# s-elkazdadi/ddp-pinocchio

Measured on AMD Instinct MI355X. Metric: DDP iterations/sec (fwd+bwd sweep), Talos nq=38 T=200, higher is better.
Workload: dtype f64

## Files before the change

### ddp_pinocchio_amd/csrc/bwd.hip

```cpp
#include <stdio.h>
#include <stdlib.h>

#include "internal.h"

namespace {

struct BwdParams {
  Dims d;
  const int64_t* ne;
  const int64_t* Epre;
  const double *lfx, *lfxx, *lx, *lu, *lxx, *lux, *luu, *fx, *fu, *fxx, *fux, *fuu;
  const double *eq_val, *eq_x, *eq_u, *eq_xx, *eq_ux, *eq_uu;
  const double *x, *mult_val, *mult_jac;
  double *fb_origin, *fb_val, *fb_jac, *vx_trace, *vxx_trace;
  double *ws_V, *ws_Q, *reg, *mu;
  int32_t* status;
  int64_t* restarts;
  const BwdJob* jobs;
  const BwdJob* jobs_half;
  int32_t njobs_half;
  int32_t half_mode;
  const double *u, *ctrl_lo, *ctrl_hi;
  double* box_stat;
  int32_t has_tensors;
  int32_t sym_tensors;
};

constexpr int BS = 256;
typedef double f64x2 __attribute__((ext_vector_type(2)));

__global__ __launch_bounds__(BS) void bwd_init(BwdParams p) {
  const int b = blockIdx.x;
  const int s = p.status[b];
  if (s == 2) return;
  const int64_t n = p.d.n;
  double* Vx = p.ws_V + (int64_t)b * (n + n * n);
  double* Vxx = Vx + n;
  const double* lfx = p.lfx + (int64_t)b * n;
  const double* lfxx = p.lfxx + (int64_t)b * n * n;
  for (int64_t i = threadIdx.x; i < n; i += BS) Vx[i] = lfx[i];
  for (int64_t i = threadIdx.x; i < n * n; i += BS) Vxx[i] = lfxx[i];
  __syncthreads();
  if (threadIdx.x == 0 && s == 1) p.status[b] = 0;
}

template <int OC>
__device__ __forceinline__ void contract_slab(const double* __restrict__ Tn, int O_rt, int L, const double* s_v,
                                              double* s_part, double* out, int out_stride) {
  const int O = OC > 0 ? OC : O_rt;
  const int hp = O >> 1;
  const int ld = hp + 1;
  const int total = hp * L;
  const f64x2* __restrict__ T2 = reinterpret_cast<const f64x2*>(Tn);
  const int tid = threadIdx.x;
#pragma unroll 4
  for (int f = tid; f < total; f += BS) {
    const f64x2 a = __builtin_nontemporal_load(&T2[f]);
    const int j = f / hp;
    const int ip = f - j * hp;
    s_part[j * ld + ip] = s_v[2 * ip] * a.x + s_v[2 * ip + 1] * a.y;
  }
  __syncthreads();
  for (int j = tid; j < L; j += BS) {
    double s = 0.0;
    const double* pj = s_part + j * ld;
    for (int k = 0; k < hp; ++k) s += pj[k];
    out[j * out_stride] += s;
  }
  __syncthreads();
}

template <int NC, int MC>
__global__ __launch_bounds__(BS) void bwd_assemble(BwdParams p, int64_t t) {
  const int b = blockIdx.y;
  if (p.status[b] != 0) return;
  const BwdJob job = p.jobs[blockIdx.x];
  const int n = NC > 0 ? NC : (int)p.d.n;
  const int m = MC > 0 ? MC : (int)p.d.m;
  const int64_t T = p.d.T;
  const int e = (int)p.ne[t];
  const int64_t Eo = p.Epre[t];
  const int64_t Etot = p.d.Etot;
  const double mu = p.mu[b];
  const int tid = threadIdx.x;
  const int kind = job.kind, c0 = job.c0, cn = job.cn;
  const int rows = kind == 0 ? n + m : m;

  const double* Vx = p.ws_V + (int64_t)b * (n + (int64_t)n * n);
  const double* Vxx = Vx + n;
  double* Q = p.ws_Q + (int64_t)b * (n + m + (int64_t)n * n + (int64_t)m * n + (int64_t)m * m);
  double* Qx = Q;
  double* Qu = Qx + n;
  double* Qxx = Qu + m;
  double* Qux = Qxx + (int64_t)n * n;
  double* Quu = Qux + (int64_t)m * n;

  const int64_t bt = (int64_t)b * T + t;
  const double* fx = p.fx + bt * n * n;
  const double* fu = p.fu + bt * n * m;
  const double* eqv = p.eq_val + (int64_t)b * Etot + Eo;
  const double* eqx = p.eq_x + ((int64_t)b * Etot + Eo) * n;
  const double* equ = p.eq_u + ((int64_t)b * Etot + Eo) * m;
  const double* pe = p.mult_val + (int64_t)b * Etot + Eo;
  const double* pex = p.mult_jac + ((int64_t)b * Etot + Eo) * n;
// ... 332 lines not shown
    for (int i = 0; i < m; ++i) {
      double s = r[i];
      for (int l = 0; l < i; ++l) s -= A[i + l * lda] * r[l];
      r[i] = s / A[i + i * lda];
    }
    for (int i = m - 1; i >= 0; --i) {
      double s = r[i];
      for (int l = i + 1; l < m; ++l) s -= A[l + i * lda] * r[l];
      r[i] = s / A[i + i * lda];
    }
  }
  __syncthreads();

  double* fbo = p.fb_origin + bt * nx;
  double* fbk = p.fb_val + bt * m;
  double* fbK = p.fb_jac + bt * m * n;
  const double* xt = p.x + ((int64_t)b * (T + 1) + t) * nx;
  for (int i = tid; i < nx; i += BS) fbo[i] = xt[i];
  for (int i = tid; i < m; i += BS) fbk[i] = R[i];
  for (int idx = tid; idx < m * n; idx += BS) fbK[idx] = R[idx % m + (idx / m + 1) * ldr];

  for (int i = tid; i < n; i += BS) {
    double s = 0.0;
    for (int l = 0; l < m; ++l) s += S[l + i * ldr] * R[l];
    const double v = Qx[i] + s;
    Vx[i] = v;
    if (p.vx_trace) p.vx_trace[bt * n + i] = v;
  }
  for (int idx = tid; idx < n * n; idx += BS) {
    const int i = idx % n, j = idx / n;
    double s = 0.0;
    const double* si = S + i * ldr;
    const double* kj = R + (j + 1) * ldr;
    for (int l = 0; l < m; ++l) s += si[l] * kj[l];
    const double v = Qxx[idx] + s;
    Vxx[idx] = v;
    if (p.vxx_trace) p.vxx_trace[bt * n * n + idx] = v;
  }
  if (t == 0 && tid == 0) p.status[b] = 2;
}

#include "bwd_fast.h"
#include "bwd_split.h"
#include "bwd_v2.h"

size_t assemble_lds_bytes(const ddp_hip_ctx* ctx, int cn_max) {
  const Dims& d = ctx->d;
  int64_t L = d.n > d.m ? d.n : d.m;
  int64_t words = d.n + d.emax + d.n * cn_max + (d.n + d.m) * cn_max + (d.n / 2 + 1) * L;
  return (size_t)words * sizeof(double);
}
size_t gains_lds_bytes(const ddp_hip_ctx* ctx) {
  const Dims& d = ctx->d;
  int64_t ld = d.m | 1;
  int64_t words = ld * d.m + ld * (d.n + 1) + ld * d.n;
  if (ctx->flags & DDP_HIP_FLAG_CONTROL_BOUNDS) words += ld * d.m + 9 * d.m;
  return (size_t)words * sizeof(double);
}

BwdParams make_params(ddp_hip_ctx* ctx, const SweepPlan& plan) {
  BwdParams p{};
  p.d = ctx->d;
  p.ne = ctx->ne_d;
  p.Epre = ctx->Epre_d;
  auto S = [&](int s) { return ctx->seq[s].ptr; };
  p.lfx = S(DDP_HIP_SEQ_LFX); p.lfxx = S(DDP_HIP_SEQ_LFXX);
  p.lx = S(DDP_HIP_SEQ_LX); p.lu = S(DDP_HIP_SEQ_LU); p.lxx = S(DDP_HIP_SEQ_LXX); p.lux = S(DDP_HIP_SEQ_LUX); p.luu = S(DDP_HIP_SEQ_LUU);
  p.fx = S(DDP_HIP_SEQ_FX); p.fu = S(DDP_HIP_SEQ_FU);
  p.fxx = S(DDP_HIP_SEQ_FXX); p.fux = S(DDP_HIP_SEQ_FUX); p.fuu = S(DDP_HIP_SEQ_FUU);
  p.eq_val = S(DDP_HIP_SEQ_EQ_VAL); p.eq_x = S(DDP_HIP_SEQ_EQ_X); p.eq_u = S(DDP_HIP_SEQ_EQ_U);
  p.eq_xx = S(DDP_HIP_SEQ_EQ_XX); p.eq_ux = S(DDP_HIP_SEQ_EQ_UX); p.eq_uu = S(DDP_HIP_SEQ_EQ_UU);
  p.x = S(DDP_HIP_SEQ_X);
  p.u = S(DDP_HIP_SEQ_U); p.ctrl_lo = S(DDP_HIP_SEQ_CTRL_LO); p.ctrl_hi = S(DDP_HIP_SEQ_CTRL_HI); p.box_stat = S(DDP_HIP_SEQ_BOX_STAT);
  p.mult_val = S(DDP_HIP_SEQ_MULT_VAL); p.mult_jac = S(DDP_HIP_SEQ_MULT_JAC);
  p.fb_origin = S(DDP_HIP_SEQ_FB_ORIGIN); p.fb_val = S(DDP_HIP_SEQ_FB_VAL); p.fb_jac = S(DDP_HIP_SEQ_FB_JAC);
  p.vx_trace = S(DDP_HIP_SEQ_VX_TRACE); p.vxx_trace = S(DDP_HIP_SEQ_VXX_TRACE);
  p.ws_V = ctx->ws_V; p.ws_Q = ctx->ws_Q; p.reg = ctx->reg_d; p.mu = ctx->mu_d;
  p.status = ctx->status_d; p.restarts = ctx->restarts_d;
  p.sym_tensors = plan.sym ? 1 : 0;
  p.jobs = plan.sym ? ctx->jobs_sym_d : ctx->jobs_d;
  p.jobs_half = plan.half_mode ? ctx->jobs_half_d : nullptr;
  p.njobs_half = plan.half_mode ? ctx->njobs_half : 0;
  p.half_mode = plan.half_mode;
  p.has_tensors = (ctx->flags & DDP_HIP_FLAG_NO_TENSORS) ? 0 : 1;
  return p;
}

template <int NC, int MC, bool BOX = false>
int launch_sweep(ddp_hip_ctx* ctx, const BwdParams& p, size_t lds_a, size_t lds_g) {
  const Dims& d = ctx->d;
  hipLaunchKernelGGL(bwd_init, dim3((unsigned)d.batch), dim3(BS), 0, ctx->stream, p);
  for (int64_t t = d.T - 1; t >= 0; --t) {
    prof_begin(ctx, DDP_HIP_K_BWD_ASSEMBLE);
    hipLaunchKernelGGL((bwd_assemble<NC, MC>), dim3((unsigned)ctx->njobs, (unsigned)d.batch), dim3(BS), lds_a, ctx->stream, p, t);
    prof_end(ctx, DDP_HIP_K_BWD_ASSEMBLE);
    prof_begin(ctx, DDP_HIP_K_BWD_GAINS);
    hipLaunchKernelGGL((bwd_gains<NC, MC, BOX>), dim3((unsigned)d.batch), dim3(BS), lds_g, ctx->stream, p, t);
    prof_end(ctx, DDP_HIP_K_BWD_GAINS);
  }
  HIP_TRY(hipGetLastError());
  return DDP_HIP_OK;
}

template <int NC, int MC, bool BOX>
int enqueue_sweep_v2(ddp_hip_ctx* ctx, const BwdParams& p) {
  const Dims& d = ctx->d;
  const int cn_max = ctx->cbx > ctx->cbu ? ctx->cbx : ctx->cbu;
  const size_t lds_c = sizeof(double) * (size_t)(NC + (NC + MC) * cn_max + 2 * (NC / 2 + 1) * MC);
  const size_t lds_h = sizeof(double) * (size_t)(NC + 3 * NC + 2 * (MC / 2 + 1) * NC);
  const size_t lds_5 = sizeof(double) * (size_t)(NC * NC + NC * (NC + MC) + NC + d.emax);
  const unsigned nblk5 = (unsigned)((NC + MC + CB5 - 1) / CB5);
  const unsigned B = (unsigned)d.batch;
  hipLaunchKernelGGL(bwd_init, dim3(B), dim3(BS), 0, ctx->stream, p);
  for (int64_t t = d.T - 1; t >= 0; --t) {
    prof_begin(ctx, DDP_HIP_K_BWD_GAINS);
    hipLaunchKernelGGL((bwd_dense2<NC, MC>), dim3(nblk5, B), dim3(BS5), lds_5, ctx->stream, p, t);
    prof_end(ctx, DDP_HIP_K_BWD_GAINS);
    if (p.has_tensors) {
      prof_begin(ctx, DDP_HIP_K_BWD_ASSEMBLE);
      if (p.jobs_half) hipLaunchKernelGGL((bwd_contract_half<NC, MC>), dim3((unsigned)p.njobs_half, B), dim3(BSF), lds_h, ctx->stream, p, t);
      else hipLaunchKernelGGL((bwd_contract<NC, MC>), dim3((unsigned)ctx->njobs, B), dim3(BSF), lds_c, ctx->stream, p, t);
      prof_end(ctx, DDP_HIP_K_BWD_ASSEMBLE);
    }
    prof_begin(ctx, DDP_HIP_K_BWD_GAINS);
    hipLaunchKernelGGL((bwd_gains2<NC, MC, BOX>), dim3(B), dim3(BS4), 0, ctx->stream, p, t);
    prof_end(ctx, DDP_HIP_K_BWD_GAINS);
  }
  HIP_TRY(hipGetLastError());
  return DDP_HIP_OK;
}

template <int NC, int MC, bool BOX>
int build_sweep_graph(ddp_hip_ctx* ctx, const BwdParams& p0, uint64_t key_misc, ddp_hip_ctx::BwdGraph** out) {
  ddp_hip_ctx::BwdGraph* slot = &ctx->bwd_graph[ctx->bwd_graph_next];
  ctx->bwd_graph_next = (ctx->bwd_graph_next + 1) % 4;
  if (slot->exec) { (void)hipGraphExecDestroy(slot->exec); slot->exec = nullptr; }
  if (slot->graph) { (void)hipGraphDestroy(slot->graph); slot->graph = nullptr; }
  HIP_TRY(hipStreamBeginCapture(ctx->stream, hipStreamCaptureModeThreadLocal));
  const int rc = enqueue_sweep_v2<NC, MC, BOX>(ctx, p0);
  hipGraph_t graph = nullptr;
  const hipError_t e = hipStreamEndCapture(ctx->stream, &graph);
  if (rc != DDP_HIP_OK || e != hipSuccess || !graph) { (void)hipGetLastError(); if (graph) (void)hipGraphDestroy(graph); return rc != DDP_HIP_OK ? rc : DDP_HIP_E_HIP; }
  hipGraphExec_t exec = nullptr;
  if (hipGraphInstantiate(&exec, graph, nullptr, nullptr, 0) != hipSuccess) { (void)hipGetLastError(); (void)hipGraphDestroy(graph); return DDP_HIP_E_HIP; }
  slot->graph = graph; slot->exec = exec; slot->key_x = p0.x; slot->key_misc = key_misc;
  *out = slot;
  return DDP_HIP_OK;
}

template <int NC, int MC, bool BOX = false>
int launch_sweep_v2(ddp_hip_ctx* ctx, const BwdParams& p0) {
  const uint32_t bwd_mask = (2u << DDP_HIP_K_BWD_ASSEMBLE) | (2u << DDP_HIP_K_BWD_GAINS);
  if (ctx->sw.bwd_no_graph || (ctx->profile_mask & bwd_mask)) return enqueue_sweep_v2<NC, MC, BOX>(ctx, p0);
  const uint64_t key_misc = (uint64_t)p0.has_tensors | ((uint64_t)(p0.vx_trace != nullptr) << 1) | ((uint64_t)p0.sym_tensors << 2) | ((uint64_t)(p0.jobs_half != nullptr) << 3) | ((uint64_t)p0.half_mode << 4);
  auto find = [&](const void* key_x) -> ddp_hip_ctx::BwdGraph* {
    for (auto& g : ctx->bwd_graph)
      if (g.exec && g.key_x == key_x && g.key_misc == key_misc) return &g;
    return nullptr;
  };
  ddp_hip_ctx::BwdGraph* slot = find(p0.x);
  if (!slot) {
    int rc = build_sweep_graph<NC, MC, BOX>(ctx, p0, key_misc, &slot);
    if (rc != DDP_HIP_OK) return rc;
    const double* other = ctx->seq[DDP_HIP_SEQ_X_NEW].ptr;
    if (other && other != p0.x && !find(other)) {
      BwdParams p1 = p0;
      p1.x = other;
      p1.u = ctx->seq[DDP_HIP_SEQ_U_NEW].ptr;
      ddp_hip_ctx::BwdGraph* twin = nullptr;
      rc = build_sweep_graph<NC, MC, BOX>(ctx, p1, key_misc, &twin);
      if (rc != DDP_HIP_OK) return rc;
      slot = find(p0.x);
      if (!slot) return DDP_HIP_E_HIP;
    }
  }
  HIP_TRY(hipGraphLaunch(slot->exec, ctx->stream));
  return DDP_HIP_OK;
}

}

SweepPlan sweep_plan(const ddp_hip_ctx* ctx) {
  const Dims& d = ctx->d;
  const DevSwitches& sw = ctx->sw;
  SweepPlan s{};
  s.fast = d.n == 76 && d.m == 38 && d.emax <= 52 && !sw.generic_bwd;
  s.sym_ok = s.fast && ctx->jobs_sym_d && !sw.k3_no_sym;
  const TensorOrigin o = ctx->tensors.origin;
  s.sym = s.sym_ok && (o == TensorOrigin::Symmetric || o == TensorOrigin::Stencil);
  const bool half_ok = s.fast && ctx->jobs_half_d && !sw.k3_no_half;
  if (half_ok && s.sym && o == TensorOrigin::Stencil) s.half_mode = 1;
  else if (half_ok && o == TensorOrigin::Analytic1) s.half_mode = 2;
  return s;
}

int bwd_setup(ddp_hip_ctx* ctx) {
  const Dims& d = ctx->d;
  const int64_t n = d.n, m = d.m, B = d.batch;
  HIP_TRY(hipMalloc(&ctx->ws_V, sizeof(double) * (size_t)(B * (n + n * n))));
  HIP_TRY(hipMalloc(&ctx->ws_Q, sizeof(double) * (size_t)(B * (n + m + n * n + m * n + m * m))));
  HIP_TRY(hipMalloc(&ctx->reg_d, sizeof(double) * (size_t)B));
  HIP_TRY(hipMalloc(&ctx->mu_d, sizeof(double) * (size_t)B));
  HIP_TRY(hipMalloc(&ctx->status_d, sizeof(int32_t) * (size_t)B));
  HIP_TRY(hipMalloc(&ctx->restarts_d, sizeof(int64_t) * (size_t)B));

  int64_t units = 3 * n + m;
  int64_t want = 2048 / B;
  if (want < 1) want = 1;
  if (want > n + m) want = n + m;
  int64_t upj = (units + want - 1) / want;
  int64_t cbx = upj / 3; if (cbx < 1) cbx = 1; if (cbx > 8) cbx = 8;
  int64_t cbu = upj;     if (cbu < 1) cbu = 1; if (cbu > 16) cbu = 16;
  if (n == 76 && m == 38) { cbx = 1; cbu = 3; }
  if (ctx->sw.bwd_cbx) cbx = ctx->sw.bwd_cbx;
  if (ctx->sw.bwd_cbu) cbu = ctx->sw.bwd_cbu;
  ctx->cbx = (int32_t)cbx; ctx->cbu = (int32_t)cbu;
  std::vector<BwdJob> jobs;
  for (int64_t c = 0; c < n; c += cbx) jobs.push_back(BwdJob{0, (int32_t)c, (int32_t)((n - c) < cbx ? (n - c) : cbx), 0});
  for (int64_t c = 0; c < m; c += cbu) jobs.push_back(BwdJob{1, (int32_t)c, (int32_t)((m - c) < cbu ? (m - c) : cbu), 0});
  ctx->njobs = (int32_t)jobs.size();
  if (n == 76 && m == 38) {
    const size_t lds_5 = sizeof(double) * (size_t)(76 * 76 + 76 * (76 + 38) + 76 + d.emax);
    HIP_TRY(hipFuncSetAttribute(reinterpret_cast<const void*>(&bwd_dense2<76, 38>), hipFuncAttributeMaxDynamicSharedMemorySize, (int)lds_5));
  }
  if ((ctx->flags & DDP_HIP_FLAG_CONTROL_BOUNDS) && gains_lds_bytes(ctx) <= 160 * 1024) {
    HIP_TRY(hipFuncSetAttribute(reinterpret_cast<const void*>(&bwd_gains<0, 0, true>), hipFuncAttributeMaxDynamicSharedMemorySize, (int)gains_lds_bytes(ctx)));
  }
  HIP_TRY(hipMalloc(&ctx->jobs_d, sizeof(BwdJob) * jobs.size()));
  HIP_TRY(hipMemcpy(ctx->jobs_d, jobs.data(), sizeof(BwdJob) * jobs.size(), hipMemcpyHostToDevice));
  if (n == 76 && m == 38 && cbx == 1) {
    std::vector<BwdJob> js = jobs;
    for (auto& j : js) if (j.kind == 0 && j.c0 >= m) j.kind = 2;
    HIP_TRY(hipMalloc(&ctx->jobs_sym_d, sizeof(BwdJob) * js.size()));
    HIP_TRY(hipMemcpy(ctx->jobs_sym_d, js.data(), sizeof(BwdJob) * js.size(), hipMemcpyHostToDevice));
    std::vector<BwdJob> jh;
    for (int64_t c = 0; c < n; c += 2) jh.push_back(BwdJob{10, (int32_t)c, 2, 0});
    for (int64_t c = 0; c < m; c += 6) jh.push_back(BwdJob{11, (int32_t)c, (int32_t)((m - c) < 6 ? (m - c) : 6), 0});
    ctx->njobs_half = (int32_t)jh.size();
    HIP_TRY(hipMalloc(&ctx->jobs_half_d, sizeof(BwdJob) * jh.size()));
    HIP_TRY(hipMemcpy(ctx->jobs_half_d, jh.data(), sizeof(BwdJob) * jh.size(), hipMemcpyHostToDevice));
  }
  return DDP_HIP_OK;
}

void bwd_teardown(ddp_hip_ctx* ctx) {
  for (auto& g : ctx->bwd_graph) {
    if (g.exec) (void)hipGraphExecDestroy(g.exec);
    if (g.graph) (void)hipGraphDestroy(g.graph);
  }
  if (ctx->ws_V) (void)hipFree(ctx->ws_V);
  if (ctx->ws_Q) (void)hipFree(ctx->ws_Q);
  if (ctx->reg_d) (void)hipFree(ctx->reg_d);
  if (ctx->mu_d) (void)hipFree(ctx->mu_d);
  if (ctx->status_d) (void)hipFree(ctx->status_d);
  if (ctx->restarts_d) (void)hipFree(ctx->restarts_d);
  if (ctx->jobs_d) (void)hipFree(ctx->jobs_d);
  if (ctx->jobs_sym_d) (void)hipFree(ctx->jobs_sym_d);
  if (ctx->jobs_half_d) (void)hipFree(ctx->jobs_half_d);
}

extern "C" int ddp_hip_backward(ddp_hip_ctx* ctx, double* reg_io, double* mu_io, int64_t* restarts_out, int64_t max_restarts) {
  if (!ctx || !reg_io || !mu_io) return DDP_HIP_E_ARG;
  const Dims& d = ctx->d;
  const int64_t B = d.batch;
  HIP_TRY(hipSetDevice(ctx->device));
  const SweepPlan plan = sweep_plan(ctx);
  BwdParams p = make_params(ctx, plan);
  if (p.has_tensors && (!p.fxx || !p.fux || !p.fuu)) return DDP_HIP_E_UNSUPPORTED;
  const bool box = (ctx->flags & DDP_HIP_FLAG_CONTROL_BOUNDS) != 0;
  if (box) { const int rc_ = box_check(ctx); if (rc_ != DDP_HIP_OK) return rc_; }
  if (p.has_tensors && ctx->tensors.mirror_pending && !plan.sym) { const int rc_ = lin_materialize_fxx(ctx); if (rc_ != DDP_HIP_OK) return rc_; }

  HIP_TRY(hipMemcpyAsync(ctx->reg_d, reg_io, sizeof(double) * (size_t)B, hipMemcpyHostToDevice, ctx->stream));
  HIP_TRY(hipMemcpyAsync(ctx->mu_d, mu_io, sizeof(double) * (size_t)B, hipMemcpyHostToDevice, ctx->stream));
  std::vector<int32_t> status((size_t)B);
  for (int64_t b = 0; b < B; ++b) status[(size_t)b] = ctx->active_h[(size_t)b] ? 0 : 2;
  HIP_TRY(hipMemcpyAsync(ctx->status_d, status.data(), sizeof(int32_t) * (size_t)B, hipMemcpyHostToDevice, ctx->stream));
  HIP_TRY(hipMemsetAsync(ctx->restarts_d, 0, sizeof(int64_t) * (size_t)B, ctx->stream));

  const int cn_max = ctx->cbx > ctx->cbu ? ctx->cbx : ctx->cbu;
  const size_t lds_a = assemble_lds_bytes(ctx, cn_max);
  const size_t lds_g = gains_lds_bytes(ctx);
  if (lds_a > 160 * 1024 || lds_g > 160 * 1024) return DDP_HIP_E_UNSUPPORTED;

  bool any_restart = false;
  int rc = DDP_HIP_OK;
  for (int64_t attempt = 0;; ++attempt) {
    if (plan.fast) rc = box ? launch_sweep_v2<76, 38, true>(ctx, p) : launch_sweep_v2<76, 38>(ctx, p);
    else if (d.n == 12 && d.m == 6) rc = box ? launch_sweep<12, 6, true>(ctx, p, lds_a, lds_g) : launch_sweep<12, 6>(ctx, p, lds_a, lds_g);
    else rc = box ? launch_sweep<0, 0, true>(ctx, p, lds_a, lds_g) : launch_sweep<0, 0>(ctx, p, lds_a, lds_g);
    if (rc != DDP_HIP_OK) return rc;
    HIP_TRY(hipMemcpyAsync(status.data(), ctx->status_d, sizeof(int32_t) * (size_t)B, hipMemcpyDeviceToHost, ctx->stream));
    HIP_TRY(hipStreamSynchronize(ctx->stream));
    bool failed = false;
    for (int64_t b = 0; b < B; ++b) failed |= status[(size_t)b] == 1;
    if (!failed) break;
    any_restart = true;
    if (max_restarts >= 0 && attempt >= max_restarts) { rc = DDP_HIP_E_MAX_RESTARTS; break; }
  }
  HIP_TRY(hipMemcpyAsync(reg_io, ctx->reg_d, sizeof(double) * (size_t)B, hipMemcpyDeviceToHost, ctx->stream));
  HIP_TRY(hipMemcpyAsync(mu_io, ctx->mu_d, sizeof(double) * (size_t)B, hipMemcpyDeviceToHost, ctx->stream));
  if (restarts_out)
    HIP_TRY(hipMemcpyAsync(restarts_out, ctx->restarts_d, sizeof(int64_t) * (size_t)B, hipMemcpyDeviceToHost, ctx->stream));
  HIP_TRY(hipStreamSynchronize(ctx->stream));
  if (rc != DDP_HIP_OK) return rc;
  return any_restart ? DDP_HIP_EV_LLT_RESTART : DDP_HIP_OK;
}

#ifdef BWD_STAMPS
extern "C" int ddp_hip_debug_stamps(unsigned long long* out32) {
  return hipMemcpyFromSymbol(out32, HIP_SYMBOL(g_bwd_stamps), sizeof(unsigned long long) * 32) == hipSuccess ? 0 : -2;
}
#endif
```

### ddp_pinocchio_amd/csrc/bwd_split.h

```cpp
#pragma once

template <int N, int M>
__global__ __launch_bounds__(BSF, BWD_WAVES_PER_SIMD) void bwd_contract(BwdParams p, int64_t t) {
  int b, jb;
  {
    const int njobs = (int)gridDim.x, B = (int)gridDim.y;
    const int lin = blockIdx.y * njobs + blockIdx.x;
    if ((B & 7) == 0) {
      const int xcd = lin & 7, k = lin >> 3;
      b = xcd + 8 * (k / njobs);
      jb = k % njobs;
    } else { b = blockIdx.y; jb = blockIdx.x; }
  }
  if (p.status[b] != 0) return;
  const BwdJob job = p.jobs[jb];
  constexpr int n = N, m = M;
  const int64_t T = p.d.T;
  const int tid = threadIdx.x;
  const int kind = job.kind, c0 = job.c0, cn = job.cn;
  const int rows = kind == 1 ? m : n + m;
  static_assert(N == 2 * M, "half-slabs: the state tangent is twice the control dimension");
  const int64_t bt = (int64_t)b * T + t;

  const double* Vx = p.ws_V + (int64_t)b * (n + n * n);
// ... 11 lines not shown

  const int upc = kind == 0 ? 3 : (kind == 2 ? 2 : 1);
  const int part0 = kind == 2 ? 1 : 0;
  const int U = upc * cn;
  const double* Txx = p.fxx + (bt * n + c0) * (int64_t)n * n;
  const double* Tux = p.fux + (bt * n + c0) * (int64_t)n * m;
  const double* Tuu = p.fuu + (bt * m + c0) * (int64_t)n * m;
  auto unit_ptr = [&](int u) -> const double* {
    const int c = u / upc, part = u - c * upc + part0;
    if (kind != 1) return part < 2 ? Txx + (int64_t)c * n * n + part * (M * n) : Tux + (int64_t)c * n * m;
    return Tuu + (int64_t)c * n * m;
  };
  const bool sym = p.sym_tensors != 0;
  auto unit_jmin = [&](int u) -> int {
    if (!sym) return 0;
    const int c = u / upc, part = u - c * upc + part0, col = c0 + c;
    if (kind == 1) return col;
    if (part == 0) return col < M ? col : M;
    if (part == 1) return col > M ? col - M : 0;
    return 0;
  };
  f64x2 buf0[US::R], buf1[US::R], buf2[US::R], buf3[US::R];
#define C_ISSUE(BUF, u) do { if ((u) < U) slab_issue_from<N, M, BWD_NT>(unit_ptr(u), BUF, unit_jmin(u)); } while (0)
  C_ISSUE(buf0, 0); C_ISSUE(buf1, 1); C_ISSUE(buf2, 2); C_ISSUE(buf3, 3);

  for (int i = tid; i < n; i += BSF) s_v[i] = Vx[i];
  for (int i = tid; i < rows * cn; i += BSF) s_out[i] = 0.0;
  __syncthreads();

#define C_STEP(BUF, u)                                                                      \
  do {                                                                                      \
    if ((u) < U) {                                                                          \
      double* sp = ((u) & 1) ? s_p1 : s_p0;                                                 \
      _Pragma("unroll") for (int r = 0; r < US::R; ++r) {                                   \
        const int f = tid + r * BSF;                                                        \
        if (r < US::R - 1 || f < US::TOTAL) {                                               \
          const int j = f / US::HP;                                                         \
          const int ip = f - j * US::HP;                                                    \
          const f64x2 vv = *reinterpret_cast<const f64x2*>(s_v + 2 * ip);                   \
          sp[j * US::LD + ip] = vv.x * BUF[r].x + vv.y * BUF[r].y;                          \
        }                                                                                   \
      }                                                                                     \
      __syncthreads();                                                                      \
      if (tid < M) {                                                                        \
        const double* pj = sp + tid * US::LD;                                               \
        double sacc = 0.0;                                                                  \
        _Pragma("unroll") for (int k = 0; k < US::HP; ++k) sacc += pj[k];                   \
        const int c_ = (u) / upc, part_ = (u) - c_ * upc + part0;                           \
        s_out[c_ * rows + part_ * M + tid] = sacc;                                          \
      }                                                                                     \
      C_ISSUE(BUF, (u) + 4);                                                                \
    }                                                                                       \
  } while (0)
  for (int u = 0; u < U; u += 4) {
    C_STEP(buf0, u);
    C_STEP(buf1, u + 1);
    C_STEP(buf2, u + 2);
    C_STEP(buf3, u + 3);
  }
  __syncthreads();
#undef C_STEP
#undef C_ISSUE
  for (int idx = tid; idx < rows * cn; idx += BSF) {
    const int r = idx % rows, c = idx / rows;
    const int col = c0 + c;
    if (kind == 2 && r < M) continue;
    const bool square = kind == 1 || r < n;
    if (sym && square && r < col) continue;
    double* dst = kind != 1 ? (r < n ? Cxx + r + col * n : Cux + (r - n) + col * m) : Cuu + r + col * m;
    *dst = *dst + s_out[idx];
    if (sym && square && r > col) {
      double* dm = kind != 1 ? Cxx + col + r * n : Cuu + col + r * m;
      *dm = *dm + s_out[idx];
    }
  }
}

template <int N, int M>
struct HalfShape {
  static constexpr int HP = M / 2, LD = M / 2 + 1, TOTAL = (M / 2) * N, R = ((M / 2) * N + BSF - 1) / BSF;
};
static_assert(38 % 2 == 0, "row pairs");

template <int N, int M>
__global__ __launch_bounds__(BSF, BWD_WAVES_PER_SIMD) void bwd_contract_half(BwdParams p, int64_t t) {
  int b, jb;
  {
    const int njobs = (int)gridDim.x, B = (int)gridDim.y;
    const int lin = blockIdx.y * njobs + blockIdx.x;
    if ((B & 7) == 0) {
      const int xcd = lin & 7, k = lin >> 3;
      b = xcd + 8 * (k / njobs);
      jb = k % njobs;
    } else { b = blockIdx.y; jb = blockIdx.x; }
  }
  if (p.status[b] != 0) return;
  const BwdJob job = p.jobs_half[jb];
  constexpr int n = N, m = M;
  static_assert(N == 2 * M && M % 2 == 0, "lower halves of M rows, in row pairs");
  const int64_t T = p.d.T;
  const int tid = threadIdx.x;
  const int kind = job.kind, c0 = job.c0, cn = job.cn;
  const bool m1 = p.half_mode == 2;
  const int64_t bt = (int64_t)b * T + t;
  const double* Vx = p.ws_V + (int64_t)b * (n + n * n);
  double* C = p.ws_Q + (int64_t)b * (n + m + n * n + m * n + m * m) + n + m;
  double* Cxx = C;
  double* Cux = Cxx + n * n;
  double* Cuu = Cux + m * n;
  using HS = HalfShape<N, M>;
  extern __shared__ __attribute__((aligned(16))) double smem[];
  double* s_v = smem;
  double* s_out = s_v + n;
  double* s_p0 = s_out + 3 * N;
  double* s_p1 = s_p0 + HS::LD * N;
  const int U = kind == 10 ? 3 : cn / 2;
  auto unit_base = [&](int u) -> const double* {
    if (kind == 10) return u < 2 ? p.fxx + (bt * n + c0 + u) * (int64_t)n * n : p.fux + (bt * n + c0) * (int64_t)n * m;
    return p.fuu + (bt * m + c0 + 2 * u) * (int64_t)n * m;
  };
  auto col_info = [&](int u, int jj, int& slab, int& j, bool& xcol) -> bool {
    if (kind == 10) {
      if (u < 2) { slab = c0 + u; j = jj; xcol = true; return m1 || j >= slab; }
      slab = c0 + (jj >= m ? 1 : 0); j = jj >= m ? jj - m : jj; xcol = false; return true;
    }
    slab = c0 + 2 * u + (jj >= m ? 1 : 0); j = jj >= m ? jj - m : jj; xcol = false; return m1 || j >= slab;
  };
  f64x2 buf0[HS::R], buf1[HS::R], buf2[HS::R], buf3[HS::R];
  double top0[2], top1[2], top2[2], top3[2];
  auto issue = [&](int u, f64x2 (&buf)[HS::R], double (&top)[2]) {
    const f64x2* base = reinterpret_cast<const f64x2*>(unit_base(u));
#pragma unroll
    for (int r = 0; r < HS::R; ++r) {
      const int f = tid + r * BSF;
      bool need = r < HS::R - 1 || f < HS::TOTAL;
      const int jj = f / HS::HP, ip = f - jj * HS::HP;
      int slab, j; bool xcol;
      if (need) need = col_info(u, jj < n ? jj : n - 1, slab, j, xcol) && !(m1 && kind == 11);
      if (need) buf[r] = BWD_NT ? __builtin_nontemporal_load(&base[jj * (N / 2) + HS::HP + ip]) : base[jj * (N / 2) + HS::HP + ip];
      else buf[r] = f64x2{0.0, 0.0};
    }
    top[0] = 0.0; top[1] = 0.0;
    if (tid < n) {
      int slab, j; bool xcol;
      if (col_info(u, tid, slab, j, xcol) && kind == 10 && !m1) {
        const double* colp = unit_base(u) + (int64_t)tid * n;
        top[0] = colp[slab % M];
        if (xcol && (j % M) != (slab % M)) top[1] = colp[j % M];
      }
    }
  };
  if (U > 0) issue(0, buf0, top0);
  if (U > 1) issue(1, buf1, top1);
  if (U > 2) issue(2, buf2, top2);
  double* dst = nullptr;
  double* dm = nullptr;
  double old_d = 0.0, old_m = 0.0;
  static_assert(3 * N <= BSF, "one output entry per lane");
  if (tid < U * N) {
    const int u = tid / N, jj = tid - u * N;
    int slab, j; bool xcol;
    if (col_info(u, jj, slab, j, xcol)) {
      if (kind == 10) {
        if (u < 2) { dst = Cxx + j + slab * n; if (j > slab && !m1) dm = Cxx + slab + j * n; }
        else dst = Cux + j + slab * m;
      } else { dst = Cuu + j + slab * m; if (j > slab && !m1) dm = Cuu + slab + j * m; }
      old_d = *dst;
      if (dm) old_m = *dm;
    }
  }
  for (int i = tid; i < n; i += BSF) s_v[i] = Vx[i];
  __syncthreads();
  auto step = [&](int u, f64x2 (&buf)[HS::R], double (&top)[2]) {
    double* sp = (u & 1) ? s_p1 : s_p0;
#pragma unroll
    for (int r = 0; r < HS::R; ++r) {
      const int f = tid + r * BSF;
      if (r < HS::R - 1 || f < HS::TOTAL) {
        const int jj = f / HS::HP, ip = f - jj * HS::HP;
        const f64x2 vv = *reinterpret_cast<const f64x2*>(s_v + M + 2 * ip);
        sp[jj * HS::LD + ip] = vv.x * buf[r].x + vv.y * buf[r].y;
      }
    }
    __syncthreads();
    if (tid < n) {
      int slab, j; bool xcol;
      const bool need = col_info(u, tid, slab, j, xcol);
      double sacc = 0.0;
      if (need && kind == 10 && !m1) {
        const int ra = slab % M, rb = xcol ? j % M : ra;
        const int lo = ra < rb ? ra : rb, hi = ra < rb ? rb : ra;
        const double tlo = ra <= rb ? top[0] : top[1], thi = ra <= rb ? (ra == rb ? 0.0 : top[1]) : top[0];
        if (lo == hi) {
          const int e = lo & ~1;
          const f64x2 vv = *reinterpret_cast<const f64x2*>(s_v + e);
          const double tx = (lo & 1) ? 0.0 : tlo, ty = (lo & 1) ? tlo : 0.0;
          sacc += vv.x * tx + vv.y * ty;
        } else if ((lo >> 1) == (hi >> 1)) {
          const f64x2 vv = *reinterpret_cast<const f64x2*>(s_v + lo);
          sacc += vv.x * tlo + vv.y * thi;
        } else {
          const f64x2 va = *reinterpret_cast<const f64x2*>(s_v + (lo & ~1));
          const f64x2 vb = *reinterpret_cast<const f64x2*>(s_v + (hi & ~1));
          sacc += va.x * ((lo & 1) ? 0.0 : tlo) + va.y * ((lo & 1) ? tlo : 0.0);
          sacc += vb.x * ((hi & 1) ? 0.0 : thi) + vb.y * ((hi & 1) ? thi : 0.0);
        }
      }
      const double* pj = sp + tid * HS::LD;
#pragma unroll
      for (int k = 0; k < HS::HP; ++k) sacc += pj[k];
      s_out[u * N + tid] = sacc;
    }
  };
  if (U > 0) step(0, buf0, top0);
  if (U > 1) step(1, buf1, top1);
  if (U > 2) step(2, buf2, top2);
  (void)buf3; (void)top3;
  __syncthreads();
  if (dst) {
    const double v = s_out[tid];
    *dst = old_d + v;
    if (dm) *dm = old_m + v;
  }
}
```

### ddp_pinocchio_amd/csrc/ctx.hip

```cpp
#include <math.h>
#include <stdio.h>
#include <stdlib.h>
#include <string.h>

#include <limits>
#include <new>

#include "internal.h"

extern "C" int ddp_hip_abi_version(void) { return DDP_HIP_ABI_VERSION; }

extern "C" const char* ddp_hip_strerror(int code) {
  switch (code) {
    case DDP_HIP_OK: return "ok";
    case DDP_HIP_EV_LLT_RESTART: return "backward sweep restarted after a non-positive LLT pivot";
    case DDP_HIP_EV_LINESEARCH_FLOOR: return "line search reached step < 1e-10";
    case DDP_HIP_E_ARG: return "invalid argument";
    case DDP_HIP_E_HIP: return "HIP runtime error";
    case DDP_HIP_E_NODEVICE: return "no HIP device (there is no CPU fallback)";
    case DDP_HIP_E_UNSUPPORTED: return "unsupported configuration";
    case DDP_HIP_E_MAX_RESTARTS: return "backward sweep exceeded max_restarts";
    case DDP_HIP_E_COMM: return "RCCL error";
    default: return "unknown";
  }
// ... 104 lines not shown
bool ddp_hip_build_tables(DevModel& dm) { return build_slot_tables(dm); }

static int64_t seq_size_of(const Dims& d, int s) {
  const int64_t T = d.T, n = d.n, m = d.m, nx = d.nx, E = d.Etot;
  switch (s) {
    case DDP_HIP_SEQ_X: case DDP_HIP_SEQ_X_NEW: return (T + 1) * nx;
    case DDP_HIP_SEQ_U: case DDP_HIP_SEQ_U_NEW: return T * m;
    case DDP_HIP_SEQ_LFX: return n;
    case DDP_HIP_SEQ_LFXX: return n * n;
    case DDP_HIP_SEQ_LX: return T * n;
    case DDP_HIP_SEQ_LU: return T * m;
    case DDP_HIP_SEQ_LXX: return T * n * n;
    case DDP_HIP_SEQ_LUX: return T * m * n;
    case DDP_HIP_SEQ_LUU: return T * m * m;
    case DDP_HIP_SEQ_F_VAL: return T * nx;
    case DDP_HIP_SEQ_FX: return T * n * n;
    case DDP_HIP_SEQ_FU: return T * n * m;
    case DDP_HIP_SEQ_FXX: return T * n * n * n;
    case DDP_HIP_SEQ_FUX: return T * n * m * n;
    case DDP_HIP_SEQ_FUU: return T * n * m * m;
    case DDP_HIP_SEQ_EQ_VAL: return E;
    case DDP_HIP_SEQ_EQ_X: return E * n;
    case DDP_HIP_SEQ_EQ_U: return E * m;
    case DDP_HIP_SEQ_EQ_XX: return E * n * n;
    case DDP_HIP_SEQ_EQ_UX: return E * m * n;
    case DDP_HIP_SEQ_EQ_UU: return E * m * m;
    case DDP_HIP_SEQ_MULT_ORIGIN: return T * nx;
    case DDP_HIP_SEQ_MULT_VAL: return E;
    case DDP_HIP_SEQ_MULT_JAC: return E * n;
    case DDP_HIP_SEQ_FB_ORIGIN: return T * nx;
    case DDP_HIP_SEQ_FB_VAL: return T * m;
    case DDP_HIP_SEQ_FB_JAC: return T * m * n;
    case DDP_HIP_SEQ_VX_TRACE: return T * n;
    case DDP_HIP_SEQ_VXX_TRACE: return T * n * n;
    case DDP_HIP_SEQ_COSTS_OLD: case DDP_HIP_SEQ_COSTS_NEW: return T + 1;
    case DDP_HIP_SEQ_COST_XREF: return (T + 1) * nx;
    case DDP_HIP_SEQ_COST_WX: return (T + 1) * n;
    case DDP_HIP_SEQ_COST_UREF: case DDP_HIP_SEQ_COST_WU: return T * m;
    case DDP_HIP_SEQ_CTRL_LO: case DDP_HIP_SEQ_CTRL_HI: return T * m;
    case DDP_HIP_SEQ_BOX_STAT: return T * 2;
    default: return -1;
  }
}

static bool is_tensor_seq(int s) {
  return s == DDP_HIP_SEQ_FXX || s == DDP_HIP_SEQ_FUX || s == DDP_HIP_SEQ_FUU || s == DDP_HIP_SEQ_EQ_XX ||
         s == DDP_HIP_SEQ_EQ_UX || s == DDP_HIP_SEQ_EQ_UU;
}
static bool is_trace_seq(int s) { return s == DDP_HIP_SEQ_VX_TRACE || s == DDP_HIP_SEQ_VXX_TRACE; }
static bool is_cost_seq(int s) { return s >= DDP_HIP_SEQ_COST_XREF && s <= DDP_HIP_SEQ_COST_WU; }
static bool is_box_seq(int s) { return s >= DDP_HIP_SEQ_CTRL_LO && s <= DDP_HIP_SEQ_BOX_STAT; }
static bool nan_init_seq(int s) {
  return s == DDP_HIP_SEQ_LFX || s == DDP_HIP_SEQ_LFXX || s == DDP_HIP_SEQ_F_VAL || s == DDP_HIP_SEQ_FB_ORIGIN ||
         s == DDP_HIP_SEQ_FB_VAL || s == DDP_HIP_SEQ_FB_JAC || s == DDP_HIP_SEQ_X || s == DDP_HIP_SEQ_U ||
         s == DDP_HIP_SEQ_X_NEW || s == DDP_HIP_SEQ_U_NEW || is_trace_seq(s);
}

__global__ void fill_kernel(double* p, int64_t n, double v) {
  int64_t i = (int64_t)blockIdx.x * blockDim.x + threadIdx.x;
  int64_t stride = (int64_t)gridDim.x * blockDim.x;
  for (; i < n; i += stride) p[i] = v;
}

static int fill_device(ddp_hip_ctx* ctx, double* p, int64_t n, double v) {
  if (n <= 0) return DDP_HIP_OK;
  if (v == 0.0) {
    HIP_TRY(hipMemsetAsync(p, 0, (size_t)n * sizeof(double), ctx->stream));
    return DDP_HIP_OK;
  }
  int64_t blocks = (n + 255) / 256;
  if (blocks > 2048) blocks = 2048;
  hipLaunchKernelGGL(fill_kernel, dim3((unsigned)blocks), dim3(256), 0, ctx->stream, p, n, v);
  HIP_TRY(hipGetLastError());
  return DDP_HIP_OK;
}

static DevSwitches read_switches() {
  auto on = [](const char* name) { return getenv(name) != nullptr; };
  auto knob = [](const char* name, int lo, int hi) { const char* ev = getenv(name); const int v = ev ? atoi(ev) : 0; return v >= lo && v <= hi ? v : 0; };
  DevSwitches sw;
  sw.generic_bwd = on("DDP_HIP_GENERIC_BWD");
  sw.k3_no_sym = on("DDP_HIP_K3_NO_SYM");
  sw.k3_no_half = on("DDP_HIP_K3_NO_HALF");
  sw.fxx_full = on("DDP_HIP_FXX_FULL");
  sw.no_static = on("DDP_HIP_NO_STATIC");
  sw.no_qcache = on("DDP_HIP_NO_QCACHE");
  sw.cfg_full_aba = on("DDP_HIP_CFG_FULL_ABA");
  sw.ana_own_aba = on("DDP_HIP_ANA_OWN_ABA");
  sw.ana_split = on("DDP_HIP_ANA_SPLIT");
  sw.ana_eq_kernel = on("DDP_HIP_ANA_EQ_KERNEL");
  sw.bwd_no_graph = on("DDP_HIP_BWD_NO_GRAPH");
  sw.solve_sync = on("DDP_HIP_SOLVE_SYNC");
  sw.bwd_cbx = knob("DDP_HIP_BWD_CBX", 1, 8);
  sw.bwd_cbu = knob("DDP_HIP_BWD_CBU", 1, 16);
  sw.qws_bt = knob("DDP_HIP_QWS_BT", 16, 65536);
  sw.ana_bt = knob("DDP_HIP_ANA_BT", 1, 65536);
  return sw;
}

static int frame_orient_reset(ddp_hip_ctx* ctx) {
  const int64_t slots = ctx->d.batch * (ctx->d.T + 1) * DDP_HIP_MAX_COST_FRAMES;
  std::vector<double> qt((size_t)(slots * 4), 0.0);
  for (size_t k = 3; k < qt.size(); k += 4) qt[k] = 1.0;
  HIP_TRY(hipMemcpyAsync(ctx->fo_quat_d, qt.data(), sizeof(double) * qt.size(), hipMemcpyHostToDevice, ctx->stream));
  HIP_TRY(hipMemsetAsync(ctx->fo_weight_d, 0, sizeof(double) * (size_t)(slots * 3), ctx->stream));
  HIP_TRY(hipStreamSynchronize(ctx->stream));
  ctx->fo_live = false;
  return DDP_HIP_OK;
}

extern "C" int ddp_hip_create(const ddp_hip_problem* prob, int device, uint32_t flags, ddp_hip_ctx** out) {
  if (!prob || !out) return DDP_HIP_E_ARG;
  *out = nullptr;
  const ddp_hip_model& mo = prob->model;
  if (prob->T < 1 || prob->batch < 1 || mo.nv < 1 || mo.nv > DDP_MAXJ) return DDP_HIP_E_ARG;
  if (mo.kind != DDP_HIP_MODEL_PENDULUM && mo.kind != DDP_HIP_MODEL_TREE) return DDP_HIP_E_ARG;
  if (mo.kind == DDP_HIP_MODEL_PENDULUM && mo.nv != 1) return DDP_HIP_E_ARG;
  if (prob->fd_mode < 0 || prob->fd_mode > 2) return DDP_HIP_E_ARG;
  if ((flags & DDP_HIP_FLAG_FRAME_COST) && mo.kind != DDP_HIP_MODEL_TREE) return DDP_HIP_E_UNSUPPORTED;
  if ((flags & DDP_HIP_FLAG_FRAME_ORIENT_COST) && !(flags & DDP_HIP_FLAG_FRAME_COST)) return DDP_HIP_E_ARG;
  if (prob->eq_kind != DDP_HIP_EQ_NONE && (!prob->ne || prob->eq_advance < 0 || prob->eq_advance > 4)) return DDP_HIP_E_ARG;
  if (prob->eq_kind == DDP_HIP_EQ_FRAME && (mo.kind != DDP_HIP_MODEL_TREE || prob->frame_joint < 0 ||
                                            prob->frame_joint >= (mo.jtype && mo.jtype[0] == DDP_HIP_JOINT_FREEFLYER ? mo.nv - 5 : mo.nv)))
    return DDP_HIP_E_ARG;
  bool ff = false;
  if (mo.kind == DDP_HIP_MODEL_TREE) {
    if (!mo.parent || !mo.jtype || !mo.axis || !mo.Rp || !mo.pp || !mo.mass_j || !mo.com || !mo.Ic) return DDP_HIP_E_ARG;
    ff = mo.jtype[0] == DDP_HIP_JOINT_FREEFLYER;
    const int nj = ff ? mo.nv - 5 : mo.nv;
    if (nj < 1 || (ff && mo.parent[0] != -1)) return DDP_HIP_E_ARG;
    for (int i = 0; i < nj; ++i) {
      if (mo.parent[i] >= i || mo.parent[i] < -1) return DDP_HIP_E_ARG;
      if (i > 0 && mo.jtype[i] != DDP_HIP_JOINT_REVOLUTE && mo.jtype[i] != DDP_HIP_JOINT_PRISMATIC) return DDP_HIP_E_ARG;
    }
    if (ff && (prob->fd_mode == 1 || prob->eq_kind == DDP_HIP_EQ_CONFIG)) return DDP_HIP_E_UNSUPPORTED;
  }
  int ndev = ddp_hip_device_count();
  if (ndev <= 0) return DDP_HIP_E_NODEVICE;
  if (device < 0 || device >= ndev) return DDP_HIP_E_ARG;
  HIP_TRY(hipSetDevice(device));

  ddp_hip_ctx* ctx = new (std::nothrow) ddp_hip_ctx();
  if (!ctx) return DDP_HIP_E_HIP;
  ctx->device = device;
  ctx->flags = flags;
  ctx->sw = read_switches();
  ctx->active_h.assign((size_t)prob->batch, 1);
  Dims& d = ctx->d;
  d.T = prob->T; d.nv = mo.nv; d.n = 2 * (int64_t)mo.nv; d.m = mo.nv; d.nx = 2 * (int64_t)mo.nv + (ff ? 1 : 0); d.batch = prob->batch;
  ctx->ne_h.assign((size_t)d.T, 0);
  ctx->Epre_h.assign((size_t)d.T + 1, 0);
  d.emax = 0;
  for (int64_t t = 0; t < d.T; ++t) {
    int64_t e = (prob->eq_kind != DDP_HIP_EQ_NONE && prob->ne) ? prob->ne[t] : 0;
    if (e < 0) { delete ctx; return DDP_HIP_E_ARG; }
    if (prob->eq_kind == DDP_HIP_EQ_CONFIG && e != 0 && e != mo.nv) { delete ctx; return DDP_HIP_E_ARG; }
    if (prob->eq_kind == DDP_HIP_EQ_FRAME && e != 0 && e != 3) { delete ctx; return DDP_HIP_E_ARG; }
    ctx->ne_h[(size_t)t] = e;
    ctx->Epre_h[(size_t)t + 1] = ctx->Epre_h[(size_t)t] + e;
    if (e > d.emax) d.emax = e;
  }
  d.Etot = ctx->Epre_h[(size_t)d.T];

#define CTX_TRY(expr)                                                              \
  do {                                                                             \
    hipError_t e__ = (expr);                                                       \
// ... 40 lines not shown
  if (flags & DDP_HIP_FLAG_TRACKING_COST) {
    std::vector<double> xr((size_t)(ctx->seq[DDP_HIP_SEQ_COST_XREF].size * d.batch), 0.0);
    if (ff)
      for (size_t k = 0; k < xr.size(); k += (size_t)d.nx) xr[k + 6] = 1.0;
    CTX_TRY(hipMemcpyAsync(ctx->seq[DDP_HIP_SEQ_COST_XREF].ptr, xr.data(), sizeof(double) * xr.size(), hipMemcpyHostToDevice, ctx->stream));
    CTX_TRY(hipStreamSynchronize(ctx->stream));
  }
  if (flags & DDP_HIP_FLAG_FRAME_COST) {
    const size_t words = (size_t)(d.batch * (d.T + 1) * DDP_HIP_MAX_COST_FRAMES * 3);
    CTX_TRY(hipMalloc(&ctx->fc_target_d, sizeof(double) * words));
    CTX_TRY(hipMalloc(&ctx->fc_weight_d, sizeof(double) * words));
    CTX_TRY(hipMemsetAsync(ctx->fc_target_d, 0, sizeof(double) * words, ctx->stream));
    CTX_TRY(hipMemsetAsync(ctx->fc_weight_d, 0, sizeof(double) * words, ctx->stream));
  }
  if (flags & DDP_HIP_FLAG_FRAME_ORIENT_COST) {
    const int64_t slots = d.batch * (d.T + 1) * DDP_HIP_MAX_COST_FRAMES;
    CTX_TRY(hipMalloc(&ctx->fo_quat_d, sizeof(double) * (size_t)(slots * 4)));
    CTX_TRY(hipMalloc(&ctx->fo_weight_d, sizeof(double) * (size_t)(slots * 3)));
    if (frame_orient_reset(ctx) != DDP_HIP_OK) { ddp_hip_destroy(ctx); return DDP_HIP_E_HIP; }
  }
  if (flags & DDP_HIP_FLAG_STATE_LIMITS) {
    const int64_t words = d.batch * (d.T + 1) * d.n;
    CTX_TRY(hipMalloc(&ctx->sl_d, sizeof(double) * (size_t)(3 * words)));
    if (fill_device(ctx, ctx->sl_d, words, -INFINITY) != DDP_HIP_OK || fill_device(ctx, ctx->sl_d + words, words, INFINITY) != DDP_HIP_OK ||
        fill_device(ctx, ctx->sl_d + 2 * words, words, 0.0) != DDP_HIP_OK) {
      ddp_hip_destroy(ctx);
      return DDP_HIP_E_HIP;
    }
  }
  int rc = bwd_setup(ctx);
  if (rc == DDP_HIP_OK) rc = fwd_setup(ctx);
  if (rc == DDP_HIP_OK) rc = lin_setup(ctx);
  if (rc != DDP_HIP_OK) { ddp_hip_destroy(ctx); return rc; }
  CTX_TRY(hipStreamSynchronize(ctx->stream));
#undef CTX_TRY
  *out = ctx;
  return DDP_HIP_OK;
}

extern "C" int ddp_hip_destroy(ddp_hip_ctx* ctx) {
  if (!ctx) return DDP_HIP_E_ARG;
  (void)hipSetDevice(ctx->device);
  if (ctx->stream) (void)hipStreamSynchronize(ctx->stream);
  lin_teardown(ctx);
  fwd_teardown(ctx);
  bwd_teardown(ctx);
  for (int s = 0; s < DDP_HIP_SEQ_COUNT; ++s)
    if (ctx->seq[s].ptr) (void)hipFree(ctx->seq[s].ptr);
  if (ctx->fc_target_d) (void)hipFree(ctx->fc_target_d);
  if (ctx->fc_weight_d) (void)hipFree(ctx->fc_weight_d);
  if (ctx->fo_quat_d) (void)hipFree(ctx->fo_quat_d);
  if (ctx->fo_weight_d) (void)hipFree(ctx->fo_weight_d);
  if (ctx->sl_d) (void)hipFree(ctx->sl_d);
  if (ctx->ne_d) (void)hipFree(ctx->ne_d);
  if (ctx->Epre_d) (void)hipFree(ctx->Epre_d);
  if (ctx->target_d) (void)hipFree(ctx->target_d);
  if (ctx->model_d) (void)hipFree(ctx->model_d);
  for (int k = 0; k < DDP_HIP_K_COUNT; ++k) {
    for (auto e : ctx->prof[k].starts) (void)hipEventDestroy(e);
    for (auto e : ctx->prof[k].stops) (void)hipEventDestroy(e);
  }
  if (ctx->stream) (void)hipStreamDestroy(ctx->stream);
  delete ctx;
  return DDP_HIP_OK;
}

extern "C" void* ddp_hip_stream(ddp_hip_ctx* ctx) { return ctx ? (void*)ctx->stream : nullptr; }

extern "C" int ddp_hip_synchronize(ddp_hip_ctx* ctx) {
  if (!ctx) return DDP_HIP_E_ARG;
  HIP_TRY(hipStreamSynchronize(ctx->stream));
  return DDP_HIP_OK;
}

extern "C" int64_t ddp_hip_batch(const ddp_hip_ctx* ctx) { return ctx ? ctx->d.batch : -1; }

extern "C" int64_t ddp_hip_seq_size(const ddp_hip_ctx* ctx, int seq) {
  if (!ctx || seq < 0 || seq >= DDP_HIP_SEQ_COUNT) return -1;
  return ctx->seq[seq].size;
}

extern "C" double* ddp_hip_device_ptr(ddp_hip_ctx* ctx, int seq) {
  if (!ctx || seq < 0 || seq >= DDP_HIP_SEQ_COUNT) return nullptr;
  if (seq == DDP_HIP_SEQ_FXX || seq == DDP_HIP_SEQ_FUU) (void)hipSetDevice(ctx->device);
  if (tensors_written_outside(ctx, seq) != DDP_HIP_OK) return nullptr;
  return ctx->seq[seq].ptr;
}

static int check_range(ddp_hip_ctx* ctx, int seq, int64_t first, int64_t count) {
  if (!ctx || seq < 0 || seq >= DDP_HIP_SEQ_COUNT) return DDP_HIP_E_ARG;
  if (first < 0 || count < 0 || first + count > ctx->d.batch) return DDP_HIP_E_ARG;
  if (ctx->seq[seq].size > 0 && !ctx->seq[seq].ptr) return DDP_HIP_E_UNSUPPORTED;
  return DDP_HIP_OK;
}

static bool cost_weight_ok(double w) { return isfinite(w) && w >= 0.0; }
static bool cost_quat_ok(double norm2) { return isfinite(norm2) && fabs(sqrt(norm2) - 1.0) <= 1e-10; }

static bool bound_ok(int seq, double v) { return !isnan(v) && !(seq == DDP_HIP_SEQ_CTRL_LO ? v == INFINITY : v == -INFINITY); }

static bool cost_values_ok(const ddp_hip_ctx* ctx, int seq, const double* host, int64_t words) {
  if (seq == DDP_HIP_SEQ_CTRL_LO || seq == DDP_HIP_SEQ_CTRL_HI) {
    for (int64_t i = 0; i < words; ++i)
      if (!bound_ok(seq, host[i])) return false;
    return true;
  }
  if (seq == DDP_HIP_SEQ_COST_WX || seq == DDP_HIP_SEQ_COST_WU) {
    for (int64_t i = 0; i < words; ++i)
      if (!cost_weight_ok(host[i])) return false;
  } else if (seq == DDP_HIP_SEQ_COST_XREF && ctx->model_h.ff) {
    for (int64_t k = 0; k < words; k += ctx->d.nx) {
      const double* qt = host + k + 3;
      if (!cost_quat_ok(qt[0] * qt[0] + qt[1] * qt[1] + qt[2] * qt[2] + qt[3] * qt[3])) return false;
    }
  }
  return true;
}

extern "C" int ddp_hip_upload(ddp_hip_ctx* ctx, int seq, const double* host, int64_t first, int64_t count) {
  int rc = check_range(ctx, seq, first, count);
  if (rc != DDP_HIP_OK) return rc;
  int64_t sz = ctx->seq[seq].size;
  if (is_box_seq(seq) && !(ctx->flags & DDP_HIP_FLAG_CONTROL_BOUNDS)) return DDP_HIP_E_UNSUPPORTED;
  if (sz == 0 || count == 0) return DDP_HIP_OK;
  if (!host) return DDP_HIP_E_ARG;
  if (!cost_values_ok(ctx, seq, host, sz * count)) return DDP_HIP_E_ARG;
  HIP_TRY(hipSetDevice(ctx->device));
  { const int rc_ = tensors_written_outside(ctx, seq); if (rc_ != DDP_HIP_OK) return rc_; }
  HIP_TRY(hipMemcpyAsync(ctx->seq[seq].ptr + first * sz, host, sizeof(double) * (size_t)(sz * count), hipMemcpyHostToDevice, ctx->stream));
  HIP_TRY(hipStreamSynchronize(ctx->stream));
  if (seq == DDP_HIP_SEQ_CTRL_LO || seq == DDP_HIP_SEQ_CTRL_HI) ctx->box_dirty = true;
  return DDP_HIP_OK;
}

int box_check(ddp_hip_ctx* ctx) {
  if (!ctx->box_dirty) return DDP_HIP_OK;
  const size_t words = (size_t)(ctx->seq[DDP_HIP_SEQ_CTRL_LO].size * ctx->d.batch);
  std::vector<double> lo(words), hi(words);
  HIP_TRY(hipMemcpyAsync(lo.data(), ctx->seq[DDP_HIP_SEQ_CTRL_LO].ptr, sizeof(double) * words, hipMemcpyDeviceToHost, ctx->stream));
  HIP_TRY(hipMemcpyAsync(hi.data(), ctx->seq[DDP_HIP_SEQ_CTRL_HI].ptr, sizeof(double) * words, hipMemcpyDeviceToHost, ctx->stream));
  HIP_TRY(hipStreamSynchronize(ctx->stream));
  for (size_t i = 0; i < words; ++i)
    if (lo[i] > hi[i]) return DDP_HIP_E_ARG;
  ctx->box_dirty = false;
  return DDP_HIP_OK;
}

extern "C" int ddp_hip_download(ddp_hip_ctx* ctx, int seq, double* host, int64_t first, int64_t count) {
  int rc = check_range(ctx, seq, first, count);
  if (rc != DDP_HIP_OK) return rc;
  int64_t sz = ctx->seq[seq].size;
  if (sz == 0 || count == 0) return DDP_HIP_OK;
  if (!host) return DDP_HIP_E_ARG;
  HIP_TRY(hipSetDevice(ctx->device));
  if (seq == DDP_HIP_SEQ_FXX || seq == DDP_HIP_SEQ_FUU) { const int rc_ = lin_materialize_fxx(ctx); if (rc_ != DDP_HIP_OK) return rc_; }
  HIP_TRY(hipMemcpyAsync(host, ctx->seq[seq].ptr + first * sz, sizeof(double) * (size_t)(sz * count), hipMemcpyDeviceToHost, ctx->stream));
  HIP_TRY(hipStreamSynchronize(ctx->stream));
  return DDP_HIP_OK;
}

extern "C" int ddp_hip_fill(ddp_hip_ctx* ctx, int seq, double value) {
  int rc = check_range(ctx, seq, 0, 0);
  if (rc != DDP_HIP_OK) return rc;
  if ((seq == DDP_HIP_SEQ_COST_WX || seq == DDP_HIP_SEQ_COST_WU) && !cost_weight_ok(value)) return DDP_HIP_E_ARG;
  if (seq == DDP_HIP_SEQ_COST_XREF && ctx->model_h.ff && !cost_quat_ok(4 * value * value)) return DDP_HIP_E_ARG;
  if ((seq == DDP_HIP_SEQ_CTRL_LO || seq == DDP_HIP_SEQ_CTRL_HI) && !bound_ok(seq, value)) return DDP_HIP_E_ARG;
  if (seq == DDP_HIP_SEQ_CTRL_LO || seq == DDP_HIP_SEQ_CTRL_HI) ctx->box_dirty = true;
  HIP_TRY(hipSetDevice(ctx->device));
  { const int rc_ = tensors_written_outside(ctx, seq); if (rc_ != DDP_HIP_OK) return rc_; }
  return fill_device(ctx, ctx->seq[seq].ptr, ctx->seq[seq].size * ctx->d.batch, value);
}

extern "C" int ddp_hip_frame_cost_set_frames(ddp_hip_ctx* ctx, int32_t n_frames, const int32_t* joint, const double* off) {
  if (!ctx) return DDP_HIP_E_ARG;
  if (!(ctx->flags & DDP_HIP_FLAG_FRAME_COST)) return DDP_HIP_E_UNSUPPORTED;
  if (n_frames < 1 || n_frames > DDP_HIP_MAX_COST_FRAMES || !joint || !off) return DDP_HIP_E_ARG;
  for (int f = 0; f < n_frames; ++f) {
    if (joint[f] < 0 || joint[f] >= ctx->model_h.nj) return DDP_HIP_E_ARG;
    for (int a = 0; a < 3; ++a)
      if (!isfinite(off[3 * f + a])) return DDP_HIP_E_ARG;
  }
  if (n_frames != ctx->fc_nf) {
    HIP_TRY(hipSetDevice(ctx->device));
    const size_t words = (size_t)(ctx->d.batch * (ctx->d.T + 1) * DDP_HIP_MAX_COST_FRAMES * 3);
    HIP_TRY(hipMemsetAsync(ctx->fc_target_d, 0, sizeof(double) * words, ctx->stream));
    HIP_TRY(hipMemsetAsync(ctx->fc_weight_d, 0, sizeof(double) * words, ctx->stream));
    ctx->fc_live = false;
    if (ctx->flags & DDP_HIP_FLAG_FRAME_ORIENT_COST) { const int rc_ = frame_orient_reset(ctx); if (rc_ != DDP_HIP_OK) return rc_; }
  }
  ctx->fc_nf = n_frames;
  for (int f = 0; f < n_frames; ++f) {
    ctx->fc_joint[f] = joint[f];
    for (int a = 0; a < 3; ++a) ctx->fc_off[f][a] = off[3 * f + a];
  }
  return DDP_HIP_OK;
}

static int frame_cost_range(ddp_hip_ctx* ctx, int64_t first, int64_t count) {
  if (!ctx) return DDP_HIP_E_ARG;
  if (!(ctx->flags & DDP_HIP_FLAG_FRAME_COST)) return DDP_HIP_E_UNSUPPORTED;
  if (first < 0 || count < 0 || first + count > ctx->d.batch) return DDP_HIP_E_ARG;
  return DDP_HIP_OK;
}

extern "C" int ddp_hip_frame_cost_upload(ddp_hip_ctx* ctx, const double* target, const double* weight, int64_t first, int64_t count) {
  int rc = frame_cost_range(ctx, first, count);
  if (rc != DDP_HIP_OK) return rc;
  if (ctx->fc_nf == 0) return DDP_HIP_E_ARG;
  const int64_t sz = (ctx->d.T + 1) * ctx->fc_nf * 3;
  bool nonzero = false;
  if (target)
    for (int64_t i = 0; i < sz * count; ++i)
      if (!isfinite(target[i])) return DDP_HIP_E_ARG;
  if (weight)
    for (int64_t i = 0; i < sz * count; ++i) {
      if (!cost_weight_ok(weight[i])) return DDP_HIP_E_ARG;
      nonzero |= weight[i] != 0.0;
    }
  if (count == 0 || (!target && !weight)) return DDP_HIP_OK;
  HIP_TRY(hipSetDevice(ctx->device));
  if (target) HIP_TRY(hipMemcpyAsync(ctx->fc_target_d + first * sz, target, sizeof(double) * (size_t)(sz * count), hipMemcpyHostToDevice, ctx->stream));
  if (weight) HIP_TRY(hipMemcpyAsync(ctx->fc_weight_d + first * sz, weight, sizeof(double) * (size_t)(sz * count), hipMemcpyHostToDevice, ctx->stream));
  HIP_TRY(hipStreamSynchronize(ctx->stream));
  if (weight) ctx->fc_live = nonzero || (ctx->fc_live && !(first == 0 && count == ctx->d.batch));
  return DDP_HIP_OK;
}

extern "C" int ddp_hip_frame_cost_download(ddp_hip_ctx* ctx, double* target, double* weight, int64_t first, int64_t count) {
  int rc = frame_cost_range(ctx, first, count);
  if (rc != DDP_HIP_OK) return rc;
  const int64_t sz = (ctx->d.T + 1) * ctx->fc_nf * 3;
  if (sz == 0 || count == 0 || (!target && !weight)) return DDP_HIP_OK;
  HIP_TRY(hipSetDevice(ctx->device));
  if (target) HIP_TRY(hipMemcpyAsync(target, ctx->fc_target_d + first * sz, sizeof(double) * (size_t)(sz * count), hipMemcpyDeviceToHost, ctx->stream));
  if (weight) HIP_TRY(hipMemcpyAsync(weight, ctx->fc_weight_d + first * sz, sizeof(double) * (size_t)(sz * count), hipMemcpyDeviceToHost, ctx->stream));
  HIP_TRY(hipStreamSynchronize(ctx->stream));
  return DDP_HIP_OK;
}
// ... 239 lines not shown
```

### ddp_pinocchio_amd/csrc/internal.h

```cpp
#pragma once

#include <hip/hip_runtime.h>
#include <stdint.h>

#include <vector>

#include "ddp_hip/ddp_hip.h"

#define DDP_MAXJ DDP_HIP_MAX_JOINTS

struct DevModel {
  int32_t kind, nv;
  int32_t ff, nj, nq, pad0_;
  double mass, length;
  double gravity[3];
  double dt, c;
  int32_t parent[DDP_MAXJ];
  int32_t jtype[DDP_MAXJ];
  double axis[DDP_MAXJ][3];
  double Rp[DDP_MAXJ][9];
  double pp[DDP_MAXJ][3];
  double I6[DDP_MAXJ][21];
  int32_t has_child[DDP_MAXJ];
  int32_t first_contrib[DDP_MAXJ];
  int32_t last_child[DDP_MAXJ];
  int32_t slot_up[DDP_MAXJ];
  int32_t slot_down[DDP_MAXJ];
  int32_t n_slots;
  int32_t n_levels, max_level_width;
  int32_t lvl_start[DDP_MAXJ + 1];
  int32_t lvl_joint[DDP_MAXJ];
  int32_t child_start[DDP_MAXJ + 1];
  int32_t child_list[DDP_MAXJ];
  int32_t eq_kind, eq_advance, frame_joint, first_order_fd, fd_mode, pad_;
  double frame_off[3];
};

struct Dims {
  int64_t T, n, m, nx, nv, batch;
  int64_t Etot;
  int64_t emax;
};

struct SeqBuf {
  double* ptr = nullptr;
  int64_t size = 0;
};

struct BwdJob {
  int32_t kind;
  int32_t c0, cn;
  int32_t pad_;
};

struct DevSwitches {
  bool generic_bwd = false;
  bool k3_no_sym = false;
  bool k3_no_half = false;
  bool fxx_full = false;
  bool no_static = false;
  bool no_qcache = false;
  bool cfg_full_aba = false;
  bool ana_own_aba = false;
  bool ana_split = false;
  bool ana_eq_kernel = false;
  bool bwd_no_graph = false;
  bool solve_sync = false;
  int32_t bwd_cbx = 0, bwd_cbu = 0;
  int64_t qws_bt = 0;
  int64_t ana_bt = 0;
};

struct SweepPlan {
  bool fast;
  bool sym_ok;
  bool sym;
  int32_t half_mode;
};

enum class LinFirst : int32_t {
  Base,
  AnalyticSmall,
  AnalyticWave,
  AnalyticFF,
  FdStatic,
  FdGeneric,
};
enum class LinSecond : int32_t {
  None,
  Zeros,
  Mode2Static,
  Mode2Caches,
  Mode2Plain,
  Mode1Small,
  Mode1Wave,
};
enum class LinEq : int32_t {
  None,
  PerLane,
  Analytic,
  Chain,
};
enum class LinEqJac : int32_t { None, Fd, FfLookahead };
enum class LinEqSecond : int32_t { None, Zeros, Mode2, Mode1Small, Mode1Wave };
struct LinPlan {
  int32_t refuse = 0;
  int32_t nj = 0;
  int32_t topo = 0;
  LinFirst first = LinFirst::Base;
  LinSecond second = LinSecond::None;
  LinEq eq = LinEq::None;
  LinEqJac eq_jac = LinEqJac::None;
  LinEqSecond eq_second = LinEqSecond::None;
  bool eq_inline = false;
  bool accel_static = false;
  bool accel_with_u = false;
  bool m1_fused = false;
  int32_t ncfg = 0, nvcfg = 0;
  bool has_tensors = false;
  bool skip_top = false;
  bool skip_qv_mirror = false;
  bool ws_lin = false, ws_qws = false, ws_qws2 = false;
  bool ws_ana_T = false, ws_ana_M = false, ws_ana_M0 = false, ws_ana_A = false, ws_ana_F = false;
  bool ws_eq = false;
  bool ana_sliced = false;
  int64_t eq_fxk_off = 0, eq_c_off = 0, eq_words = 0;
  int32_t lin_path = 0, first_order = 0;
};
LinPlan lin_plan_decide(const DevModel& m, const Dims& d, uint32_t flags, const DevSwitches& sw, int topo_id, bool sweep_sym_ok);

enum class TensorOrigin : int32_t {
  Unknown,
  Symmetric,
  Stencil,
  Analytic1,
};
struct TensorState {
  TensorOrigin origin = TensorOrigin::Unknown;
  bool mirror_pending = false;
};

struct LinCall {
  bool ana_A_fresh = false;
  bool ana_M0_fresh = false;
  bool fuu_zero = false;
};

struct ProfSlot {
  std::vector<hipEvent_t> starts, stops;
  size_t used = 0;
  double total_ms = 0;
  int64_t launches = 0;
};

struct ddp_hip_ctx {
  int device = 0;
  uint32_t flags = 0;
  hipStream_t stream = nullptr;
  Dims d{};
  std::vector<int64_t> ne_h, Epre_h;
  int64_t* ne_d = nullptr;
  int64_t* Epre_d = nullptr;
  double* target_d = nullptr;
  DevModel model_h{};
  DevModel* model_d = nullptr;
  SeqBuf seq[DDP_HIP_SEQ_COUNT];
  DevSwitches sw;

  double* ws_V = nullptr;
  double* ws_Q = nullptr;
  double* reg_d = nullptr;
  double* mu_d = nullptr;
  int32_t* status_d = nullptr;
  int64_t* restarts_d = nullptr;
  BwdJob* jobs_d = nullptr;
  BwdJob* jobs_half_d = nullptr;
  int32_t njobs_half = 0;
  TensorState tensors;
  BwdJob* jobs_sym_d = nullptr;
  int32_t njobs = 0;
  int32_t cbx = 0, cbu = 0;
  struct BwdGraph { const void* key_x = nullptr; uint64_t key_misc = 0; hipGraphExec_t exec = nullptr; hipGraph_t graph = nullptr; };
  BwdGraph bwd_graph[4];
  int bwd_graph_next = 0;

  double* fw_x = nullptr;
  double* fw_u = nullptr;
  double* fw_dcost = nullptr;
  double* fw_cost = nullptr;
  double* fw_cost_old = nullptr;
  double* step_d = nullptr;
  int32_t* fw_state_d = nullptr;
  double* fw_dcost_acc_d = nullptr;
  int32_t n_alpha_max = 8;
  double* pick_pair_d = nullptr;

  double* eq_ws = nullptr;
  double* lin_ws = nullptr;
  LinPlan plan;
  double* lin_qws = nullptr;
  int64_t lin_qws_bt = 0;
  double* lin_qws2 = nullptr;
  hipStream_t lin_stream2 = nullptr;
  hipEvent_t lin_ev_up[2] = {nullptr, nullptr}, lin_ev_dn[2] = {nullptr, nullptr};
  double* ana_T = nullptr;
  double* ana_M = nullptr;
  double* ana_F = nullptr;
  double* ana_M0 = nullptr;
  double* ana_A = nullptr;
  int64_t ana_nbt = 0;

  std::vector<int32_t> active_h;
  bool all_active = true;

  int32_t fc_nf = 0;
  int32_t fc_joint[DDP_HIP_MAX_COST_FRAMES] = {};
  double fc_off[DDP_HIP_MAX_COST_FRAMES][3] = {};
  double* fc_target_d = nullptr;
  double* fc_weight_d = nullptr;
  bool fc_live = false;
  double* fo_quat_d = nullptr;
  double* fo_weight_d = nullptr;
// ... 40 lines not shown
```

### ddp_pinocchio_amd/csrc/lin.hip

```cpp
#include <float.h>
#include <math.h>
#include <stdlib.h>

#include "frame_cost.h"
#include "internal.h"
#include "lin_common.h"
#include "rbd.h"
#include "rbd_deriv.h"
#include "state_limits.h"

namespace {



__global__ void lin_cost_kernel(LinParams p) {
  const int64_t T = p.d.T;
  const int64_t bt = blockIdx.x;
  const int b = (int)(bt / T);
  const int64_t t = bt % T;
  const int n = (int)p.d.n, m = (int)p.d.m;
  const double c = p.model->c;
  const int tid = threadIdx.x;
  if (t == 0) {
    for (int i = tid; i < n; i += blockDim.x) p.lfx[(int64_t)b * n + i] = 0.0;
// ... 793 lines not shown
  if (stage == 0) { i = (int)pid; j = -1; }
  else {
    i = (int)floor(((2.0 * W - 1.0) - sqrt((2.0 * W - 1.0) * (2.0 * W - 1.0) - 8.0 * (double)pid)) * 0.5);
    if (i < 0) i = 0;
    while ((int64_t)i * (2 * W - i - 1) / 2 > pid) --i;
    while ((int64_t)(i + 1) * (2 * W - i - 2) / 2 <= pid) ++i;
    j = (int)(pid - (int64_t)i * (2 * W - i - 1) / 2) + i + 1;
  }
  const DevModel& m = *p.model;
  constexpr int EM = NJ > 3 ? NJ : 3;
  double x[2 * NJ + 1], u[NJ], f1[EM];
  load_xu<NJ>(p, b, t, x, u);
  const double eps = sqrt(sqrt(DBL_EPSILON));
  const double eps2 = eps * eps;
  const int64_t Eo = p.Epre[t], Eb = (int64_t)b * p.d.Etot + Eo;
  const double* f0 = p.eq_val + Eb;
  double* exx = p.eq_xx + Eb * n * n;
  double* eux = p.eq_ux + Eb * mm * n;
  double* euu = p.eq_uu + Eb * mm * mm;
  const bool at_x_1 = i < n;
  const int idx_1 = at_x_1 ? i : i - n;
  const bool both_base = stage != 0 && m.ff && i < 6 && j < 6;
  if (both_base) {
    double nu[6] = {0, 0, 0, 0, 0, 0}, q7[7];
    nu[i] = eps; nu[j] = eps;
    lie::se3_integrate(x, nu, q7);
    for (int k = 0; k < 7; ++k) x[k] = q7[k];
  } else if (at_x_1) lie::perturb_x(m, x, idx_1, eps); else u[idx_1] = u[idx_1] + eps;
  const double* fcol_1 = at_x_1 ? p.eq_x + Eb * n + (int64_t)idx_1 * e : p.eq_u + Eb * mm + (int64_t)idx_1 * e;
  const int L1 = at_x_1 ? n : mm;
  double* tensor_1 = at_x_1 ? exx : euu;
  if (stage == 0) {
    eq_eval<NJ>(m, p.target + Eo, e, x, u, f1);
    for (int k = 0; k < e; ++k) {
      double df = f1[k] - f0[k];
      df -= eps * fcol_1[k];
      df *= 2;
      tensor_1[k + (int64_t)idx_1 * e + (int64_t)idx_1 * e * L1] = df / eps2;
    }
    return;
  }
  const bool at_x_2 = j < n;
  const int idx_2 = at_x_2 ? j : j - n;
  if (both_base) {} else if (at_x_2) lie::perturb_x(m, x, idx_2, eps); else u[idx_2] = u[idx_2] + eps;
  const double* fcol_2 = at_x_2 ? p.eq_x + Eb * n + (int64_t)idx_2 * e : p.eq_u + Eb * mm + (int64_t)idx_2 * e;
  const int L2 = at_x_2 ? n : mm;
  const double* tensor_2 = at_x_2 ? exx : euu;
  double* tensor;
  int L;
  if (at_x_1) { if (at_x_2) { tensor = exx; L = n; } else { tensor = eux; L = mm; } }
  else { tensor = euu; L = mm; }
  eq_eval<NJ>(m, p.target + Eo, e, x, u, f1);
  for (int k = 0; k < e; ++k) {
    double df = f1[k] - f0[k];
    df -= eps * fcol_1[k];
    df -= eps * fcol_2[k];
    df *= 2;
    const double val = 0.5 * (df / eps2 - tensor_1[k + (int64_t)idx_1 * e + (int64_t)idx_1 * e * L1] -
                              tensor_2[k + (int64_t)idx_2 * e + (int64_t)idx_2 * e * L2]);
    tensor[k + (int64_t)idx_2 * e + (int64_t)idx_1 * e * L] = val;
    if (at_x_1 == at_x_2) tensor[k + (int64_t)idx_1 * e + (int64_t)idx_2 * e * L] = val;
  }
}

__global__ void tensor_mirror_kernel(double* Tn, int64_t BT, int n, int L) {
  const int64_t per = (int64_t)n * L * L, total = BT * per;
  for (int64_t g = (int64_t)blockIdx.x * blockDim.x + threadIdx.x; g < total; g += (int64_t)gridDim.x * blockDim.x) {
    const int64_t bt = g / per, r = g % per;
    const int k = (int)(r % n), j = (int)((r / n) % L), c = (int)(r / ((int64_t)n * L));
    if (j >= c) continue;
    double* T = Tn + bt * per;
    T[k + (int64_t)j * n + (int64_t)c * n * L] = T[k + (int64_t)c * n + (int64_t)j * n * L];
  }
}

__global__ void tensor_zero_top_kernel(double* Tn, int64_t total_cols, int n, int nv) {
  const int64_t total = total_cols * nv;
  for (int64_t g = (int64_t)blockIdx.x * blockDim.x + threadIdx.x; g < total; g += (int64_t)gridDim.x * blockDim.x) {
    const int64_t col = g / nv;
    Tn[col * n + (g % nv)] = 0.0;
  }
}

LinParams make_params(ddp_hip_ctx* ctx) {
  LinParams p{};
  p.d = ctx->d;
  p.model = ctx->model_d;
  p.ne = ctx->ne_d;
  p.Epre = ctx->Epre_d;
  p.target = ctx->target_d;
  auto S = [&](int s) { return ctx->seq[s].ptr; };
  p.x = S(DDP_HIP_SEQ_X); p.u = S(DDP_HIP_SEQ_U);
  p.lfx = S(DDP_HIP_SEQ_LFX); p.lfxx = S(DDP_HIP_SEQ_LFXX);
  p.lx = S(DDP_HIP_SEQ_LX); p.lu = S(DDP_HIP_SEQ_LU); p.lxx = S(DDP_HIP_SEQ_LXX); p.lux = S(DDP_HIP_SEQ_LUX); p.luu = S(DDP_HIP_SEQ_LUU);
  p.f_val = S(DDP_HIP_SEQ_F_VAL); p.fx = S(DDP_HIP_SEQ_FX); p.fu = S(DDP_HIP_SEQ_FU);
  p.fxx = S(DDP_HIP_SEQ_FXX); p.fux = S(DDP_HIP_SEQ_FUX); p.fuu = S(DDP_HIP_SEQ_FUU);
  p.eq_val = S(DDP_HIP_SEQ_EQ_VAL); p.eq_x = S(DDP_HIP_SEQ_EQ_X); p.eq_u = S(DDP_HIP_SEQ_EQ_U);
  p.eq_xx = S(DDP_HIP_SEQ_EQ_XX); p.eq_ux = S(DDP_HIP_SEQ_EQ_UX); p.eq_uu = S(DDP_HIP_SEQ_EQ_UU);
  const LinPlan& pl = ctx->plan;
  p.has_tensors = pl.has_tensors ? 1 : 0;
  p.skip_top = pl.skip_top ? 1 : 0;
  p.skip_qv_mirror = pl.skip_qv_mirror ? 1 : 0;
  p.eq_xk = ctx->eq_ws;
  if (p.eq_xk) { p.eq_fxk = p.eq_xk + pl.eq_fxk_off; p.eq_c = p.eq_xk + pl.eq_c_off; }
  p.qcache = ctx->lin_ws;
  p.ncfg = pl.ncfg; p.nvcfg = pl.nvcfg;
  p.vcache = p.qcache ? p.qcache + ctx->d.batch * ctx->d.T * (int64_t)pl.ncfg * ctx->d.nv * rbd::QC_STRIDE : nullptr;
  p.xref = S(DDP_HIP_SEQ_COST_XREF); p.wx = S(DDP_HIP_SEQ_COST_WX); p.uref = S(DDP_HIP_SEQ_COST_UREF); p.wu = S(DDP_HIP_SEQ_COST_WU);
  return p;
}

inline unsigned blocks_for(int64_t total) { return (unsigned)((total + LBS - 1) / LBS); }

template <int NJ>
int eq_second_order(ddp_hip_ctx* ctx, const LinParams& p, LinCall& call, uint32_t stages) {
  const Dims& d = ctx->d;
  const int64_t BT = d.batch * d.T;
  const int W = (int)(d.n + d.m);
  const int64_t P = (int64_t)W * (W - 1) / 2;
  switch (ctx->plan.eq_second) {
    case LinEqSecond::None: break;
    case LinEqSecond::Mode2:
      hipLaunchKernelGGL((eq_second_m2_kernel<NJ>), dim3(blocks_for(BT * W)), dim3(LBS), 0, ctx->stream, p, 0);
      hipLaunchKernelGGL((eq_second_m2_kernel<NJ>), dim3(blocks_for(BT * P)), dim3(LBS), 0, ctx->stream, p, 1);
      break;
    case LinEqSecond::Mode1Small:
      if constexpr (NJ <= 6) hipLaunchKernelGGL((second_m1_kernel<NJ>), dim3(blocks_for(BT * W)), dim3(LBS), 0, ctx->stream, p, 1);
      break;
    case LinEqSecond::Mode1Wave: {
      const int fl = LIN_ANA_EQ | ((stages & DDP_HIP_LIN_SECOND) ? LIN_ANA_F : 0);
      if (fl & LIN_ANA_F) prof_begin(ctx, DDP_HIP_K_LIN_SECOND);
      const int rc_ = lin_analytic_launch(ctx, p, call, 1, fl);
      if (fl & LIN_ANA_F) prof_end(ctx, DDP_HIP_K_LIN_SECOND);
      if (rc_ != DDP_HIP_OK) return rc_;
      break;
    }
    case LinEqSecond::Zeros:
      HIP_TRY(hipMemsetAsync(p.eq_xx, 0, sizeof(double) * (size_t)(ctx->seq[DDP_HIP_SEQ_EQ_XX].size * d.batch), ctx->stream));
      HIP_TRY(hipMemsetAsync(p.eq_ux, 0, sizeof(double) * (size_t)(ctx->seq[DDP_HIP_SEQ_EQ_UX].size * d.batch), ctx->stream));
      HIP_TRY(hipMemsetAsync(p.eq_uu, 0, sizeof(double) * (size_t)(ctx->seq[DDP_HIP_SEQ_EQ_UU].size * d.batch), ctx->stream));
      break;
  }
  return DDP_HIP_OK;
}

template <int NJ>
int run_linearize(ddp_hip_ctx* ctx, const LinParams& p, LinCall& call, uint32_t stages) {
  const LinPlan& pl = ctx->plan;
  const Dims& d = ctx->d;
  const int64_t BT = d.batch * d.T;
  const int W = (int)(d.n + d.m);
  const int nv = (int)d.nv;
  [[maybe_unused]] constexpr bool small = NJ <= 6;
  const bool second_stage = (stages & DDP_HIP_LIN_SECOND) && pl.second != LinSecond::None;
  const bool eq_stage = (stages & DDP_HIP_LIN_EQ) && pl.eq != LinEq::None;
  const bool m1_fused = pl.m1_fused && eq_stage;
  if (stages & DDP_HIP_LIN_COST) {
    if (ctx->flags & DDP_HIP_FLAG_TRACKING_COST)
      hipLaunchKernelGGL(lin_track_cost_kernel, dim3((unsigned)(BT + d.batch)), dim3(64), 0, ctx->stream, p);
    else hipLaunchKernelGGL(lin_cost_kernel, dim3((unsigned)BT), dim3(64), 0, ctx->stream, p);
    const FrameCostDev fc = frame_cost_dev(ctx);
    if (fc.target) hipLaunchKernelGGL(lin_frame_cost_kernel, dim3((unsigned)(BT + d.batch)), dim3(64), 0, ctx->stream, p, fc);
    if (fc.oquat) hipLaunchKernelGGL(lin_frame_orient_cost_kernel, dim3((unsigned)(BT + d.batch)), dim3(64), 0, ctx->stream, p, fc);
    const StateLimitsDev sl = state_limits_dev(ctx);
    if (sl.weight) hipLaunchKernelGGL(lin_limit_cost_kernel, dim3((unsigned)(BT + d.batch)), dim3(64), 0, ctx->stream, p, sl);
  }
  bool caches_built = false;
  int static_rc = DDP_HIP_OK;
  auto build_caches = [&]() {
    if (caches_built) return;
    if (pl.topo) { const int rc_ = lin_static_launch(ctx, p, StaticLevel::Caches); if (rc_ != DDP_HIP_OK) static_rc = rc_; }
    else {
      hipLaunchKernelGGL((lin_qcache_kernel<NJ>), dim3(blocks_for(BT * (nv + 1))), dim3(LBS), 0, ctx->stream, p);
      hipLaunchKernelGGL((lin_vcache_kernel<NJ>), dim3(blocks_for(BT * (2 * nv + 1))), dim3(LBS), 0, ctx->stream, p);
    }
    caches_built = true;
  };
  if (stages & DDP_HIP_LIN_FIRST) {
    prof_begin(ctx, DDP_HIP_K_LIN_FIRST);
    hipLaunchKernelGGL((lin_base_kernel<NJ>), dim3(blocks_for(BT)), dim3(LBS), 0, ctx->stream, p);
    switch (pl.first) {
      case LinFirst::Base: break;
      case LinFirst::AnalyticSmall:
        if constexpr (small) hipLaunchKernelGGL((lin_first_analytic_small_kernel<NJ>), dim3(blocks_for(BT)), dim3(LBS), 0, ctx->stream, p);
        break;
// ... 4 lines not shown
        if (rc_ != DDP_HIP_OK) return rc_;
        break;
      }
      case LinFirst::FdStatic: {
        build_caches();
        const int rc_ = lin_static_launch(ctx, p, StaticLevel::FirstOrder);
        if (rc_ != DDP_HIP_OK) return rc_;
        break;
      }
      case LinFirst::FdGeneric:
        hipLaunchKernelGGL((lin_first_kernel<NJ>), dim3(blocks_for(BT * W)), dim3(LBS), 0, ctx->stream, p);
        break;
    }
    prof_end(ctx, DDP_HIP_K_LIN_FIRST);
  }
  if (second_stage) {
    const int64_t P = (int64_t)W * (W - 1) / 2, TRI = (int64_t)nv * (nv - 1) / 2, Pv = (int64_t)nv * nv + TRI, Pu = 2 * (int64_t)nv * nv + TRI;
    prof_begin(ctx, DDP_HIP_K_LIN_SECOND);
    switch (pl.second) {
      case LinSecond::None: break;
      case LinSecond::Mode2Static:
        build_caches();
        for (StaticLevel level : {StaticLevel::UDiagonal, StaticLevel::Torque, StaticLevel::Velocity, StaticLevel::Configuration}) {
          const int rc_ = lin_static_launch(ctx, p, level);
          if (rc_ != DDP_HIP_OK) return rc_;
        }
        break;
      case LinSecond::Mode2Caches:
        build_caches();
        hipLaunchKernelGGL((lin_diag_kernel<NJ>), dim3(blocks_for(BT * W)), dim3(LBS), 0, ctx->stream, p);
        hipLaunchKernelGGL((lin_offdiag_kernel<NJ, 3>), dim3(blocks_for(BT * Pu)), dim3(LBS), 0, ctx->stream, p);
        hipLaunchKernelGGL((lin_offdiag_kernel<NJ, 2>), dim3(blocks_for(BT * Pv)), dim3(LBS), 0, ctx->stream, p);
        hipLaunchKernelGGL((lin_offdiag_kernel<NJ, 1>), dim3(blocks_for(BT * TRI)), dim3(LBS), 0, ctx->stream, p);
        break;
      case LinSecond::Mode2Plain:
        hipLaunchKernelGGL((lin_diag_kernel<NJ>), dim3(blocks_for(BT * W)), dim3(LBS), 0, ctx->stream, p);
        hipLaunchKernelGGL((lin_offdiag_kernel<NJ, 0>), dim3(blocks_for(BT * P)), dim3(LBS), 0, ctx->stream, p);
        break;
      case LinSecond::Mode1Small:
        if constexpr (small) hipLaunchKernelGGL((second_m1_kernel<NJ>), dim3(blocks_for(BT * W)), dim3(LBS), 0, ctx->stream, p, 0);
        break;
      case LinSecond::Mode1Wave:
        if (!m1_fused) { const int rc_ = lin_analytic_launch(ctx, p, call, 1, LIN_ANA_F); if (rc_ != DDP_HIP_OK) return rc_; }
        break;
      case LinSecond::Zeros:
        HIP_TRY(hipMemsetAsync(p.fxx, 0, sizeof(double) * (size_t)(ctx->seq[DDP_HIP_SEQ_FXX].size * d.batch), ctx->stream));
        HIP_TRY(hipMemsetAsync(p.fux, 0, sizeof(double) * (size_t)(ctx->seq[DDP_HIP_SEQ_FUX].size * d.batch), ctx->stream));
        HIP_TRY(hipMemsetAsync(p.fuu, 0, sizeof(double) * (size_t)(ctx->seq[DDP_HIP_SEQ_FUU].size * d.batch), ctx->stream));
        break;
    }
    prof_end(ctx, DDP_HIP_K_LIN_SECOND);
  }
  if (eq_stage) {
    switch (pl.eq) {
      case LinEq::None: break;
      case LinEq::PerLane:
        if constexpr (small) hipLaunchKernelGGL((eq_first_kernel<NJ>), dim3(blocks_for(BT)), dim3(LBS), 0, ctx->stream, p);
        break;
      case LinEq::Analytic: {
        const int rc_ = lin_analytic_launch(ctx, p, call, 0, LIN_ANA_EQ);
        if (rc_ != DDP_HIP_OK) return rc_;
        break;
      }
      case LinEq::Chain: {
        const int K = ctx->model_h.eq_advance;
        if (K < 1) return DDP_HIP_E_UNSUPPORTED;
        hipLaunchKernelGGL((eq_chain_kernel<NJ>), dim3(blocks_for(BT)), dim3(LBS), 0, ctx->stream, p);
        if (pl.eq_jac == LinEqJac::Fd) hipLaunchKernelGGL((eq_fdjac_kernel<NJ>), dim3(blocks_for(BT * (K - 1) * d.n)), dim3(LBS), 0, ctx->stream, p);
        else if (pl.eq_jac == LinEqJac::FfLookahead) { const int rc_ = lin_analytic_ff_lookahead(ctx, p); if (rc_ != DDP_HIP_OK) return rc_; }
        hipLaunchKernelGGL(eq_combine_kernel, dim3((unsigned)BT), dim3(256), sizeof(double) * (size_t)(2 * d.emax * d.n), ctx->stream, p);
        break;
      }
    }
    const int rc_ = eq_second_order<NJ>(ctx, p, call, stages);
    if (rc_ != DDP_HIP_OK) return rc_;
  }
  HIP_TRY(hipGetLastError());
  return static_rc;
}

int tensors_begin_second(ddp_hip_ctx* ctx, const LinParams& p, LinCall& call) {
  const TensorOrigin was = ctx->tensors.origin;
  ctx->tensors.origin = TensorOrigin::Unknown;
  call.fuu_zero = was == TensorOrigin::Analytic1;
  if (p.skip_top && was != TensorOrigin::Stencil) {
    const int64_t BT = ctx->d.batch * ctx->d.T, n = ctx->d.n, m = ctx->d.m;
    const int nv = (int)ctx->d.nv;
    hipLaunchKernelGGL(tensor_zero_top_kernel, dim3(8192), dim3(256), 0, ctx->stream, p.fxx, BT * n * n, (int)n, nv);
    hipLaunchKernelGGL(tensor_zero_top_kernel, dim3(8192), dim3(256), 0, ctx->stream, p.fux, BT * m * n, (int)n, nv);
    hipLaunchKernelGGL(tensor_zero_top_kernel, dim3(8192), dim3(256), 0, ctx->stream, p.fuu, BT * m * m, (int)n, nv);
    HIP_TRY(hipGetLastError());
  }
  return DDP_HIP_OK;
}

void tensors_end_second(ddp_hip_ctx* ctx, const LinParams& p, const LinCall& call) {
  TensorState& t = ctx->tensors;
  if (ctx->model_h.fd_mode == 1) t.origin = call.fuu_zero ? TensorOrigin::Analytic1 : TensorOrigin::Unknown;
  else t.origin = p.skip_top ? TensorOrigin::Stencil : TensorOrigin::Symmetric;
  t.mirror_pending = p.skip_qv_mirror != 0;
}

}

int lin_setup(ddp_hip_ctx* ctx) {
  const Dims& d = ctx->d;
  const int topo_id = ctx->model_h.kind == DDP_HIP_MODEL_TREE ? lin_static_supported(ctx->model_h) : 0;
  ctx->plan = lin_plan_decide(ctx->model_h, d, ctx->flags, ctx->sw, topo_id, sweep_plan(ctx).sym_ok);
  const LinPlan& pl = ctx->plan;
  if (pl.refuse) return pl.refuse;
  if (pl.ws_lin)
    HIP_TRY(hipMalloc(&ctx->lin_ws, sizeof(double) * (size_t)(d.batch * d.T * ((int64_t)pl.ncfg * d.nv * rbd::QC_STRIDE + (int64_t)pl.nvcfg * d.nv * rbd::VC_STRIDE))));
  if (pl.ws_qws) {
    const int64_t BT = d.batch * d.T;
    int64_t slice = 1024;
    if (ctx->sw.qws_bt) slice = ctx->sw.qws_bt;
    ctx->lin_qws_bt = BT < slice ? BT : slice;
    HIP_TRY(hipMalloc(&ctx->lin_qws, sizeof(double) * (size_t)(ctx->lin_qws_bt * lin_static_ws_per_bt(ctx->model_h))));
    if (pl.ws_qws2) {
      HIP_TRY(hipMalloc(&ctx->lin_qws2, sizeof(double) * (size_t)(ctx->lin_qws_bt * lin_static_ws_per_bt(ctx->model_h))));
      HIP_TRY(hipStreamCreateWithFlags(&ctx->lin_stream2, hipStreamNonBlocking));
      for (int k = 0; k < 2; ++k) {
        HIP_TRY(hipEventCreateWithFlags(&ctx->lin_ev_up[k], hipEventDisableTiming));
        HIP_TRY(hipEventCreateWithFlags(&ctx->lin_ev_dn[k], hipEventDisableTiming));
      }
    }
  }
  { const int rc_ = lin_analytic_setup(ctx); if (rc_ != DDP_HIP_OK) return rc_; }
  if (pl.ws_eq) HIP_TRY(hipMalloc(&ctx->eq_ws, sizeof(double) * (size_t)pl.eq_words));
  return DDP_HIP_OK;
}
void lin_teardown(ddp_hip_ctx* ctx) {
  lin_analytic_teardown(ctx);
  for (int k = 0; k < 2; ++k) {
    if (ctx->lin_ev_up[k]) (void)hipEventDestroy(ctx->lin_ev_up[k]);
    if (ctx->lin_ev_dn[k]) (void)hipEventDestroy(ctx->lin_ev_dn[k]);
  }
  if (ctx->lin_stream2) (void)hipStreamDestroy(ctx->lin_stream2);
  if (ctx->lin_qws2) (void)hipFree(ctx->lin_qws2);
  if (ctx->lin_qws) (void)hipFree(ctx->lin_qws);
  if (ctx->eq_ws) (void)hipFree(ctx->eq_ws);
  if (ctx->lin_ws) (void)hipFree(ctx->lin_ws);
}

extern "C" int ddp_hip_linearize_stages(ddp_hip_ctx* ctx, uint32_t stages) {
  if (!ctx) return DDP_HIP_E_ARG;
  HIP_TRY(hipSetDevice(ctx->device));
  LinParams p = make_params(ctx);
  LinCall call;
  const bool second = (stages & DDP_HIP_LIN_SECOND) && p.has_tensors;
  if (second) { const int rc_ = tensors_begin_second(ctx, p, call); if (rc_ != DDP_HIP_OK) return rc_; }
  int rc;
  switch (ctx->plan.nj) {
    case 1: rc = run_linearize<1>(ctx, p, call, stages); break;
    case 6: rc = run_linearize<6>(ctx, p, call, stages); break;
    case 38: rc = run_linearize<38>(ctx, p, call, stages); break;
    default: rc = run_linearize<64>(ctx, p, call, stages); break;
  }
  if (rc != DDP_HIP_OK) return rc;
  END_SYNC(ctx);
  if (second) tensors_end_second(ctx, p, call);
  return DDP_HIP_OK;
}

int tensors_written_outside(ddp_hip_ctx* ctx, int seq) {
  if (seq != DDP_HIP_SEQ_FXX && seq != DDP_HIP_SEQ_FUX && seq != DDP_HIP_SEQ_FUU) return DDP_HIP_OK;
  TensorState& t = ctx->tensors;
  if (seq == DDP_HIP_SEQ_FUX) {
    t.origin = (t.origin == TensorOrigin::Symmetric || t.origin == TensorOrigin::Stencil) ? TensorOrigin::Symmetric : TensorOrigin::Unknown;
    return DDP_HIP_OK;
  }
  const int rc_ = lin_materialize_fxx(ctx);
  if (rc_ != DDP_HIP_OK) return rc_;
  t.origin = TensorOrigin::Unknown;
  return DDP_HIP_OK;
}

int lin_materialize_fxx(ddp_hip_ctx* ctx) {
  if (!ctx->tensors.mirror_pending) return DDP_HIP_OK;
  double* fxx = ctx->seq[DDP_HIP_SEQ_FXX].ptr;
  double* fuu = ctx->seq[DDP_HIP_SEQ_FUU].ptr;
  if (fxx && fuu) {
    const int64_t BT = ctx->d.batch * ctx->d.T;
    hipLaunchKernelGGL(tensor_mirror_kernel, dim3(8192), dim3(256), 0, ctx->stream, fxx, BT, (int)ctx->d.n, (int)ctx->d.n);
    hipLaunchKernelGGL(tensor_mirror_kernel, dim3(4096), dim3(256), 0, ctx->stream, fuu, BT, (int)ctx->d.n, (int)ctx->d.m);
    HIP_TRY(hipGetLastError());
    HIP_TRY(hipStreamSynchronize(ctx->stream));
  }
  ctx->tensors.mirror_pending = false;
  return DDP_HIP_OK;
}

extern "C" int ddp_hip_linearize(ddp_hip_ctx* ctx) {
  return ddp_hip_linearize_stages(ctx, DDP_HIP_LIN_COST | DDP_HIP_LIN_FIRST | DDP_HIP_LIN_SECOND | DDP_HIP_LIN_EQ);
}
```

### ddp_pinocchio_amd/csrc/lin_common.h

```cpp
#pragma once
#include "internal.h"

struct LinParams {
  Dims d;
  const DevModel* model;
  const int64_t* ne;
  const int64_t* Epre;
  const double* target;
  const double *x, *u;
  double *lfx, *lfxx, *lx, *lu, *lxx, *lux, *luu;
  double *f_val, *fx, *fu, *fxx, *fux, *fuu;
  double *eq_val, *eq_x, *eq_u, *eq_xx, *eq_ux, *eq_uu;
  int32_t has_tensors;
  double *eq_xk, *eq_fxk, *eq_c;
  double* vcache;
  double* qcache;
  int32_t skip_qv_mirror;
  int32_t skip_top;
  double* accel_out;
  int32_t ncfg, nvcfg;
  const double *xref, *wx, *uref, *wu;
};

constexpr int LBS = 64;

int lin_static_supported(const DevModel& m);
enum class StaticLevel {
  Caches,
  FirstOrder,
  UDiagonal,
  Torque,
  Velocity,
  Configuration,
  AccelX,
  AccelXU,
};
int lin_static_launch(ddp_hip_ctx* ctx, const LinParams& p, StaticLevel level);
int64_t lin_static_ws_per_bt(const DevModel& m);

int lin_analytic_setup(ddp_hip_ctx* ctx);
void lin_analytic_teardown(ddp_hip_ctx* ctx);
constexpr int LIN_ANA_F = 1, LIN_ANA_EQ = 2;
constexpr int LIN_ANA_ACCEL = 4;
int lin_analytic_launch(ddp_hip_ctx* ctx, const LinParams& p, LinCall& call, int stage, int flags);
int lin_analytic_ff_lookahead(ddp_hip_ctx* ctx, const LinParams& p);
```

### ddp_pinocchio_amd/csrc/lin_plan.cpp

```cpp
#include "internal.h"

LinPlan lin_plan_decide(const DevModel& m, const Dims& d, uint32_t flags, const DevSwitches& sw, int topo_id, bool sweep_sym_ok) {
  LinPlan pl;
  const bool tree = m.kind == DDP_HIP_MODEL_TREE, ff = m.ff != 0, fo_fd = m.first_order_fd != 0;
  const bool tensors = !(flags & DDP_HIP_FLAG_NO_TENSORS);
  const bool analytic = tree && !fo_fd;
  const int mode = m.fd_mode;
  const int64_t nv = d.nv, K = m.eq_advance;
  pl.has_tensors = tensors;
  pl.nj = nv <= 1 ? 1 : (nv <= 6 && !ff) ? 6 : nv <= 38 ? 38 : 64;
  const bool small = pl.nj <= 6;
  const bool wave = analytic && !small && !ff;

  if (mode == 1 && fo_fd && tensors) pl.refuse = DDP_HIP_E_UNSUPPORTED;
  if (analytic && ff && nv > 38) pl.refuse = DDP_HIP_E_UNSUPPORTED;
  if (wave && m.max_level_width > 64) pl.refuse = DDP_HIP_E_UNSUPPORTED;
  if (wave && d.Etot > 0 && (K < 1 || K > 2)) pl.refuse = DDP_HIP_E_UNSUPPORTED;

  const int topo = (tree && !ff && !sw.no_static) ? topo_id : 0;
  const bool stencil_caches = tree && mode == 2 && tensors && !ff && !sw.no_qcache;
  const bool accel = topo && wave && mode == 1 && tensors && !sw.ana_own_aba;
  if (stencil_caches) { pl.ncfg = (int32_t)nv + 1; pl.nvcfg = 2 * (int32_t)nv + 1; }
  else if ((topo && fo_fd) || accel) { pl.ncfg = 1; pl.nvcfg = 1; }
  pl.ws_lin = pl.ncfg > 0;
  pl.topo = pl.ws_lin ? topo : 0;
  pl.ws_qws = pl.topo != 0;

  if (analytic) pl.first = small ? LinFirst::AnalyticSmall : ff ? LinFirst::AnalyticFF : LinFirst::AnalyticWave;
  else if (fo_fd) pl.first = pl.topo ? LinFirst::FdStatic : LinFirst::FdGeneric;
  else pl.first = LinFirst::Base;

  if (!tensors) pl.second = LinSecond::None;
  else if (mode == 0) pl.second = LinSecond::Zeros;
  else if (mode == 1) pl.second = small ? LinSecond::Mode1Small : LinSecond::Mode1Wave;
  else if (pl.ncfg > 1) pl.second = pl.topo ? LinSecond::Mode2Static : LinSecond::Mode2Caches;
  else pl.second = LinSecond::Mode2Plain;
  pl.ws_qws2 = pl.second == LinSecond::Mode2Static && sw.cfg_full_aba;
  pl.skip_top = pl.topo && mode == 2 && tensors && !sw.fxx_full;
  pl.skip_qv_mirror = pl.skip_top && sweep_sym_ok;

  const bool m1_wave = wave && pl.second == LinSecond::Mode1Wave;
  pl.ana_sliced = analytic && !small;
  pl.ws_ana_T = wave && sw.ana_split;
  pl.ws_ana_M = wave && (sw.ana_split || (m1_wave && d.Etot > 0));
  pl.ws_ana_M0 = m1_wave && !sw.ana_split;
  pl.ws_ana_A = pl.accel_static = accel;
  pl.accel_with_u = accel && d.Etot > 0;
  pl.ws_ana_F = m1_wave && d.Etot > 0;

  pl.ws_eq = d.Etot > 0 && tree && (fo_fd || ff);
  if (d.Etot > 0) {
    pl.eq = (small && !pl.ws_eq) ? LinEq::PerLane : wave ? LinEq::Analytic : LinEq::Chain;
    if (pl.eq == LinEq::Chain && K > 1) pl.eq_jac = fo_fd ? LinEqJac::Fd : LinEqJac::FfLookahead;
    pl.eq_second = !tensors ? LinEqSecond::None : mode == 0 ? LinEqSecond::Zeros : mode == 2 ? LinEqSecond::Mode2
                   : small ? LinEqSecond::Mode1Small : LinEqSecond::Mode1Wave;
    pl.m1_fused = m1_wave;
    pl.eq_inline = m1_wave && !sw.ana_split && m.eq_kind == DDP_HIP_EQ_CONFIG && !sw.ana_eq_kernel;
  }
  if (pl.ws_eq) {
    pl.eq_fxk_off = d.batch * d.T * K * d.nx;
    pl.eq_c_off = pl.eq_fxk_off + d.batch * d.T * (K > 1 ? K - 1 : 0) * d.n * d.n;
    pl.eq_words = pl.eq_c_off + d.batch * d.T * d.emax * d.n;
  }
  pl.lin_path = tree ? 1 + pl.topo : 0;
  pl.first_order = tree ? (fo_fd ? 1 : 2) : 0;
  return pl;
}

#ifdef LIN_PLAN_TABLE
#include <stdio.h>

int main() {
  static const char* const sw_names[] = {"none", "generic_bwd", "k3_no_sym", "k3_no_half", "fxx_full", "no_static", "no_qcache",
                                         "cfg_full_aba", "ana_own_aba", "ana_split", "ana_eq_kernel", "bwd_no_graph", "solve_sync"};
  printf("kind nv ff fo_fd mode tensors etot eq_kind K matched sw sym_ok created refuse nj topo first second eq eq_jac eq_second "
         "eq_inline accel_static accel_with_u m1_fused ncfg nvcfg has_tensors skip_top skip_qv_mirror ws_lin ws_qws ws_qws2 ws_ana_T "
         "ws_ana_M ws_ana_M0 ws_ana_A ws_ana_F ws_eq ana_sliced eq_fxk_off eq_c_off eq_words lin_path first_order\n");
  printf("#");
  for (const char* s : sw_names) printf(" %s", s);
  printf("\n");
  const int nvs[] = {1, 6, 7, 38, 39, 64};
  for (int kind : {DDP_HIP_MODEL_PENDULUM, DDP_HIP_MODEL_TREE})
  for (int nv : nvs) for (int ff = 0; ff < 2; ++ff) for (int fo = 0; fo < 2; ++fo) for (int mode = 0; mode < 3; ++mode)
  for (int tensors = 0; tensors < 2; ++tensors) for (int etot = 0; etot < 2; ++etot)
  for (int eqk : {DDP_HIP_EQ_NONE, DDP_HIP_EQ_CONFIG, DDP_HIP_EQ_FRAME}) for (int K = 1; K <= 3; ++K)
  for (int matched = 0; matched < 2; ++matched) for (int s = 0; s < 13; ++s) {
    DevModel m{};
    m.kind = kind; m.nv = nv; m.ff = ff; m.nj = ff ? nv - 5 : nv; m.nq = nv + ff;
    m.first_order_fd = fo; m.fd_mode = mode; m.eq_kind = eqk; m.eq_advance = K; m.max_level_width = 4;
    Dims d{};
    d.T = 3; d.batch = 2; d.nv = nv; d.n = 2 * nv; d.m = nv; d.nx = 2 * nv + ff;
    d.emax = etot ? (eqk == DDP_HIP_EQ_CONFIG ? nv : 3) : 0; d.Etot = etot ? d.emax * d.T : 0;
    DevSwitches sw;
    bool* const sws[] = {nullptr, &sw.generic_bwd, &sw.k3_no_sym, &sw.k3_no_half, &sw.fxx_full, &sw.no_static, &sw.no_qcache,
                         &sw.cfg_full_aba, &sw.ana_own_aba, &sw.ana_split, &sw.ana_eq_kernel, &sw.bwd_no_graph, &sw.solve_sync};
    if (sws[s]) *sws[s] = true;
    const int sym_ok = nv == 38 && !sw.generic_bwd && !sw.k3_no_sym;
    const bool created = (kind == DDP_HIP_MODEL_TREE || (nv == 1 && !ff)) && (!ff || (nv >= 6 && mode != 1 && eqk != DDP_HIP_EQ_CONFIG)) &&
                         (eqk != DDP_HIP_EQ_NONE || !etot);
    const LinPlan p = lin_plan_decide(m, d, tensors ? 0u : (uint32_t)DDP_HIP_FLAG_NO_TENSORS, sw, matched && !ff ? 1 : 0, sym_ok != 0);
    printf("%d %d %d %d %d %d %d %d %d %d %d %d %d %d %d %d %d %d %d %d %d %d %d %d %d %d %d %d %d %d %d %d %d %d %d %d %d %d %d %d %lld %lld %lld %d %d\n",
           kind == DDP_HIP_MODEL_TREE, nv, ff, fo, mode, tensors, etot, eqk == DDP_HIP_EQ_NONE ? 0 : eqk == DDP_HIP_EQ_CONFIG ? 1 : 2, K, matched, s, sym_ok,
           (int)created, p.refuse != 0, p.nj, p.topo, (int)p.first, (int)p.second, (int)p.eq, (int)p.eq_jac, (int)p.eq_second,
           (int)p.eq_inline, (int)p.accel_static, (int)p.accel_with_u, (int)p.m1_fused, p.ncfg, p.nvcfg, (int)p.has_tensors, (int)p.skip_top,
           (int)p.skip_qv_mirror, (int)p.ws_lin, (int)p.ws_qws, (int)p.ws_qws2, (int)p.ws_ana_T, (int)p.ws_ana_M, (int)p.ws_ana_M0, (int)p.ws_ana_A,
           (int)p.ws_ana_F, (int)p.ws_eq, (int)p.ana_sliced, (long long)p.eq_fxk_off, (long long)p.eq_c_off, (long long)p.eq_words, p.lin_path, p.first_order);
  }
  return 0;
}
#endif
```

### ddp_pinocchio_amd/csrc/lin_static.hip

```cpp
#include <float.h>
#include <math.h>
#include <stdlib.h>

#include <type_traits>
#include <utility>

#include "internal.h"
#include "lin_common.h"
#include "rbd.h"

#ifndef DEV_NO_EMIT
#define DEV_NO_EMIT 0
#endif
namespace {

struct TopoTalos38 {
  static constexpr int N = 38;
  static constexpr int parent[N] = {-1, 0, 1, 2, 3, 4,
                                    5, 6, 7, 8, 9, 10,
                                    5, 12, 13, 14, 15, 16,
                                    5, 18,
                                    19, 20, 21, 22, 23, 24, 25, 26,
                                    19, 28, 29, 30, 31, 32, 33, 34,
                                    19, 36};
// ... 108 lines not shown
  if constexpr (QS == rbd::QC_STRIDE || (K % 2) == 0) __builtin_amdgcn_sched_barrier(0);
}

template <class T, int QS, class TauFn, int... Ks>
__device__ __forceinline__ void tau_up_all(const DevModel& m, const double* __restrict__ qc, const double* __restrict__ vc, TauFn tau,
                                           TauState<T>& s, std::integer_sequence<int, Ks...>) {
  (tau_up<T, T::N - 1 - Ks, QS>(m, qc, vc, tau(T::N - 1 - Ks), s), ...);
}
template <class T, int QS, int HI, class TauFn, int... Ks>
__device__ __forceinline__ void tau_up_range(const DevModel& m, const double* __restrict__ qc, const double* __restrict__ vc, TauFn tau,
                                             TauState<T>& s, std::integer_sequence<int, Ks...>) {
  (tau_up<T, HI - Ks, QS>(m, qc, vc, tau(HI - Ks), s), ...);
}
template <class T, int QS, int... Ks>
__device__ __forceinline__ void tau_down_all(const DevModel& m, const double* __restrict__ qc, const double* __restrict__ vc,
                                             TauState<T>& s, std::integer_sequence<int, Ks...>) {
  (tau_down<T, Ks, QS>(m, qc, vc, s), ...);
}

constexpr int PS = 20;
template <int NV>
__device__ __forceinline__ void stage_placements(double* sp, const double* __restrict__ qc, int lane) {
  for (int idx = lane; idx < NV * 19; idx += LBS) {
    const int K = idx / 19, e = idx - K * 19;
    sp[K * PS + e] = qc[K * rbd::QC_STRIDE + e];
  }
}

template <class T> constexpr bool parents_at_least(int from, int lo) {
  for (int k = from; k < T::N; ++k) if (T::parent[k] < lo) return false;
  return true;
}
template <class T> constexpr int stage_split() {
  for (int kh = T::N / 2; kh > 0; --kh) if (parents_at_least<T>(kh + 1, kh)) return kh;
  return 0;
}

template <int NV, int K0, int K1, bool WITH_V = true>
struct StageRegs {
  static constexpr int NPW = (K1 - K0) * 19, NVW = WITH_V ? (K1 - K0) * rbd::VC_STRIDE : 0;
  static constexpr int CP = (NPW + LBS - 1) / LBS, CV = (NVW + LBS - 1) / LBS;
  double rp[CP], rv[CV > 0 ? CV : 1];
  __device__ __forceinline__ void load(const double* __restrict__ qc, const double* __restrict__ vc, int lane) {
#pragma unroll
    for (int c = 0; c < CP; ++c) {
      int idx = c * LBS + lane;
      idx = idx < NPW ? idx : NPW - 1;
      const int K = K0 + idx / 19, e = idx % 19;
      rp[c] = qc[K * rbd::QC_STRIDE + e];
    }
#pragma unroll
    for (int c = 0; c < CV; ++c) {
      int idx = c * LBS + lane;
      idx = idx < NVW ? idx : NVW - 1;
      rv[c] = vc[K0 * rbd::VC_STRIDE + idx];
    }
  }
  __device__ __forceinline__ void park(double* sp, double* sv, int lane) const {
#pragma unroll
    for (int c = 0; c < CP; ++c) {
      int idx = c * LBS + lane;
      idx = idx < NPW ? idx : NPW - 1;
      const int K = K0 + idx / 19, e = idx % 19;
      sp[K * PS + e] = rp[c];
    }
#pragma unroll
    for (int c = 0; c < CV; ++c) {
      int idx = c * LBS + lane;
      idx = idx < NVW ? idx : NVW - 1;
      sv[K0 * rbd::VC_STRIDE + idx] = rv[c];
    }
  }
};

__device__ __forceinline__ void tri_index(int64_t q, int Wd, int& ii, int& jj) {
  int a = (int)floor(((2.0 * Wd - 1.0) - sqrt((2.0 * Wd - 1.0) * (2.0 * Wd - 1.0) - 8.0 * (double)q)) * 0.5);
  if (a < 0) a = 0;
  while ((int64_t)a * (2 * Wd - a - 1) / 2 > q) --a;
  while ((int64_t)(a + 1) * (2 * Wd - a - 2) / 2 <= q) ++a;
  ii = a;
  jj = (int)(q - (int64_t)a * (2 * Wd - a - 1) / 2) + a + 1;
}

template <int NV, int NP = LBS>
struct OutStage {
  double qdd[NP * (NV + 1)];
  int pij[NP];
};

template <int NV, int NP>
__device__ __forceinline__ void offdiag_emit(const LinParams& p, OutStage<NV, NP>& S, bool valid, int i, int j, int64_t bt,
                                             const double* __restrict__ xg, double dt, int pass = 0) {
  constexpr int n = 2 * NV, mm = NV;
  constexpr int RW = 16, NJ = (n + RW - 1) / RW, GRP = LBS / RW, PPG = NP / GRP, NB = NP == LBS ? 2 : 1;
  static_assert(PPG % NB == 0, "points per group");
  const double eps = sqrt(sqrt(DBL_EPSILON));
  const double eps2 = eps * eps;
  const int lane = threadIdx.x;
  if (lane / NP == pass) S.pij[lane % NP] = i | (j << 8) | ((valid ? 1 : 0) << 16);
  double* const fxx = p.fxx + bt * n * n * n;
  double* const fux = p.fux + bt * n * mm * n;
  double* const fuu = p.fuu + bt * n * mm * mm;
  const double* const fxb = p.fx + bt * n * n;
  const double* const fub = p.fu + bt * n * mm;
  __syncthreads();
  const int kk = lane % RW, grp = lane / RW;
  const double* f0 = p.f_val + bt * n;
  double f0k[NJ], xk[NJ], xvk[NJ];
#pragma unroll
  for (int jx = 0; jx < NJ; ++jx) {
    const int k = kk + RW * jx;
    const int kc = k < n ? k : n - 1;
    f0k[jx] = f0[kc];
    xk[jx] = xg[kc];
    xvk[jx] = kc < NV ? xg[NV + kc] : 0.0;
  }
  if (DEV_NO_EMIT) return;
  for (int pt = 0; pt < PPG; pt += NB) {
    double a1[NB][NJ], a2[NB][NJ], d1[NB][NJ], d2[NB][NJ];
    double* o0[NB];
    double* o1[NB];
    int ie[NB], je[NB], ee[NB];
#pragma unroll
    for (int u = 0; u < NB; ++u) {
      const int e = (pt + u) * GRP + grp;
      ee[u] = e;
      const int pk = S.pij[e];
      const int i1 = pk & 255, j1 = (pk >> 8) & 255;
      ie[u] = i1;
      je[u] = j1;
      const bool at_x_1 = i1 < n, at_x_2 = j1 < n;
      const int idx_1 = at_x_1 ? i1 : i1 - n, idx_2 = at_x_2 ? j1 : j1 - n;
      double* tensor;
      int L;
      if (at_x_1) { if (at_x_2) { tensor = fxx; L = n; } else { tensor = fux; L = mm; } }
      else { tensor = fuu; L = mm; }
      o0[u] = (pk >> 16) ? tensor + (int64_t)idx_2 * n + (int64_t)idx_1 * n * L : nullptr;
      o1[u] = ((pk >> 16) && at_x_1 == at_x_2 && !p.skip_qv_mirror) ? tensor + (int64_t)idx_1 * n + (int64_t)idx_2 * n * L : nullptr;
      if (o0[u]) {
        const double* q0 = at_x_1 ? fxb + (int64_t)idx_1 * n : fub + (int64_t)idx_1 * n;
        const double* q1 = at_x_2 ? fxb + (int64_t)idx_2 * n : fub + (int64_t)idx_2 * n;
        const double* q2 = at_x_1 ? fxx + (int64_t)idx_1 * n + (int64_t)idx_1 * n * n : fuu + (int64_t)idx_1 * n + (int64_t)idx_1 * n * mm;
        const double* q3 = at_x_2 ? fxx + (int64_t)idx_2 * n + (int64_t)idx_2 * n * n : fuu + (int64_t)idx_2 * n + (int64_t)idx_2 * n * mm;
#pragma unroll
        for (int jx = 0; jx < NJ; ++jx) {
          const int k = kk + RW * jx;
          const int kc = k < n ? k : n - 1;
          a1[u][jx] = q0[kc]; a2[u][jx] = q1[kc]; d1[u][jx] = q2[kc]; d2[u][jx] = q3[kc];
        }
      }
    }
#pragma unroll
    for (int u = 0; u < NB; ++u) {
      if (!o0[u]) continue;
#pragma unroll
      for (int jx = 0; jx < NJ; ++jx) {
        const int k = kk + RW * jx;
        if (k >= n) continue;
        if (p.skip_top && k < NV && !((ie[u] < n && ie[u] % NV == k) || (je[u] < n && je[u] % NV == k))) continue;
        double xs = k == ie[u] ? xk[jx] + eps : xk[jx];
        if (k == je[u]) xs = xs + eps;
        double fv;
        if (k < NV) {
          double xv = (NV + k) == ie[u] ? xvk[jx] + eps : xvk[jx];
          if (NV + k == je[u]) xv = xv + eps;
          const double vo = dt * xv;
          fv = xs + vo;
        } else {
          fv = xs + S.qdd[ee[u] * (NV + 1) + (k - NV)] * dt;
        }
        double df = fv - f0k[jx];
        df -= eps * a1[u][jx];
        df -= eps * a2[u][jx];
        df *= 2;
        const double val = 0.5 * (df / eps2 - d1[u][jx] - d2[u][jx]);
        o0[u][k] = val;
        if (o1[u]) o1[u][k] = val;
      }
    }
  }
}

template <int NV>
struct RowStage {
  double q[(NV + 2) * (NV + 1)];
};

template <int NV, bool DIAG_ROW, class ST>
__device__ __forceinline__ void rowblock_emit(const ST& S, int lane, int i, int jb, double* __restrict__ out, double* __restrict__ mirror,
                                              int64_t mstride, const double* __restrict__ a2, const double* __restrict__ d2, int64_t dstride,
                                              double dt, const double* __restrict__ f0g, const double* __restrict__ a1g,
                                              double* __restrict__ d1g, const double* __restrict__ xg, bool skip_top = false) {
  constexpr int n = 2 * NV, RW = 16, NJ = (n + RW - 1) / RW, CG = LBS / RW, NIT = (NV + CG - 1) / CG;
  const int r1 = i % NV;
  const double eps = sqrt(sqrt(DBL_EPSILON));
  const double eps2 = eps * eps;
  const int kk = lane % RW, cg = lane / RW;
  double xk[NJ], xvk[NJ], f0k[NJ], a1k[NJ], d1k[NJ];
#pragma unroll
  for (int j = 0; j < NJ; ++j) {
    const int k = kk + RW * j;
    const int kc = k < n ? k : n - 1;
    f0k[j] = f0g[kc];
    a1k[j] = a1g[kc];
    double x = xg[kc];
    if (kc == i) x = x + eps;
    xk[j] = x;
    double xv = xg[kc < NV ? NV + kc : kc];
    if (NV + kc == i) xv = xv + eps;
    xvk[j] = xv;
    if constexpr (DIAG_ROW) {
      double fv;
      if (kc < NV) {
        const double vo = dt * xv;
        fv = x + vo;
      } else {
        fv = x + S.q[NV * (NV + 1) + (kc - NV)] * dt;
      }
      double df = fv - f0k[j];
      df -= eps * a1k[j];
      df *= 2;
      const double dd = df / eps2;
      d1k[j] = dd;
      if (cg == 0 && k < n && !(skip_top && k < NV && k != r1)) d1g[k] = dd;
    } else {
      d1k[j] = d1g[kc];
    }
  }
  double va2[2][NJ], vd2[2][NJ];
  auto fetch = [&](int it, double (&A)[NJ], double (&D)[NJ]) {
    const int c = it * CG + cg;
    const int cc = c < NV ? c : NV - 1;
#pragma unroll
    for (int j = 0; j < NJ; ++j) {
      const int k = kk + RW * j;
      const int kc = k < n ? k : n - 1;
      A[j] = a2[kc + cc * n];
      D[j] = d2[kc + cc * dstride];
    }
  };
  auto form = [&](int it, const double (&A)[NJ], const double (&D)[NJ]) {
    const int c = it * CG + cg;
    const bool cv = c < NV;
    const int cc = cv ? c : NV - 1;
    const int jp = jb + cc;
#pragma unroll
    for (int j = 0; j < NJ; ++j) {
      const int k = kk + RW * j;
      if (!(cv && k < n)) continue;
      if (skip_top && k < NV && k != r1 && !(jp < n && jp % NV == k)) continue;
      double x = xk[j];
      if (k == jp) x = x + eps;
      double fv;
      if (k < NV) {
        double xv = xvk[j];
        if (NV + k == jp) xv = xv + eps;
        const double vo = dt * xv;
        fv = x + vo;
      } else {
        fv = x + S.q[cc * (NV + 1) + (k - NV)] * dt;
      }
      double df = fv - f0k[j];
      df -= eps * a1k[j];
      df -= eps * A[j];
      df *= 2;
      const double val = 0.5 * (df / eps2 - d1k[j] - D[j]);
      out[k + c * n] = val;
      if (mirror) mirror[k + c * mstride] = val;
    }
  };
  if (DEV_NO_EMIT) return;
  fetch(0, va2[0], vd2[0]);
  for (int it = 0; it < NIT; it += 2) {
    if (it + 1 < NIT) fetch(it + 1, va2[1], vd2[1]);
    form(it, va2[0], vd2[0]);
    if (it + 1 < NIT) {
      if (it + 2 < NIT) fetch(it + 2, va2[0], vd2[0]);
      form(it + 1, va2[1], vd2[1]);
    }
  }
}

template <class T, bool ROWS>
__global__ __launch_bounds__(LBS, ROWS ? 1 : 3) void lin_static_tau_kernel(LinParams p) {
  constexpr int nv = T::N, n = 2 * nv;
  constexpr int TRI = nv * (nv - 1) / 2, GU = (TRI + LBS - 1) / LBS, G = ROWS ? 2 * nv : GU;
  const int64_t bt = blockIdx.x / G;
  const int g = (int)(blockIdx.x % G) + (ROWS ? 0 : 2 * nv);
  const int lane = threadIdx.x;
  const int64_t Tn = p.d.T;
  const int b = (int)(bt / Tn);
  const int64_t t = bt % Tn;
  const DevModel& m = *p.model;
  int i, j, cfg, vcfg;
  bool valid;
  if (g < nv) { i = g; j = n + lane; cfg = 1 + g; vcfg = nv + 1 + g; valid = lane < nv; }
  else if (g < 2 * nv) { i = g; j = n + lane; cfg = 0; vcfg = 1 + (g - nv); valid = lane < nv; }
  else {
    const int pid = (g - 2 * nv) * LBS + lane;
    valid = pid < TRI;
    tri_index(valid ? pid : 0, nv, i, j);
    i += n; j += n; cfg = 0; vcfg = 0;
  }
  const double eps = sqrt(sqrt(DBL_EPSILON));
  const double* __restrict__ qc = p.qcache + (bt * (nv + 1) + cfg) * (int64_t)nv * rbd::QC_STRIDE;
  const double* __restrict__ vc = p.vcache + (bt * (2 * nv + 1) + vcfg) * (int64_t)nv * rbd::VC_STRIDE;
  const double* __restrict__ xg = p.x + ((int64_t)b * (Tn + 1) + t) * n;
  const double* __restrict__ ug = p.u + ((int64_t)b * Tn + t) * nv;
  const int iu = i - n, ju = j - n;
  __shared__ union TauLds { double P[nv * PS + nv * rbd::VC_STRIDE]; RowStage<nv> S; OutStage<nv, LBS / 2> O; } s_lds;
  double* s_P = s_lds.P;
  double* s_V = s_P + nv * PS;
  constexpr int KH = stage_split<T>();
  StageRegs<nv, 0, (KH > 0) ? KH : 1> lower;
  {
    StageRegs<nv, KH, nv> upper;
    upper.load(qc, vc, lane);
    lower.load(qc, vc, lane);
    upper.park(s_P, s_V, lane);
    rbd::coop_sync<true>();
  }
  TauState<T> s;
  auto tau = [&](int k) { double v = ug[k]; if (k == iu) v = v + eps; if (k == ju) v = v + eps; return v; };
  static_assert(parents_at_least<T>(KH + 1, KH), "the first half of the pass must not reach below record KH");
  tau_up_range<T, PS, nv - 1>(m, s_P, s_V, tau, s, std::make_integer_sequence<int, nv - 1 - KH>{});
  lower.park(s_P, s_V, lane);
  rbd::coop_sync<true>();
  tau_up_range<T, PS, KH>(m, s_P, s_V, tau, s, std::make_integer_sequence<int, KH + 1>{});
  tau_down_all<T, PS>(m, s_P, s_V, s, std::make_integer_sequence<int, nv>{});
  __builtin_amdgcn_sched_barrier(0);
  typedef __attribute__((address_space(4))) const LinParams* kernarg_t;
  const kernarg_t kp = (kernarg_t)__builtin_amdgcn_kernarg_segment_ptr();
  if constexpr (ROWS) {
    RowStage<nv>& S = s_lds.S;
    const int mm = nv;
    __syncthreads();
    const int row = lane <= nv ? lane : nv + 1;
#pragma unroll
    for (int k = 0; k < nv; ++k) S.q[row * (nv + 1) + k] = s.uu[k];
    __syncthreads();
    rowblock_emit<nv, true>(S, lane, i, n, kp->fux + bt * n * mm * n + (int64_t)i * n * mm, nullptr, 0, kp->fu + bt * n * mm,
                            kp->fuu + bt * n * mm * mm, (int64_t)n + (int64_t)n * mm, m.dt, kp->f_val + bt * n,
                            kp->fx + bt * n * n + (int64_t)i * n, kp->fxx + bt * n * n * n + (int64_t)i * n + (int64_t)i * n * n, xg, kp->skip_top != 0);
  } else {
    OutStage<nv, LBS / 2>& S = s_lds.O;
    LinParams po;
    po.f_val = kp->f_val; po.fx = kp->fx; po.fu = kp->fu; po.fxx = kp->fxx; po.fux = kp->fux; po.fuu = kp->fuu; po.skip_qv_mirror = kp->skip_qv_mirror; po.skip_top = kp->skip_top;
    const double dt = m.dt;
    __syncthreads();
#pragma unroll 1
    for (int pass = 0; pass < 2; ++pass) {
      if (pass) __syncthreads();
      if (lane / (LBS / 2) == pass) {
#pragma unroll
        for (int k = 0; k < nv; ++k) S.qdd[(lane % (LBS / 2)) * (nv + 1) + k] = s.uu[k];
      }
      offdiag_emit<nv, LBS / 2>(po, S, valid, i, j, bt, xg, dt, pass);
    }
  }
}

template <class T> constexpr int n_children(int k) {
  int c = 0;
  for (int j = k + 1; j < T::N; ++j) if (T::parent[j] == k) ++c;
  return c;
}
template <class T> constexpr bool chain_start(int k) { return T::parent[k] < 0 || T::parent[k] != k - 1 || n_children<T>(T::parent[k]) > 1; }
template <class T> constexpr bool chain_end(int k) { return k == T::N - 1 || chain_start<T>(k + 1); }
template <class T> constexpr int chain_first(int k) { while (!chain_start<T>(k)) --k; return k; }
template <class T> constexpr int max_chain() {
  int best = 1;
  for (int k = 0; k < T::N; ++k)
    if (chain_end<T>(k)) { const int len = k - chain_first<T>(k) + 1; if (len > best) best = len; }
  return best;
}

template <class T>
struct VelState {
  double vel[T::N][6];
  double acc[T::N][6];
  double uu[T::N];
};

template <int UQS_, int QS_ = rbd::QC_STRIDE>
struct VelCtx {
  static constexpr int UQS = UQS_;
  static constexpr int QS = QS_;
  const DevModel* m;
  const double* qp;
  const double* __restrict__ qc;
  const double* __restrict__ xg;
  const double* __restrict__ ug;
  double* uq;
  int i, j;
  double eps;
  template <int K> __device__ __forceinline__ const double* er(double*) const { return qp + K * QS; }
  template <int K> __device__ __forceinline__ const double* er_down(double* b) const { return er<K>(b); }
  template <int K> __device__ __forceinline__ const double* ud() const { return qp + K * QS + 12; }
  template <int K> __device__ __forceinline__ void ia_cb(const double*, const double* cb, double* Iac) const { rbd::sym6_mv(qc + K * rbd::QC_STRIDE + 19, cb, Iac); }
  template <int K> __device__ __forceinline__ const double* ud_down() const { return ud<K>(); }
};

template <int NV, class C>
__device__ __forceinline__ double lane_v(const C& c, int K) {
  double v = c.xg[NV + K];
  if (NV + K == c.i) v = v + c.eps;
  if (NV + K == c.j) v = v + c.eps;
  return v;
}

template <class T, int K, class C>
__device__ __forceinline__ void joint_vel(const C& c, const double* vel_par, double* vel) {
  constexpr int o = T::prismatic[K] ? 3 : 0;
  double Pb[12];
  const double* E = c.template er<K>(Pb);
  const double* r = E + 9;
  const double* a = c.m->axis[K];
  const double vK = lane_v<T::N>(c, K);
  double vJ[6] = {0, 0, 0, 0, 0, 0};
  vJ[o] = a[0] * vK; vJ[o + 1] = a[1] * vK; vJ[o + 2] = a[2] * vK;
  if constexpr (T::parent[K] >= 0) rbd::xform_motion(E, r, vel_par, vel);
  else {
#pragma unroll
    for (int k = 0; k < 6; ++k) vel[k] = 0.0;
  }
#pragma unroll
  for (int k = 0; k < 6; ++k) vel[k] += vJ[k];
}
template <class T, int K, class C>
__device__ __forceinline__ void vel_from_root(const C& c, double* vel) {
  if constexpr (T::parent[K] >= 0) {
    double vp[6];
    vel_from_root<T, T::parent[K]>(c, vp);
    joint_vel<T, K>(c, vp, vel);
  } else {
    joint_vel<T, K>(c, nullptr, vel);
  }
}
template <class T, int K, class C>
__device__ __forceinline__ void bias_force0(const C& c, const double* vel, double* pA) {
// ... 93 lines not shown
    for (int k = 0; k < 6; ++k) vel[k] = 0.0;
    rbd::xform_motion(E, r, a0, ap);
  }
#pragma unroll
  for (int k = 0; k < 6; ++k) vel[k] += vJ[k];
  rbd::crm(vel, vJ, cb);
  double sum = 0;
#pragma unroll
  for (int k = 0; k < 6; ++k) { ap[k] += cb[k]; sum += U[k] * ap[k]; }
  double ui;
  if constexpr (C::UQS == 0) ui = s.uu[K]; else ui = c.uq[K * C::UQS];
  const double qd = (ui - sum) * dinv;
  if constexpr (C::UQS == 0) s.uu[K] = qd; else c.uq[K * C::UQS] = qd;
  if constexpr (has_child<T>(K)) {
#pragma unroll
    for (int k = 0; k < 6; ++k) { s.vel[K][k] = vel[k]; s.acc[K][k] = ap[k]; }
    s.acc[K][o] += a[0] * qd; s.acc[K][o + 1] += a[1] * qd; s.acc[K][o + 2] += a[2] * qd;
  }
  __builtin_amdgcn_sched_barrier(0);
}
template <class T, class C, int... Ks>
__device__ __forceinline__ void vel_down_all(const C& c, VelState<T>& s, std::integer_sequence<int, Ks...>) {
  (vel_down<T, Ks>(c, s), ...);
}

template <class T, bool ROWS>
__global__ __launch_bounds__(LBS, ROWS ? 3 : 2) void lin_static_vel_kernel(LinParams p) {
  constexpr int nv = T::N, n = 2 * nv;
  constexpr int TRI = nv * (nv - 1) / 2, GU = (TRI + LBS - 1) / LBS, G = ROWS ? nv : GU;
  const int64_t bt = blockIdx.x / G;
  const int g = (int)(blockIdx.x % G);
  const int lane = threadIdx.x;
  const int64_t Tn = p.d.T;
  const int b = (int)(bt / Tn);
  const int64_t t = bt % Tn;
  int i, j, cfg;
  bool valid;
  if (ROWS) { i = g; j = nv + lane; cfg = 1 + g; valid = lane < nv; }
  else {
    const int pid = g * LBS + lane;
    valid = pid < TRI;
    tri_index(valid ? pid : 0, nv, i, j);
    i += nv; j += nv; cfg = 0;
  }
  struct PairStage { OutStage<nv, LBS / 2> O; double spare[nv + 1]; };
  using Stage = typename std::conditional<ROWS, RowStage<nv>, PairStage>::type;
  __shared__ union VelLds { Stage S; double P[nv * rbd::QC_STRIDE]; } s_lds;
  Stage& S = s_lds.S;
  double* s_P = s_lds.P;
  VelCtx<0, rbd::QC_STRIDE> c;
  c.m = p.model;
  c.qc = p.qcache + (bt * (nv + 1) + cfg) * (int64_t)nv * rbd::QC_STRIDE;
  c.qp = s_P;
  c.xg = p.x + ((int64_t)b * (Tn + 1) + t) * n;
  c.ug = p.u + ((int64_t)b * Tn + t) * nv;
  c.i = i; c.j = j;
  c.eps = sqrt(sqrt(DBL_EPSILON));
  c.uq = nullptr;
  {
    constexpr int NW = nv * rbd::QC_STRIDE, CW = (NW + LBS - 1) / LBS;
    double rq[CW];
#pragma unroll
    for (int r = 0; r < CW; ++r) { const int idx = r * LBS + lane; rq[r] = c.qc[idx < NW ? idx : NW - 1]; }
#pragma unroll
    for (int r = 0; r < CW; ++r) { const int idx = r * LBS + lane; s_P[idx < NW ? idx : NW - 1] = rq[r]; }
    c.qc = s_P;
    rbd::coop_sync<true>();
  }
  VelState<T> s;
  vel_up_all<T>(c, s, std::make_integer_sequence<int, nv>{});
  vel_down_all<T>(c, s, std::make_integer_sequence<int, nv>{});
  __builtin_amdgcn_sched_barrier(0);
  typedef __attribute__((address_space(4))) const LinParams* kernarg_t;
  const kernarg_t kp = (kernarg_t)__builtin_amdgcn_kernarg_segment_ptr();
  const double dt = c.m->dt;
  if constexpr (ROWS) {
    double* fxx = kp->fxx + bt * n * n * n;
    const double* fxb = kp->fx + bt * n * n;
    __syncthreads();
    const int row = valid ? lane : nv;
#pragma unroll
    for (int k = 0; k < nv; ++k) S.q[row * (nv + 1) + k] = s.uu[k];
    __syncthreads();
    rowblock_emit<nv, false>(S, lane, i, nv, fxx + (int64_t)nv * n + (int64_t)i * n * n,
                             kp->skip_qv_mirror ? nullptr : fxx + (int64_t)i * n + (int64_t)nv * n * n, (int64_t)n * n,
                             fxb + (int64_t)nv * n, fxx + (int64_t)nv * n + (int64_t)nv * n * n, (int64_t)n + (int64_t)n * n, dt,
                             kp->f_val + bt * n, fxb + (int64_t)i * n, fxx + (int64_t)i * n + (int64_t)i * n * n, c.xg, kp->skip_top != 0);
  } else {
    constexpr int NP = LBS / 2;
    LinParams po;
    po.f_val = kp->f_val; po.fx = kp->fx; po.fu = kp->fu; po.fxx = kp->fxx; po.fux = kp->fux; po.fuu = kp->fuu; po.skip_qv_mirror = kp->skip_qv_mirror; po.skip_top = kp->skip_top;
    __syncthreads();
    double* const own = &S.O.qdd[(lane % NP) * (nv + 1)];
    double* const row = lane < NP ? own : S.spare;
#pragma unroll
    for (int k = 0; k < nv; ++k) row[k] = s.uu[k];
#pragma unroll 1
    for (int pass = 0; pass < 2; ++pass) {
      if (pass) {
        __syncthreads();
        if (lane >= NP) {
#pragma unroll
          for (int k = 0; k < nv; ++k) own[k] = s.uu[k];
        }
      }
      offdiag_emit<nv, NP>(po, S.O, valid, i, j, bt, c.xg, dt, pass);
    }
  }
}

constexpr int WS_PER_JOINT = 8;

template <class T>
struct CfgState {
  double vel[T::N][6];
  double accP[T::N][6];
  double accI[T::N][21];
  double w[2][WS_PER_JOINT];
};

struct CfgCtx {
  const DevModel* __restrict__ m;
  const double* __restrict__ qc0;
  const double* __restrict__ xg;
  const double* __restrict__ ug;
  double* __restrict__ W;
  double* lvel;
  int i, j;
  const double* own;
};

template <int K, int NV>
__device__ __forceinline__ void lane_placement(const CfgCtx& c, double* P) {
  const double* base = c.qc0 + K * rbd::QC_STRIDE;
  const double* pert = c.own ? c.own : c.qc0 + ((int64_t)(1 + K) * NV + K) * rbd::QC_STRIDE;
  const bool own = K == c.i || K == c.j;
#pragma unroll
  for (int e = 0; e < 12; ++e) P[e] = own ? pert[e] : base[e];
}

template <class T, int K>
__device__ __forceinline__ void cfg_joint_vel(const CfgCtx& c, const double* P, const double* vel_par, double* vel) {
  constexpr int o = T::prismatic[K] ? 3 : 0;
  const double* a = c.m->axis[K];
  const double vK = c.xg[T::N + K];
  double vJ[6] = {0, 0, 0, 0, 0, 0};
  vJ[o] = a[0] * vK; vJ[o + 1] = a[1] * vK; vJ[o + 2] = a[2] * vK;
  if constexpr (T::parent[K] >= 0) rbd::xform_motion(P, P + 9, vel_par, vel);
  else {
#pragma unroll
    for (int k = 0; k < 6; ++k) vel[k] = 0.0;
  }
#pragma unroll
  for (int k = 0; k < 6; ++k) vel[k] += vJ[k];
}
template <class T, int K>
__device__ __forceinline__ void cfg_vel_from_root(const CfgCtx& c, double* vel) {
  double P[12];
  lane_placement<K, T::N>(c, P);
  if constexpr (T::parent[K] >= 0) {
    double vp[6];
    cfg_vel_from_root<T, T::parent[K]>(c, vp);
    cfg_joint_vel<T, K>(c, P, vp, vel);
  } else {
    cfg_joint_vel<T, K>(c, P, nullptr, vel);
  }
}
template <int K>
__device__ __forceinline__ void cfg_bias_force0(const CfgCtx& c, const double* vel, double* pA) {
  double Iv[6];
  rbd::sym6_mv(c.m->I6[K], vel, Iv);
  rbd::crf(vel, Iv, pA);
}

// ... 123 lines not shown
#pragma unroll
    for (int k = 0; k < 6; ++k) vel[k] = 0.0;
    rbd::xform_motion(P, P + 9, a0, ap);
  }
#pragma unroll
  for (int k = 0; k < 6; ++k) vel[k] += vJ[k];
  rbd::crm(vel, vJ, cb);
  double sum = 0;
#pragma unroll
  for (int k = 0; k < 6; ++k) { ap[k] += cb[k]; sum += U[k] * ap[k]; }
  const double qd = (ui - sum) * dinv;
  out.uq[K * (O::STRIDE == LBS ? LBS : 1)] = qd;
  if constexpr (has_child<T>(K)) {
#pragma unroll
    for (int k = 0; k < 6; ++k) { s.vel[K][k] = vel[k]; s.accP[K][k] = ap[k]; }
    s.accP[K][o] += a[0] * qd; s.accP[K][o + 1] += a[1] * qd; s.accP[K][o + 2] += a[2] * qd;
  }
  __builtin_amdgcn_sched_barrier(0);
}
template <class T, class O, int... Ks>
__device__ __forceinline__ void cfg_down_all(const CfgCtx& c, CfgState<T>& s, const O& out, std::integer_sequence<int, Ks...>) {
  (cfg_down<T, Ks>(c, s, out), ...);
}

template <class T>
__device__ __forceinline__ void cfg_setup(CfgCtx& c, const LinParams& p, const DevModel* __restrict__ model, const double* __restrict__ qcache,
                                          const double* __restrict__ xs, const double* __restrict__ us, double* __restrict__ ws,
                                          int64_t bt0, int64_t& bt, bool& valid) {
  constexpr int nv = T::N, n = 2 * nv;
  constexpr int TRI = nv * (nv - 1) / 2, GU = (TRI + LBS - 1) / LBS;
  bt = bt0 + blockIdx.x / GU;
  const int g = (int)(blockIdx.x % GU);
  const int lane = threadIdx.x;
  const int64_t Tn = p.d.T;
  const int b = (int)(bt / Tn);
  const int64_t t = bt % Tn;
  const int pid = g * LBS + lane;
  valid = pid < TRI;
  tri_index(valid ? pid : 0, nv, c.i, c.j);
  c.m = model;
  c.qc0 = qcache + (bt * (nv + 1)) * (int64_t)nv * rbd::QC_STRIDE;
  c.xg = xs + ((int64_t)b * (Tn + 1) + t) * n;
  c.ug = us + ((int64_t)b * Tn + t) * nv;
  c.W = ws + (int64_t)blockIdx.x * (nv * WS_PER_JOINT * LBS) + lane;
  c.own = nullptr;
}

template <class T>
__global__ __launch_bounds__(LBS) void lin_static_cfg_up_kernel(LinParams p, const DevModel* __restrict__ model, const double* __restrict__ qcache,
                                                                const double* __restrict__ xs, const double* __restrict__ us,
                                                                double* __restrict__ ws, int64_t bt0) {
  constexpr int nv = T::N;
  constexpr int MAXCH = max_chain<T>();
  __shared__ double s_vel[MAXCH * 6 * LBS];
  CfgCtx c;
  int64_t bt;
  bool valid;
  cfg_setup<T>(c, p, model, qcache, xs, us, ws, bt0, bt, valid);
  c.lvel = s_vel + threadIdx.x;
  CfgState<T> s;
  cfg_up_all<T>(c, s, std::make_integer_sequence<int, nv>{});
}

template <class T>
__global__ __launch_bounds__(LBS) void lin_static_cfg_down_kernel(LinParams p, const DevModel* __restrict__ model, const double* __restrict__ qcache,
                                                                  const double* __restrict__ xs, const double* __restrict__ us,
                                                                  double* __restrict__ ws, int64_t bt0) {
  constexpr int nv = T::N;
  __shared__ OutStage<nv> S;
  CfgCtx c;
  int64_t bt;
  bool valid;
  cfg_setup<T>(c, p, model, qcache, xs, us, ws, bt0, bt, valid);
  c.lvel = nullptr;
  CfgState<T> s;
#pragma unroll
  for (int e = 0; e < WS_PER_JOINT; ++e) s.w[0][e] = c.W[e * LBS];
  CfgDownOut<nv + 1> o{&S.qdd[threadIdx.x * (nv + 1)]};
  cfg_down_all<T>(c, s, o, std::make_integer_sequence<int, nv>{});
  __builtin_amdgcn_sched_barrier(0);
  typedef __attribute__((address_space(4))) const LinParams* kernarg_t;
  const kernarg_t kp = (kernarg_t)__builtin_amdgcn_kernarg_segment_ptr();
  LinParams po;
  po.f_val = kp->f_val; po.fx = kp->fx; po.fu = kp->fu; po.fxx = kp->fxx; po.fux = kp->fux; po.fuu = kp->fuu; po.skip_qv_mirror = kp->skip_qv_mirror; po.skip_top = kp->skip_top;
  offdiag_emit<nv, LBS>(po, S, valid, c.i, c.j, bt, c.xg, model->dt);
}

constexpr int SREC = 13;

template <class T>
struct SpineTab {
  static constexpr int N = T::N, TRI = N * (N - 1) / 2;
  static_assert(N >= 2 && N <= 64, "ancestor masks are 64 bits wide");
  unsigned long long mask[N];
  unsigned long long anc[N];
  int depth[N];
  int nrec;
  short pi[TRI], pj[TRI];
  short top[TRI];
  int rbase[TRI], rstride[TRI];
};
template <class T>
constexpr SpineTab<T> make_spine_tab() {
  SpineTab<T> t{};
  for (int k = 0; k < T::N; ++k)
    for (int a = T::parent[k]; a >= 0; a = T::parent[a]) { ++t.depth[k]; t.mask[a] |= 1ull << k; t.anc[k] |= 1ull << a; }
  int cnt[T::N + 2] = {}, start[T::N + 2] = {}, goff[T::N + 2] = {};
  for (int i = 0; i < T::N; ++i)
    for (int j = i + 1; j < T::N; ++j) {
      int a = T::parent[i];
      while (a >= 0 && !((t.mask[a] >> j) & 1)) a = T::parent[a];
      ++cnt[a + 1];
    }
  for (int g = 0; g <= T::N; ++g) {
    start[g + 1] = start[g] + cnt[g];
    goff[g + 1] = goff[g] + cnt[g] * (g == 0 ? 0 : t.depth[g - 1] + 1);
  }
  t.nrec = goff[T::N + 1];
  int fill[T::N + 2] = {};
  for (int i = 0; i < T::N; ++i)
    for (int j = i + 1; j < T::N; ++j) {
      int a = T::parent[i];
      while (a >= 0 && !((t.mask[a] >> j) & 1)) a = T::parent[a];
      const int g = a + 1, rank = fill[g]++, slot = start[g] + rank;
      t.pi[slot] = (short)i; t.pj[slot] = (short)j; t.top[slot] = (short)a;
      t.rbase[slot] = goff[g] + rank;
      t.rstride[slot] = cnt[g];
    }
  return t;
}
template <class T> __device__ const SpineTab<T> g_spine_tab = make_spine_tab<T>();
template <class T> constexpr unsigned long long desc_mask(int k) { return make_spine_tab<T>().mask[k]; }
template <class T> constexpr int depth_of(int k) { return make_spine_tab<T>().depth[k]; }
template <class T> constexpr int spine_records() { return make_spine_tab<T>().nrec; }
template <class T> constexpr bool spine_joint(int k) { const unsigned long long mk = desc_mask<T>(k); return (mk & (mk - 1)) != 0; }

template <int GU>
__device__ __forceinline__ bool xcd_slot(int nb, int& btl, int& g) {
  const int x = (int)blockIdx.x, s = x >> 3;
  btl = (s / GU) * 8 + (x & 7);
  g = s % GU;
  return btl < nb;
}

template <class T>
__global__ __launch_bounds__(LBS) void lin_static_spine_kernel(const DevModel* __restrict__ model, const double* __restrict__ qcache,
                                                               const double* __restrict__ vcache, double* __restrict__ spine, int64_t bt0, int nb) {
  constexpr int nv = T::N, TRI = nv * (nv - 1) / 2, GU = (TRI + LBS - 1) / LBS, NREC = spine_records<T>();
  int btl, g;
  if (!xcd_slot<GU>(nb, btl, g)) return;
  const int slot = g * LBS + (int)threadIdx.x;
  if (slot >= TRI) return;
  const SpineTab<T>& tab = g_spine_tab<T>;
  const DevModel& m = *model;
  const int i = tab.pi[slot], j = tab.pj[slot];
  const int rstride = tab.rstride[slot];
  const double* __restrict__ qc0 = qcache + ((bt0 + btl) * (nv + 1)) * (int64_t)nv * rbd::QC_STRIDE;
  const double* __restrict__ vc0 = vcache + ((bt0 + btl) * (2 * nv + 1)) * (int64_t)nv * rbd::VC_STRIDE;
  double* __restrict__ out = spine + ((int64_t)btl * NREC + tab.rbase[slot]) * SREC;
  double Ia[21];
#pragma unroll
  for (int k = 0; k < 21; ++k) Ia[k] = 0.0;
  int prev = -1;
  for (int K = tab.top[slot]; K >= 0; K = m.parent[K]) {
    double IA[21];
#pragma unroll
    for (int k = 0; k < 21; ++k) IA[k] = m.I6[K][k];
// ... 61 lines not shown
    constexpr int DK = depth_of<T>(K);
    if constexpr (desc_mask<T>(K) == 0) return qc0 + (K * rbd::QC_STRIDE + 12);
    else {
      const int si = (int)((ai >> K) & 1), sj = (int)((aj >> K) & 1);
      const int cfg = (si & (sj ^ 1)) * (1 + i) + (sj & (si ^ 1)) * (1 + j);
      const double* p = qc0 + ((cfg * T::N + K) * rbd::QC_STRIDE + 12);
      if constexpr (!spine_joint<T>(K)) return p;
      else {
        const double* q = spb + (rbase + DK * rstride) * SREC;
        return (si & sj) ? q : p;
      }
    }
  }
  template <int K> __device__ __forceinline__ const double* er_down(double*) const {
    const int64_t own = (K - i) * (K - j) == 0 ? (int64_t)(1 + K) * T::N * rbd::QC_STRIDE : 0;
    return qc0 + K * rbd::QC_STRIDE + own;
  }
  template <int K> __device__ __forceinline__ const double* ud_down() const {
    constexpr int DK = depth_of<T>(K);
    if constexpr (desc_mask<T>(K) == 0) return qc0 + (K * rbd::QC_STRIDE + 12);
    else {
      const bool si = (ai >> K) & 1, sj = (aj >> K) & 1;
      const int cfg = sj ? 1 + j : (si ? 1 + i : 0);
      const double* p = qc0 + (int64_t)cfg * (T::N * rbd::QC_STRIDE) + (K * rbd::QC_STRIDE + 12);
      if constexpr (!spine_joint<T>(K)) return p;
      else {
        const double* q = spb + ((int64_t)rbase + (int64_t)DK * rstride) * SREC;
        return ((ai & aj) >> K) & 1 ? q : p;
      }
    }
  }
  template <int K> __device__ __forceinline__ void ia_cb(const double* ud, const double* cb, double* Iac) const {
    if constexpr (!spine_joint<T>(K)) rbd::sym6_mv(ud + 7, cb, Iac);
    else {
      const int on = (int)(((ai & aj) >> K) & 1);
      const double* pIa = on ? qc0 + (K * rbd::QC_STRIDE + 19) : ud + 7;
      const double w1 = (double)on, w0 = (double)(on ^ 1);
      double t[6];
#pragma unroll
      for (int k = 0; k < 6; ++k) t[k] = ud[7 + k];
      rbd::sym6_mv(pIa, cb, Iac);
#pragma unroll
      for (int k = 0; k < 6; ++k) Iac[k] = w1 * t[k] + w0 * Iac[k];
    }
  }
};
template <int NV, class T>
__device__ __forceinline__ double lane_v(const SpliceCtx<T>& c, int K) { return c.xg[NV + K]; }

template <class T>
__global__ __launch_bounds__(LBS, 2) void lin_static_cfg_pair_kernel(LinParams p, const double* __restrict__ spine, int64_t bt0, int nb) {
  constexpr int nv = T::N, n = 2 * nv;
  constexpr int TRI = nv * (nv - 1) / 2, GU = (TRI + LBS - 1) / LBS, NREC = spine_records<T>();
  int btl, g;
  if (!xcd_slot<GU>(nb, btl, g)) return;
  const int64_t bt = bt0 + btl;
  const int lane = threadIdx.x;
  const int64_t Tn = p.d.T;
  const int b = (int)(bt / Tn);
  const int64_t t = bt % Tn;
  const int slot = g * LBS + lane;
  const bool valid = slot < TRI;
  const int sc = valid ? slot : 0;
  const SpineTab<T>& tab = g_spine_tab<T>;
  __shared__ OutStage<nv> S;
  SpliceCtx<T> c;
  c.i = tab.pi[sc]; c.j = tab.pj[sc];
  c.ai = tab.anc[c.i];
  c.aj = tab.anc[c.j];
  c.rbase = tab.rbase[sc]; c.rstride = tab.rstride[sc];
  c.m = p.model;
  c.qc0 = p.qcache + (bt * (nv + 1)) * (int64_t)nv * rbd::QC_STRIDE;
  c.xg = p.x + ((int64_t)b * (Tn + 1) + t) * n;
  c.ug = p.u + ((int64_t)b * Tn + t) * nv;
  c.spb = spine + (int64_t)btl * NREC * SREC;
  c.uq = &S.qdd[lane * (nv + 1)];
  VelState<T> s;
  vel_up_all<T>(c, s, std::make_integer_sequence<int, nv>{});
  vel_down_all<T>(c, s, std::make_integer_sequence<int, nv>{});
  __builtin_amdgcn_sched_barrier(0);
  typedef __attribute__((address_space(4))) const LinParams* kernarg_t;
  const kernarg_t kp = (kernarg_t)__builtin_amdgcn_kernarg_segment_ptr();
  LinParams po;
  po.f_val = kp->f_val; po.fx = kp->fx; po.fu = kp->fu; po.fxx = kp->fxx; po.fux = kp->fux; po.fuu = kp->fuu; po.skip_qv_mirror = kp->skip_qv_mirror; po.skip_top = kp->skip_top;
  offdiag_emit<nv, LBS>(po, S, valid, c.i, c.j, bt, c.xg, c.m->dt);
}

template <int NV, bool DIAG>
__device__ __forceinline__ void first_output(const double* q , int lane, int d0, double* __restrict__ out,
                                             int64_t ostride, const double* __restrict__ fcol, const double* __restrict__ f0,
                                             const double* __restrict__ xg, double dt, double eps, bool skip_top = false) {
  constexpr int n = 2 * NV, TOT = NV * n;
  const double eps2 = eps * eps;
  for (int e = lane; e < TOT; e += LBS) {
    const int c = e / n, k = e - c * n;
    const int d = d0 + c;
    if (DIAG && skip_top && k < NV && !(d < n && d % NV == k)) continue;
    double xk = xg[k];
    if (k == d) xk = xk + eps;
    double fv;
    if (k < NV) {
      double xv = xg[NV + k];
      if (NV + k == d) xv = xv + eps;
      const double vo = dt * xv;
      fv = xk + vo;
    } else {
      fv = xk + q[c * (NV + 1) + (k - NV)] * dt;
    }
    if constexpr (DIAG) {
      double df = fv - f0[k];
      df -= eps * fcol[e];
      df *= 2;
      out[k + c * ostride] = df / eps2;
    } else {
      out[e] = (fv - f0[k]) / eps;
    }
  }
}

template <class T, int LEVEL, bool DIAG>
__global__ __launch_bounds__(LBS) void lin_static_first_kernel(LinParams p, const DevModel* __restrict__ model, const double* __restrict__ qcache,
                                                               const double* __restrict__ xs, const double* __restrict__ us,
                                                               double* __restrict__ ws, int64_t bt0) {
  constexpr int nv = T::N, n = 2 * nv;
  const int64_t bt = bt0 + blockIdx.x;
  const int lane = threadIdx.x;
  const int64_t Tn = p.d.T;
  const int b = (int)(bt / Tn);
  const int64_t t = bt % Tn;
  const bool valid = lane < nv;
  const double eps = DIAG ? sqrt(sqrt(DBL_EPSILON)) : sqrt(DBL_EPSILON);
  const double* __restrict__ qc0 = qcache + (bt * p.ncfg) * (int64_t)nv * rbd::QC_STRIDE;
  const double* __restrict__ xg = xs + ((int64_t)b * (Tn + 1) + t) * n;
  const double* __restrict__ ug = us + ((int64_t)b * Tn + t) * nv;
  __shared__ double s_q[(nv + 1) * (nv + 1)];
  double* uq = s_q + (valid ? lane : nv) * (nv + 1);
  if constexpr (LEVEL == 3) {
    const double* __restrict__ vc = p.vcache + (bt * p.nvcfg) * (int64_t)nv * rbd::VC_STRIDE;
    TauState<T> s;
    auto tau = [&](int k) { double v = ug[k]; if (k == lane) v = v + eps; return v; };
    tau_up_all<T, rbd::QC_STRIDE>(*model, qc0, vc, tau, s, std::make_integer_sequence<int, nv>{});
    tau_down_all<T, rbd::QC_STRIDE>(*model, qc0, vc, s, std::make_integer_sequence<int, nv>{});
#pragma unroll
    for (int k = 0; k < nv; ++k) uq[k] = s.uu[k];
  } else if constexpr (LEVEL == 2) {
    VelCtx<1> c;
    c.m = model; c.qc = qc0; c.qp = qc0; c.xg = xg; c.ug = ug; c.uq = uq;
    c.i = nv + lane; c.j = -1; c.eps = eps;
    VelState<T> s;
    vel_up_all<T>(c, s, std::make_integer_sequence<int, nv>{});
    vel_down_all<T>(c, s, std::make_integer_sequence<int, nv>{});
  } else {
    constexpr int MAXCH = max_chain<T>();
    __shared__ double s_vel[MAXCH * 6 * LBS];
    __shared__ double s_own[12 * LBS];
    if constexpr (!DIAG) {
      double E[9], r[3];
      const int jn = valid ? lane : 0;
      rbd::joint_placement(*model, jn, xg[jn] + eps, E, r);
#pragma unroll
      for (int e = 0; e < 9; ++e) s_own[lane * 12 + e] = E[e];
#pragma unroll
      for (int e = 0; e < 3; ++e) s_own[lane * 12 + 9 + e] = r[e];
    }
    CfgCtx c;
    c.m = model; c.qc0 = qc0; c.xg = xg; c.ug = ug;
    c.W = ws + (int64_t)blockIdx.x * (nv * WS_PER_JOINT * LBS) + lane;
    c.lvel = s_vel + lane;
    c.i = valid ? lane : 0; c.j = -1;
    c.own = DIAG ? nullptr : s_own + lane * 12;
    CfgState<T> s;
    cfg_up_all<T>(c, s, std::make_integer_sequence<int, nv>{});
#pragma unroll
    for (int e = 0; e < WS_PER_JOINT; ++e) s.w[0][e] = c.W[e * LBS];
    CfgDownOut<nv + 1> o{uq};
    cfg_down_all<T>(c, s, o, std::make_integer_sequence<int, nv>{});
  }
  __builtin_amdgcn_sched_barrier(0);
  typedef __attribute__((address_space(4))) const LinParams* kernarg_t;
  const kernarg_t kp = (kernarg_t)__builtin_amdgcn_kernarg_segment_ptr();
  __syncthreads();
  if constexpr (!DIAG) {
    if (double* ao = kp->accel_out) {
      ao += bt * (3 * nv + 1) * nv;
      double* al = ao + (LEVEL - 1) * nv * nv;
      for (int e = lane; e < nv * nv; e += LBS) { const int c = e / nv; al[e] = s_q[c * (nv + 1) + (e - c * nv)]; }
      if (LEVEL == 2 && lane < nv) ao[3 * nv * nv + lane] = s_q[nv * (nv + 1) + lane];
      return;
    }
  }
  double* fcol = LEVEL == 3 ? kp->fu + bt * n * nv : kp->fx + bt * n * n + (LEVEL == 2 ? nv * n : 0);
  double* out = fcol;
  int64_t ostride = n;
  if constexpr (DIAG) {
    if (LEVEL == 3) { out = kp->fuu + bt * n * nv * nv; ostride = n + (int64_t)n * nv; }
    else { ostride = n + (int64_t)n * n; out = kp->fxx + bt * n * n * n + (LEVEL == 2 ? nv * ostride : 0); }
  }
  first_output<nv, DIAG>(s_q, lane, LEVEL == 1 ? 0 : (LEVEL == 2 ? nv : n), out, ostride, fcol, kp->f_val + bt * n, xg, model->dt, eps, kp->skip_top != 0);
}

template <class T, int K>
__device__ __forceinline__ void placement_static(const DevModel& m, double q, double* P) {
  const double* Rp = m.Rp[K];
  const double* a = m.axis[K];
  double* E = P;
  double* r = P + 9;
  if constexpr (!T::prismatic[K]) {
    double sn, cs;
    sincos(q, &sn, &cs);
    const double Kx[9] = {0, -a[2], a[1], a[2], 0, -a[0], -a[1], a[0], 0};
    double K2[9], RJ[9], Rc[9];
    rbd::mm3(Kx, Kx, K2);
    const double omc = 1.0 - cs;
#pragma unroll
    for (int k = 0; k < 9; ++k) RJ[k] = sn * Kx[k] + omc * K2[k];
    RJ[0] += 1.0; RJ[4] += 1.0; RJ[8] += 1.0;
    rbd::mm3(Rp, RJ, Rc);
#pragma unroll
    for (int k = 0; k < 3; ++k)
#pragma unroll
      for (int l = 0; l < 3; ++l) E[3 * k + l] = Rc[3 * l + k];
    r[0] = m.pp[K][0]; r[1] = m.pp[K][1]; r[2] = m.pp[K][2];
  } else {
    const double dd[3] = {a[0] * q, a[1] * q, a[2] * q};
    double Rd[3];
    rbd::mv3(Rp, dd, Rd);
#pragma unroll
    for (int k = 0; k < 3; ++k)
#pragma unroll
      for (int l = 0; l < 3; ++l) E[3 * k + l] = Rp[3 * l + k];
    r[0] = m.pp[K][0] + Rd[0]; r[1] = m.pp[K][1] + Rd[1]; r[2] = m.pp[K][2] + Rd[2];
  }
}

struct QvCtx {
  const DevModel* __restrict__ m;
  const double* __restrict__ xg;
  double* __restrict__ qc;
  double* __restrict__ vc;
  double* lvel;
  int jn;
  double eps;
};
template <class T>
struct QvState {
  double vel[T::N][6];
  double accI[T::N][21];
};
template <class T, int K>
__device__ __forceinline__ void qv_placement(const QvCtx& c, double* P) {
  double q = c.xg[K];
  if (K == c.jn) q = q + c.eps;
  placement_static<T, K>(*c.m, q, P);
}
template <class T, int K>
__device__ __forceinline__ void qv_joint_vel(const QvCtx& c, const double* P, const double* vel_par, double* vel) {
  constexpr int o = T::prismatic[K] ? 3 : 0;
  const double* a = c.m->axis[K];
  const double vK = c.xg[T::N + K];
  double vJ[6] = {0, 0, 0, 0, 0, 0};
  vJ[o] = a[0] * vK; vJ[o + 1] = a[1] * vK; vJ[o + 2] = a[2] * vK;
  if constexpr (T::parent[K] >= 0) rbd::xform_motion(P, P + 9, vel_par, vel);
  else {
#pragma unroll
    for (int k = 0; k < 6; ++k) vel[k] = 0.0;
  }
#pragma unroll
  for (int k = 0; k < 6; ++k) vel[k] += vJ[k];
}
template <class T, int K>
__device__ __forceinline__ void qv_vel_from_root(const QvCtx& c, double* vel) {
  double P[12];
  qv_placement<T, K>(c, P);
  if constexpr (T::parent[K] >= 0) {
    double vp[6];
    qv_vel_from_root<T, T::parent[K]>(c, vp);
    qv_joint_vel<T, K>(c, P, vp, vel);
  } else {
    qv_joint_vel<T, K>(c, P, nullptr, vel);
  }
}
// ... 121 lines not shown
  if constexpr (T::parent[K] >= 0) rbd::xform_motion(E, r, vel[T::parent[K]], v);
  else {
#pragma unroll
    for (int k = 0; k < 6; ++k) v[k] = 0.0;
  }
#pragma unroll
  for (int k = 0; k < 6; ++k) { v[k] += vJ[k]; vel[K][k] = v[k]; }
  rbd::crm(v, vJ, cb);
  rbd::sym6_mv(m.I6[K], v, Iv);
  rbd::crf(v, Iv, pA);
  rbd::sym6_mv(Ia, cb, Iac);
  double* vo = vc + K * rbd::VC_STRIDE;
#pragma unroll
  for (int k = 0; k < 6; ++k) { vo[k] = cb[k]; vo[6 + k] = pA[k]; vo[12 + k] = Iac[k]; }
  __builtin_amdgcn_sched_barrier(0);
}
template <class T, int... Ks>
__device__ __forceinline__ void vc_all(const DevModel& m, const double* __restrict__ qc, const double* __restrict__ xg, int iv, double eps,
                                       double (&vel)[T::N][6], double* __restrict__ vc, std::integer_sequence<int, Ks...>) {
  (vc_joint<T, Ks>(m, qc, xg, iv, eps, vel, vc), ...);
}
template <class T>
__global__ __launch_bounds__(LBS) void lin_static_vcache_kernel(LinParams p, const DevModel* __restrict__ model, const double* __restrict__ xs,
                                                                const double* __restrict__ qcache, double* __restrict__ vcache) {
  constexpr int nv = T::N, n = 2 * nv;
  const int64_t bt = blockIdx.x;
  const int lane = threadIdx.x;
  const int64_t Tn = p.d.T;
  const int b = (int)(bt / Tn);
  const int64_t t = bt % Tn;
  if (lane >= nv) return;
  const double* __restrict__ qc = qcache + (bt * (nv + 1)) * (int64_t)nv * rbd::QC_STRIDE;
  const double* __restrict__ xg = xs + ((int64_t)b * (Tn + 1) + t) * n;
  double* __restrict__ vc = vcache + (bt * (2 * nv + 1) + 1 + lane) * (int64_t)nv * rbd::VC_STRIDE;
  double vel[nv][6];
  vc_all<T>(*model, qc, xg, lane, sqrt(sqrt(DBL_EPSILON)), vel, vc, std::make_integer_sequence<int, nv>{});
}

}

int lin_static_supported(const DevModel& m) {
  if (m.ff) return 0;
  if (topo_matches<TopoTalos38>(m)) return 1;
  if (topo_matches<TopoChain6>(m)) return 2;
#define DDP_TOPO_MATCH(ID, TOPO) if (topo_matches<TOPO>(m)) return (ID) - 1;
  DDP_TOPO_EXTRA(DDP_TOPO_MATCH)
#undef DDP_TOPO_MATCH
  return 0;
}

int64_t lin_static_ws_per_bt(const DevModel& m) {
  const int64_t nv = m.nv, TRI = nv * (nv - 1) / 2, GU = (TRI + LBS - 1) / LBS;
  int64_t rec = 0;
  for (int i = 0; i < nv; ++i)
    for (int j = i + 1; j < nv; ++j) {
      const auto anc = [&](int a, int x) { for (int k = m.parent[x]; k >= 0; k = m.parent[k]) if (k == a) return true; return false; };
      int a = m.parent[i];
      while (a >= 0 && !anc(a, j)) a = m.parent[a];
      for (; a >= 0; a = m.parent[a]) ++rec;
    }
  const int64_t sweep = GU * nv * WS_PER_JOINT * LBS, splice = rec * SREC;
  return sweep > splice ? sweep : splice;
}

template <class T>
static void launch_first_columns(ddp_hip_ctx* ctx, const LinParams& p, bool with_u) {
  const int64_t BT = ctx->d.batch * ctx->d.T;
  constexpr int nv = T::N, TRI = nv * (nv - 1) / 2, GU = (TRI + LBS - 1) / LBS;
  const int64_t per = ctx->lin_qws_bt * GU;
  for (int64_t bt0 = 0; bt0 < BT; bt0 += per) {
    const int64_t nb = BT - bt0 < per ? BT - bt0 : per;
    hipLaunchKernelGGL((lin_static_first_kernel<T, 1, false>), dim3((unsigned)nb), dim3(LBS), 0, ctx->stream, p, p.model, p.qcache, p.x, p.u, ctx->lin_qws, bt0);
  }
  hipLaunchKernelGGL((lin_static_first_kernel<T, 2, false>), dim3((unsigned)BT), dim3(LBS), 0, ctx->stream, p, p.model, p.qcache, p.x, p.u, ctx->lin_qws, (int64_t)0);
  if (with_u) hipLaunchKernelGGL((lin_static_first_kernel<T, 3, false>), dim3((unsigned)BT), dim3(LBS), 0, ctx->stream, p, p.model, p.qcache, p.x, p.u, ctx->lin_qws, (int64_t)0);
}

template <class T>
static int lin_static_launch_t(ddp_hip_ctx* ctx, const LinParams& p, StaticLevel level) {
  const int64_t BT = ctx->d.batch * ctx->d.T;
  constexpr int nv = T::N, TRI = nv * (nv - 1) / 2, GU = (TRI + LBS - 1) / LBS;
  if (level == StaticLevel::Torque) {
    hipLaunchKernelGGL((lin_static_tau_kernel<T, true>), dim3((unsigned)(BT * 2 * nv)), dim3(LBS), 0, ctx->stream, p);
    hipLaunchKernelGGL((lin_static_tau_kernel<T, false>), dim3((unsigned)(BT * GU)), dim3(LBS), 0, ctx->stream, p);
  } else if (level == StaticLevel::Caches) {
    hipLaunchKernelGGL((lin_static_qvcache_kernel<T>), dim3((unsigned)((BT * p.ncfg + LBS - 1) / LBS)), dim3(LBS), 0, ctx->stream, p, p.model, p.x, p.qcache, p.vcache);
    if (p.nvcfg > 1) hipLaunchKernelGGL((lin_static_vcache_kernel<T>), dim3((unsigned)BT), dim3(LBS), 0, ctx->stream, p, p.model, p.x, p.qcache, p.vcache);
  } else if (level == StaticLevel::AccelXU || level == StaticLevel::AccelX) {
    if (!p.accel_out) return DDP_HIP_E_ARG;
    hipLaunchKernelGGL((lin_static_qvcache_kernel<T>), dim3((unsigned)((BT * p.ncfg + LBS - 1) / LBS)), dim3(LBS), 0, ctx->stream, p, p.model, p.x, p.qcache, p.vcache);
    launch_first_columns<T>(ctx, p, level == StaticLevel::AccelXU);
  } else if (level == StaticLevel::FirstOrder) {
    launch_first_columns<T>(ctx, p, true);
  } else if (level == StaticLevel::UDiagonal) {
    hipLaunchKernelGGL((lin_static_first_kernel<T, 3, true>), dim3((unsigned)BT), dim3(LBS), 0, ctx->stream, p, p.model, p.qcache, p.x, p.u, ctx->lin_qws, (int64_t)0);
  } else if (level == StaticLevel::Configuration && !ctx->sw.cfg_full_aba) {
    constexpr int64_t NREC = spine_records<T>(), SWEEP = (int64_t)GU * nv * WS_PER_JOINT * LBS;
    constexpr int64_t WS_BT = SWEEP > NREC * SREC ? SWEEP : NREC * SREC;
    const int64_t per = NREC > 0 ? ctx->lin_qws_bt * WS_BT / (NREC * SREC) : BT;
    for (int64_t bt0 = 0; bt0 < BT; bt0 += per) {
      const int nb = (int)(BT - bt0 < per ? BT - bt0 : per);
      const dim3 grid((unsigned)((nb + 7) / 8 * 8 * GU));
      hipLaunchKernelGGL((lin_static_spine_kernel<T>), grid, dim3(LBS), 0, ctx->stream, p.model, p.qcache, p.vcache, ctx->lin_qws, bt0, nb);
      hipLaunchKernelGGL((lin_static_cfg_pair_kernel<T>), grid, dim3(LBS), 0, ctx->stream, p, ctx->lin_qws, bt0, nb);
    }
  } else if (level == StaticLevel::Configuration) {
    const int64_t per = ctx->lin_qws_bt;
    hipStream_t s0 = ctx->stream, s1 = ctx->lin_stream2;
    int k = 0;
    for (int64_t bt0 = 0; bt0 < BT; bt0 += per, ++k) {
      const int64_t nb = BT - bt0 < per ? BT - bt0 : per;
      const int w = k & 1;
      double* ws = w ? ctx->lin_qws2 : ctx->lin_qws;
      if (k >= 2) HIP_TRY(hipStreamWaitEvent(s0, ctx->lin_ev_dn[w], 0));
      hipLaunchKernelGGL((lin_static_cfg_up_kernel<T>), dim3((unsigned)(nb * GU)), dim3(LBS), 0, s0, p, p.model, p.qcache, p.x, p.u, ws, bt0);
      HIP_TRY(hipEventRecord(ctx->lin_ev_up[w], s0));
      HIP_TRY(hipStreamWaitEvent(s1, ctx->lin_ev_up[w], 0));
      hipLaunchKernelGGL((lin_static_cfg_down_kernel<T>), dim3((unsigned)(nb * GU)), dim3(LBS), 0, s1, p, p.model, p.qcache, p.x, p.u, ws, bt0);
      HIP_TRY(hipEventRecord(ctx->lin_ev_dn[w], s1));
    }
    if (k >= 1) HIP_TRY(hipStreamWaitEvent(s0, ctx->lin_ev_dn[0], 0));
    if (k >= 2) HIP_TRY(hipStreamWaitEvent(s0, ctx->lin_ev_dn[1], 0));
  } else if (level == StaticLevel::Velocity) {
    hipLaunchKernelGGL((lin_static_vel_kernel<T, true>), dim3((unsigned)(BT * nv)), dim3(LBS), 0, ctx->stream, p);
    hipLaunchKernelGGL((lin_static_vel_kernel<T, false>), dim3((unsigned)(BT * GU)), dim3(LBS), 0, ctx->stream, p);
  }
  HIP_TRY(hipGetLastError());
  return DDP_HIP_OK;
}

int lin_static_launch(ddp_hip_ctx* ctx, const LinParams& p, StaticLevel level) {
  if (ctx->plan.topo == 1) return lin_static_launch_t<TopoTalos38>(ctx, p, level);
  if (ctx->plan.topo == 2) return lin_static_launch_t<TopoChain6>(ctx, p, level);
#define DDP_TOPO_LAUNCH(ID, TOPO) if (ctx->plan.topo == (ID) - 1) return lin_static_launch_t<TOPO>(ctx, p, level);
  DDP_TOPO_EXTRA(DDP_TOPO_LAUNCH)
#undef DDP_TOPO_LAUNCH
  return DDP_HIP_E_UNSUPPORTED;
}
```

Baseline: 712.3.

## Store second-order dynamics tensors in packed per-column record layout

Adds a packed storage format for fxx/fux/fuu in which each column keeps only the nonzero structure (two top-block entries plus the lower nv rows). The linearization kernels write this compact layout and the backward half-contraction kernel reads it through a templated path, with an unpack kernel that restores the dense form when the host or other consumers need full tensors. The goal is to cut memory traffic for writing and reading the large second-order tensors, at the cost of extra indexing logic and a lazy unpack step on other access paths.

```diff
diff --git a/ddp_pinocchio_amd/csrc/bwd.hip b/ddp_pinocchio_amd/csrc/bwd.hip
--- a/ddp_pinocchio_amd/csrc/bwd.hip
+++ b/ddp_pinocchio_amd/csrc/bwd.hip
@@ -20,6 +20,7 @@
   const BwdJob* jobs_half;
   int32_t njobs_half;
   int32_t half_mode;
+  int32_t packed;
   const double *u, *ctrl_lo, *ctrl_hi;
   double* box_stat;
   int32_t has_tensors;
@@ -518,6 +519,7 @@
   p.jobs_half = plan.half_mode ? ctx->jobs_half_d : nullptr;
   p.njobs_half = plan.half_mode ? ctx->njobs_half : 0;
   p.half_mode = plan.half_mode;
+  p.packed = plan.packed ? 1 : 0;
   p.has_tensors = (ctx->flags & DDP_HIP_FLAG_NO_TENSORS) ? 0 : 1;
   return p;
 }
@@ -554,7 +556,8 @@
     prof_end(ctx, DDP_HIP_K_BWD_GAINS);
     if (p.has_tensors) {
       prof_begin(ctx, DDP_HIP_K_BWD_ASSEMBLE);
-      if (p.jobs_half) hipLaunchKernelGGL((bwd_contract_half<NC, MC>), dim3((unsigned)p.njobs_half, B), dim3(BSF), lds_h, ctx->stream, p, t);
+      if (p.jobs_half && p.packed) hipLaunchKernelGGL((bwd_contract_half<NC, MC, true>), dim3((unsigned)p.njobs_half, B), dim3(BSF), lds_h, ctx->stream, p, t);
+      else if (p.jobs_half) hipLaunchKernelGGL((bwd_contract_half<NC, MC, false>), dim3((unsigned)p.njobs_half, B), dim3(BSF), lds_h, ctx->stream, p, t);
       else hipLaunchKernelGGL((bwd_contract<NC, MC>), dim3((unsigned)ctx->njobs, B), dim3(BSF), lds_c, ctx->stream, p, t);
       prof_end(ctx, DDP_HIP_K_BWD_ASSEMBLE);
     }
@@ -588,7 +591,7 @@
 int launch_sweep_v2(ddp_hip_ctx* ctx, const BwdParams& p0) {
   const uint32_t bwd_mask = (2u << DDP_HIP_K_BWD_ASSEMBLE) | (2u << DDP_HIP_K_BWD_GAINS);
   if (ctx->sw.bwd_no_graph || (ctx->profile_mask & bwd_mask)) return enqueue_sweep_v2<NC, MC, BOX>(ctx, p0);
-  const uint64_t key_misc = (uint64_t)p0.has_tensors | ((uint64_t)(p0.vx_trace != nullptr) << 1) | ((uint64_t)p0.sym_tensors << 2) | ((uint64_t)(p0.jobs_half != nullptr) << 3) | ((uint64_t)p0.half_mode << 4);
+  const uint64_t key_misc = (uint64_t)p0.has_tensors | ((uint64_t)(p0.vx_trace != nullptr) << 1) | ((uint64_t)p0.sym_tensors << 2) | ((uint64_t)(p0.jobs_half != nullptr) << 3) | ((uint64_t)p0.half_mode << 4) | ((uint64_t)p0.packed << 8);
   auto find = [&](const void* key_x) -> ddp_hip_ctx::BwdGraph* {
     for (auto& g : ctx->bwd_graph)
       if (g.exec && g.key_x == key_x && g.key_misc == key_misc) return &g;
@@ -625,7 +628,7 @@
   const TensorOrigin o = ctx->tensors.origin;
   s.sym = s.sym_ok && (o == TensorOrigin::Symmetric || o == TensorOrigin::Stencil);
   const bool half_ok = s.fast && ctx->jobs_half_d && !sw.k3_no_half;
-  if (half_ok && s.sym && o == TensorOrigin::Stencil) s.half_mode = 1;
+  if (half_ok && s.sym && o == TensorOrigin::Stencil) { s.half_mode = 1; s.packed = ctx->tensors.packed; }
   else if (half_ok && o == TensorOrigin::Analytic1) s.half_mode = 2;
   return s;
 }
@@ -700,7 +703,12 @@
   const Dims& d = ctx->d;
   const int64_t B = d.batch;
   HIP_TRY(hipSetDevice(ctx->device));
-  const SweepPlan plan = sweep_plan(ctx);
+  SweepPlan plan = sweep_plan(ctx);
+  if (ctx->tensors.packed && !plan.packed) {
+    const int rc_ = lin_materialize_fxx(ctx);
+    if (rc_ != DDP_HIP_OK) return rc_;
+    plan = sweep_plan(ctx);
+  }
   BwdParams p = make_params(ctx, plan);
   if (p.has_tensors && (!p.fxx || !p.fux || !p.fuu)) return DDP_HIP_E_UNSUPPORTED;
   const bool box = (ctx->flags & DDP_HIP_FLAG_CONTROL_BOUNDS) != 0;
diff --git a/ddp_pinocchio_amd/csrc/bwd_split.h b/ddp_pinocchio_amd/csrc/bwd_split.h
--- a/ddp_pinocchio_amd/csrc/bwd_split.h
+++ b/ddp_pinocchio_amd/csrc/bwd_split.h
@@ -117,7 +117,7 @@
 };
 static_assert(38 % 2 == 0, "row pairs");
 
-template <int N, int M>
+template <int N, int M, bool PK>
 __global__ __launch_bounds__(BSF, BWD_WAVES_PER_SIMD) void bwd_contract_half(BwdParams p, int64_t t) {
   int b, jb;
   {
@@ -165,6 +165,8 @@
   double top0[2], top1[2], top2[2], top3[2];
   auto issue = [&](int u, f64x2 (&buf)[HS::R], double (&top)[2]) {
     const f64x2* base = reinterpret_cast<const f64x2*>(unit_base(u));
+    const bool two = !(kind == 10 && u < 2);
+    auto rec_word = [&](int jj) -> int { return (two && jj >= m) ? (N * M) / 2 + (jj - m) * (HS::HP + 1) : jj * (HS::HP + 1); };
 #pragma unroll
     for (int r = 0; r < HS::R; ++r) {
       const int f = tid + r * BSF;
@@ -172,16 +174,23 @@
       const int jj = f / HS::HP, ip = f - jj * HS::HP;
       int slab, j; bool xcol;
       if (need) need = col_info(u, jj < n ? jj : n - 1, slab, j, xcol) && !(m1 && kind == 11);
-      if (need) buf[r] = BWD_NT ? __builtin_nontemporal_load(&base[jj * (N / 2) + HS::HP + ip]) : base[jj * (N / 2) + HS::HP + ip];
+      const int w = PK ? rec_word(jj) + 1 + ip : jj * (N / 2) + HS::HP + ip;
+      if (need) buf[r] = BWD_NT ? __builtin_nontemporal_load(&base[w]) : base[w];
       else buf[r] = f64x2{0.0, 0.0};
     }
     top[0] = 0.0; top[1] = 0.0;
     if (tid < n) {
       int slab, j; bool xcol;
       if (col_info(u, tid, slab, j, xcol) && kind == 10 && !m1) {
-        const double* colp = unit_base(u) + (int64_t)tid * n;
-        top[0] = colp[slab % M];
-        if (xcol && (j % M) != (slab % M)) top[1] = colp[j % M];
+        if constexpr (PK) {
+          const f64x2 tw = base[rec_word(tid)];
+          top[0] = tw.x;
+          if (xcol && (j % M) != (slab % M)) top[1] = tw.y;
+        } else {
+          const double* colp = unit_base(u) + (int64_t)tid * n;
+          top[0] = colp[slab % M];
+          if (xcol && (j % M) != (slab % M)) top[1] = colp[j % M];
+        }
       }
     }
   };
diff --git a/ddp_pinocchio_amd/csrc/ctx.hip b/ddp_pinocchio_amd/csrc/ctx.hip
--- a/ddp_pinocchio_amd/csrc/ctx.hip
+++ b/ddp_pinocchio_amd/csrc/ctx.hip
@@ -210,6 +210,7 @@
   sw.generic_bwd = on("DDP_HIP_GENERIC_BWD");
   sw.k3_no_sym = on("DDP_HIP_K3_NO_SYM");
   sw.k3_no_half = on("DDP_HIP_K3_NO_HALF");
+  sw.k3_no_pack = on("DDP_HIP_K3_NO_PACK");
   sw.fxx_full = on("DDP_HIP_FXX_FULL");
   sw.no_static = on("DDP_HIP_NO_STATIC");
   sw.no_qcache = on("DDP_HIP_NO_QCACHE");
@@ -416,7 +417,7 @@
 
 extern "C" double* ddp_hip_device_ptr(ddp_hip_ctx* ctx, int seq) {
   if (!ctx || seq < 0 || seq >= DDP_HIP_SEQ_COUNT) return nullptr;
-  if (seq == DDP_HIP_SEQ_FXX || seq == DDP_HIP_SEQ_FUU) (void)hipSetDevice(ctx->device);
+  if (seq == DDP_HIP_SEQ_FXX || seq == DDP_HIP_SEQ_FUX || seq == DDP_HIP_SEQ_FUU) (void)hipSetDevice(ctx->device);
   if (tensors_written_outside(ctx, seq) != DDP_HIP_OK) return nullptr;
   return ctx->seq[seq].ptr;
 }
@@ -487,7 +488,7 @@
   if (sz == 0 || count == 0) return DDP_HIP_OK;
   if (!host) return DDP_HIP_E_ARG;
   HIP_TRY(hipSetDevice(ctx->device));
-  if (seq == DDP_HIP_SEQ_FXX || seq == DDP_HIP_SEQ_FUU) { const int rc_ = lin_materialize_fxx(ctx); if (rc_ != DDP_HIP_OK) return rc_; }
+  if (seq == DDP_HIP_SEQ_FXX || seq == DDP_HIP_SEQ_FUU || (seq == DDP_HIP_SEQ_FUX && ctx->tensors.packed)) { const int rc_ = lin_materialize_fxx(ctx); if (rc_ != DDP_HIP_OK) return rc_; }
   HIP_TRY(hipMemcpyAsync(host, ctx->seq[seq].ptr + first * sz, sizeof(double) * (size_t)(sz * count), hipMemcpyDeviceToHost, ctx->stream));
   HIP_TRY(hipStreamSynchronize(ctx->stream));
   return DDP_HIP_OK;
diff --git a/ddp_pinocchio_amd/csrc/internal.h b/ddp_pinocchio_amd/csrc/internal.h
--- a/ddp_pinocchio_amd/csrc/internal.h
+++ b/ddp_pinocchio_amd/csrc/internal.h
@@ -57,6 +57,7 @@
   bool generic_bwd = false;
   bool k3_no_sym = false;
   bool k3_no_half = false;
+  bool k3_no_pack = false;
   bool fxx_full = false;
   bool no_static = false;
   bool no_qcache = false;
@@ -76,6 +77,7 @@
   bool sym_ok;
   bool sym;
   int32_t half_mode;
+  bool packed;
 };
 
 enum class LinFirst : int32_t {
@@ -120,6 +122,7 @@
   bool has_tensors = false;
   bool skip_top = false;
   bool skip_qv_mirror = false;
+  bool pack = false;
   bool ws_lin = false, ws_qws = false, ws_qws2 = false;
   bool ws_ana_T = false, ws_ana_M = false, ws_ana_M0 = false, ws_ana_A = false, ws_ana_F = false;
   bool ws_eq = false;
@@ -138,6 +141,7 @@
 struct TensorState {
   TensorOrigin origin = TensorOrigin::Unknown;
   bool mirror_pending = false;
+  bool packed = false;
 };
 
 struct LinCall {
diff --git a/ddp_pinocchio_amd/csrc/lin.hip b/ddp_pinocchio_amd/csrc/lin.hip
--- a/ddp_pinocchio_amd/csrc/lin.hip
+++ b/ddp_pinocchio_amd/csrc/lin.hip
@@ -899,6 +899,33 @@
   }
 }
 
+constexpr int UNPACK_BS = 256;
+__global__ __launch_bounds__(UNPACK_BS) void tensor_unpack_kernel(double* fxx, double* fux, double* fuu, int n, int m, int nv) {
+  extern __shared__ __attribute__((aligned(16))) double s_rec[];
+  const int per = 2 * n + m;
+  const int64_t bt = blockIdx.x / per;
+  const int s = (int)(blockIdx.x % per);
+  double* slab;
+  int L, c;
+  bool tops;
+  if (s < n) { c = s; L = n; tops = true; slab = fxx + (bt * n + c) * (int64_t)n * n; }
+  else if (s < 2 * n) { c = s - n; L = m; tops = true; slab = fux + (bt * n + c) * (int64_t)n * m; }
+  else { c = s - 2 * n; L = m; tops = false; slab = fuu + (bt * m + c) * (int64_t)n * m; }
+  const int R = nv + 2, words = L * R;
+  for (int e = threadIdx.x; e < words; e += UNPACK_BS) s_rec[e] = slab[e];
+  __syncthreads();
+  const int r0 = c % nv;
+  for (int e = threadIdx.x; e < L * n; e += UNPACK_BS) {
+    const int j = e / n, k = e - j * n;
+    const double* rec = s_rec + j * R;
+    double v = 0.0;
+    if (k >= nv) v = rec[2 + (k - nv)];
+    else if (tops && k == r0) v = rec[0];
+    else if (tops && L == n && k == j % nv) v = rec[1];
+    slab[e] = v;
+  }
+}
+
 LinParams make_params(ddp_hip_ctx* ctx) {
   LinParams p{};
   p.d = ctx->d;
@@ -918,6 +945,7 @@
   p.has_tensors = pl.has_tensors ? 1 : 0;
   p.skip_top = pl.skip_top ? 1 : 0;
   p.skip_qv_mirror = pl.skip_qv_mirror ? 1 : 0;
+  p.pack = pl.pack ? 1 : 0;
   p.eq_xk = ctx->eq_ws;
   if (p.eq_xk) { p.eq_fxk = p.eq_xk + pl.eq_fxk_off; p.eq_c = p.eq_xk + pl.eq_c_off; }
   p.qcache = ctx->lin_ws;
@@ -1088,8 +1116,9 @@
 int tensors_begin_second(ddp_hip_ctx* ctx, const LinParams& p, LinCall& call) {
   const TensorOrigin was = ctx->tensors.origin;
   ctx->tensors.origin = TensorOrigin::Unknown;
+  ctx->tensors.packed = false;
   call.fuu_zero = was == TensorOrigin::Analytic1;
-  if (p.skip_top && was != TensorOrigin::Stencil) {
+  if (p.skip_top && !p.pack && was != TensorOrigin::Stencil) {
     const int64_t BT = ctx->d.batch * ctx->d.T, n = ctx->d.n, m = ctx->d.m;
     const int nv = (int)ctx->d.nv;
     hipLaunchKernelGGL(tensor_zero_top_kernel, dim3(8192), dim3(256), 0, ctx->stream, p.fxx, BT * n * n, (int)n, nv);
@@ -1105,6 +1134,7 @@
   if (ctx->model_h.fd_mode == 1) t.origin = call.fuu_zero ? TensorOrigin::Analytic1 : TensorOrigin::Unknown;
   else t.origin = p.skip_top ? TensorOrigin::Stencil : TensorOrigin::Symmetric;
   t.mirror_pending = p.skip_qv_mirror != 0;
+  t.packed = p.pack != 0;
 }
 
 }
@@ -1172,6 +1202,7 @@
 int tensors_written_outside(ddp_hip_ctx* ctx, int seq) {
   if (seq != DDP_HIP_SEQ_FXX && seq != DDP_HIP_SEQ_FUX && seq != DDP_HIP_SEQ_FUU) return DDP_HIP_OK;
   TensorState& t = ctx->tensors;
+  if (t.packed) { const int rc_ = lin_materialize_fxx(ctx); if (rc_ != DDP_HIP_OK) return rc_; }
   if (seq == DDP_HIP_SEQ_FUX) {
     t.origin = (t.origin == TensorOrigin::Symmetric || t.origin == TensorOrigin::Stencil) ? TensorOrigin::Symmetric : TensorOrigin::Unknown;
     return DDP_HIP_OK;
@@ -1183,9 +1214,19 @@
 }
 
 int lin_materialize_fxx(ddp_hip_ctx* ctx) {
-  if (!ctx->tensors.mirror_pending) return DDP_HIP_OK;
   double* fxx = ctx->seq[DDP_HIP_SEQ_FXX].ptr;
   double* fuu = ctx->seq[DDP_HIP_SEQ_FUU].ptr;
+  if (ctx->tensors.packed) {
+    double* fux = ctx->seq[DDP_HIP_SEQ_FUX].ptr;
+    const int64_t BT = ctx->d.batch * ctx->d.T, n = ctx->d.n, m = ctx->d.m, nv = ctx->d.nv;
+    if (!fxx || !fux || !fuu || m > n) return DDP_HIP_E_UNSUPPORTED;
+    hipLaunchKernelGGL(tensor_unpack_kernel, dim3((unsigned)(BT * (2 * n + m))), dim3(UNPACK_BS), sizeof(double) * (size_t)(n * (nv + 2)), ctx->stream,
+                       fxx, fux, fuu, (int)n, (int)m, (int)nv);
+    HIP_TRY(hipGetLastError());
+    HIP_TRY(hipStreamSynchronize(ctx->stream));
+    ctx->tensors.packed = false;
+  }
+  if (!ctx->tensors.mirror_pending) return DDP_HIP_OK;
   if (fxx && fuu) {
     const int64_t BT = ctx->d.batch * ctx->d.T;
     hipLaunchKernelGGL(tensor_mirror_kernel, dim3(8192), dim3(256), 0, ctx->stream, fxx, BT, (int)ctx->d.n, (int)ctx->d.n);
diff --git a/ddp_pinocchio_amd/csrc/lin_common.h b/ddp_pinocchio_amd/csrc/lin_common.h
--- a/ddp_pinocchio_amd/csrc/lin_common.h
+++ b/ddp_pinocchio_amd/csrc/lin_common.h
@@ -17,6 +17,7 @@
   double* qcache;
   int32_t skip_qv_mirror;
   int32_t skip_top;
+  int32_t pack;
   double* accel_out;
   int32_t ncfg, nvcfg;
   const double *xref, *wx, *uref, *wu;
diff --git a/ddp_pinocchio_amd/csrc/lin_plan.cpp b/ddp_pinocchio_amd/csrc/lin_plan.cpp
--- a/ddp_pinocchio_amd/csrc/lin_plan.cpp
+++ b/ddp_pinocchio_amd/csrc/lin_plan.cpp
@@ -38,6 +38,7 @@
   pl.ws_qws2 = pl.second == LinSecond::Mode2Static && sw.cfg_full_aba;
   pl.skip_top = pl.topo && mode == 2 && tensors && !sw.fxx_full;
   pl.skip_qv_mirror = pl.skip_top && sweep_sym_ok;
+  pl.pack = pl.skip_qv_mirror && pl.second == LinSecond::Mode2Static && !sw.k3_no_half && !sw.k3_no_pack;
 
   const bool m1_wave = wave && pl.second == LinSecond::Mode1Wave;
   pl.ana_sliced = analytic && !small;
@@ -74,7 +75,7 @@
   static const char* const sw_names[] = {"none", "generic_bwd", "k3_no_sym", "k3_no_half", "fxx_full", "no_static", "no_qcache",
                                          "cfg_full_aba", "ana_own_aba", "ana_split", "ana_eq_kernel", "bwd_no_graph", "solve_sync"};
   printf("kind nv ff fo_fd mode tensors etot eq_kind K matched sw sym_ok created refuse nj topo first second eq eq_jac eq_second "
-         "eq_inline accel_static accel_with_u m1_fused ncfg nvcfg has_tensors skip_top skip_qv_mirror ws_lin ws_qws ws_qws2 ws_ana_T "
+         "eq_inline accel_static accel_with_u m1_fused ncfg nvcfg has_tensors skip_top skip_qv_mirror pack ws_lin ws_qws ws_qws2 ws_ana_T "
          "ws_ana_M ws_ana_M0 ws_ana_A ws_ana_F ws_eq ana_sliced eq_fxk_off eq_c_off eq_words lin_path first_order\n");
   printf("#");
   for (const char* s : sw_names) printf(" %s", s);
@@ -99,11 +100,11 @@
     const bool created = (kind == DDP_HIP_MODEL_TREE || (nv == 1 && !ff)) && (!ff || (nv >= 6 && mode != 1 && eqk != DDP_HIP_EQ_CONFIG)) &&
                          (eqk != DDP_HIP_EQ_NONE || !etot);
     const LinPlan p = lin_plan_decide(m, d, tensors ? 0u : (uint32_t)DDP_HIP_FLAG_NO_TENSORS, sw, matched && !ff ? 1 : 0, sym_ok != 0);
-    printf("%d %d %d %d %d %d %d %d %d %d %d %d %d %d %d %d %d %d %d %d %d %d %d %d %d %d %d %d %d %d %d %d %d %d %d %d %d %d %d %d %lld %lld %lld %d %d\n",
+    printf("%d %d %d %d %d %d %d %d %d %d %d %d %d %d %d %d %d %d %d %d %d %d %d %d %d %d %d %d %d %d %d %d %d %d %d %d %d %d %d %d %d %lld %lld %lld %d %d\n",
            kind == DDP_HIP_MODEL_TREE, nv, ff, fo, mode, tensors, etot, eqk == DDP_HIP_EQ_NONE ? 0 : eqk == DDP_HIP_EQ_CONFIG ? 1 : 2, K, matched, s, sym_ok,
            (int)created, p.refuse != 0, p.nj, p.topo, (int)p.first, (int)p.second, (int)p.eq, (int)p.eq_jac, (int)p.eq_second,
            (int)p.eq_inline, (int)p.accel_static, (int)p.accel_with_u, (int)p.m1_fused, p.ncfg, p.nvcfg, (int)p.has_tensors, (int)p.skip_top,
-           (int)p.skip_qv_mirror, (int)p.ws_lin, (int)p.ws_qws, (int)p.ws_qws2, (int)p.ws_ana_T, (int)p.ws_ana_M, (int)p.ws_ana_M0, (int)p.ws_ana_A,
+           (int)p.skip_qv_mirror, (int)p.pack, (int)p.ws_lin, (int)p.ws_qws, (int)p.ws_qws2, (int)p.ws_ana_T, (int)p.ws_ana_M, (int)p.ws_ana_M0, (int)p.ws_ana_A,
            (int)p.ws_ana_F, (int)p.ws_eq, (int)p.ana_sliced, (long long)p.eq_fxk_off, (long long)p.eq_c_off, (long long)p.eq_words, p.lin_path, p.first_order);
   }
   return 0;
diff --git a/ddp_pinocchio_amd/csrc/lin_static.hip b/ddp_pinocchio_amd/csrc/lin_static.hip
--- a/ddp_pinocchio_amd/csrc/lin_static.hip
+++ b/ddp_pinocchio_amd/csrc/lin_static.hip
@@ -214,15 +214,18 @@
   jj = (int)(q - (int64_t)a * (2 * Wd - a - 1) / 2) + a + 1;
 }
 
+template <int NV> __device__ __forceinline__ int rec_row(bool pack, int k, int r0) { return !pack ? k : (k >= NV ? k - NV + 2 : (k == r0 ? 0 : 1)); }
+template <int NV> __device__ __forceinline__ bool rec_zero(bool pack, int k, int r0) { return pack && k < NV && k != r0; }
+
 template <int NV, int NP = LBS>
 struct OutStage {
   double qdd[NP * (NV + 1)];
   int pij[NP];
 };
 
-template <int NV, int NP>
-__device__ __forceinline__ void offdiag_emit(const LinParams& p, OutStage<NV, NP>& S, bool valid, int i, int j, int64_t bt,
-                                             const double* __restrict__ xg, double dt, int pass = 0) {
+template <int NV, int NP, bool PACK, bool UU>
+__device__ __forceinline__ void offdiag_emit_as(const LinParams& p, OutStage<NV, NP>& S, bool valid, int i, int j, int64_t bt,
+                                                const double* __restrict__ xg, double dt, int pass) {
   constexpr int n = 2 * NV, mm = NV;
   constexpr int RW = 16, NJ = (n + RW - 1) / RW, GRP = LBS / RW, PPG = NP / GRP, NB = NP == LBS ? 2 : 1;
   static_assert(PPG % NB == 0, "points per group");
@@ -238,6 +241,9 @@
   __syncthreads();
   const int kk = lane % RW, grp = lane / RW;
   const double* f0 = p.f_val + bt * n;
+  constexpr bool pack = PACK, uu = UU && PACK;
+  const bool skip_top = PACK || p.skip_top != 0;
+  constexpr int cs = pack ? NV + 2 : n;
   double f0k[NJ], xk[NJ], xvk[NJ];
 #pragma unroll
   for (int jx = 0; jx < NJ; ++jx) {
@@ -252,7 +258,7 @@
     double a1[NB][NJ], a2[NB][NJ], d1[NB][NJ], d2[NB][NJ];
     double* o0[NB];
     double* o1[NB];
-    int ie[NB], je[NB], ee[NB];
+    int ie[NB], je[NB], ee[NB], r2[NB];
 #pragma unroll
     for (int u = 0; u < NB; ++u) {
       const int e = (pt + u) * GRP + grp;
@@ -261,24 +267,29 @@
       const int i1 = pk & 255, j1 = (pk >> 8) & 255;
       ie[u] = i1;
       je[u] = j1;
-      const bool at_x_1 = i1 < n, at_x_2 = j1 < n;
+      const bool at_x_1 = !uu && i1 < n, at_x_2 = !uu && j1 < n;
       const int idx_1 = at_x_1 ? i1 : i1 - n, idx_2 = at_x_2 ? j1 : j1 - n;
       double* tensor;
       int L;
       if (at_x_1) { if (at_x_2) { tensor = fxx; L = n; } else { tensor = fux; L = mm; } }
       else { tensor = fuu; L = mm; }
-      o0[u] = (pk >> 16) ? tensor + (int64_t)idx_2 * n + (int64_t)idx_1 * n * L : nullptr;
+      r2[u] = at_x_1 ? idx_1 % NV : -1;
+      o0[u] = (pk >> 16) ? tensor + (int64_t)idx_2 * cs + (int64_t)idx_1 * n * L : nullptr;
       o1[u] = ((pk >> 16) && at_x_1 == at_x_2 && !p.skip_qv_mirror) ? tensor + (int64_t)idx_1 * n + (int64_t)idx_2 * n * L : nullptr;
       if (o0[u]) {
         const double* q0 = at_x_1 ? fxb + (int64_t)idx_1 * n : fub + (int64_t)idx_1 * n;
         const double* q1 = at_x_2 ? fxb + (int64_t)idx_2 * n : fub + (int64_t)idx_2 * n;
-        const double* q2 = at_x_1 ? fxx + (int64_t)idx_1 * n + (int64_t)idx_1 * n * n : fuu + (int64_t)idx_1 * n + (int64_t)idx_1 * n * mm;
-        const double* q3 = at_x_2 ? fxx + (int64_t)idx_2 * n + (int64_t)idx_2 * n * n : fuu + (int64_t)idx_2 * n + (int64_t)idx_2 * n * mm;
+        const double* q2 = at_x_1 ? fxx + (int64_t)idx_1 * cs + (int64_t)idx_1 * n * n : fuu + (int64_t)idx_1 * cs + (int64_t)idx_1 * n * mm;
+        const double* q3 = at_x_2 ? fxx + (int64_t)idx_2 * cs + (int64_t)idx_2 * n * n : fuu + (int64_t)idx_2 * cs + (int64_t)idx_2 * n * mm;
+        const int r3 = at_x_2 ? idx_2 % NV : -1;
 #pragma unroll
         for (int jx = 0; jx < NJ; ++jx) {
           const int k = kk + RW * jx;
           const int kc = k < n ? k : n - 1;
-          a1[u][jx] = q0[kc]; a2[u][jx] = q1[kc]; d1[u][jx] = q2[kc]; d2[u][jx] = q3[kc];
+          a1[u][jx] = q0[kc]; a2[u][jx] = q1[kc];
+          const double v2 = q2[rec_row<NV>(pack, kc, r2[u])], v3 = q3[rec_row<NV>(pack, kc, r3)];
+          d1[u][jx] = rec_zero<NV>(pack, kc, r2[u]) ? 0.0 : v2;
+          d2[u][jx] = rec_zero<NV>(pack, kc, r3) ? 0.0 : v3;
         }
       }
     }
@@ -289,7 +300,7 @@
       for (int jx = 0; jx < NJ; ++jx) {
         const int k = kk + RW * jx;
         if (k >= n) continue;
-        if (p.skip_top && k < NV && !((ie[u] < n && ie[u] % NV == k) || (je[u] < n && je[u] % NV == k))) continue;
+        if (skip_top && k < NV && (uu || !((ie[u] < n && ie[u] % NV == k) || (je[u] < n && je[u] % NV == k)))) continue;
         double xs = k == ie[u] ? xk[jx] + eps : xk[jx];
         if (k == je[u]) xs = xs + eps;
         double fv;
@@ -306,11 +317,18 @@
         df -= eps * a2[u][jx];
         df *= 2;
         const double val = 0.5 * (df / eps2 - d1[u][jx] - d2[u][jx]);
-        o0[u][k] = val;
+        o0[u][rec_row<NV>(pack, k, r2[u])] = val;
         if (o1[u]) o1[u][k] = val;
       }
     }
   }
+}
+
+template <int NV, int NP>
+__device__ __forceinline__ void offdiag_emit(const LinParams& p, OutStage<NV, NP>& S, bool valid, int i, int j, int64_t bt,
+                                             const double* __restrict__ xg, double dt, int pass = 0) {
+  if (p.pack) offdiag_emit_as<NV, NP, true, false>(p, S, valid, i, j, bt, xg, dt, pass);
+  else offdiag_emit_as<NV, NP, false, false>(p, S, valid, i, j, bt, xg, dt, pass);
 }
 
 template <int NV>
@@ -322,9 +340,10 @@
 __device__ __forceinline__ void rowblock_emit(const ST& S, int lane, int i, int jb, double* __restrict__ out, double* __restrict__ mirror,
                                               int64_t mstride, const double* __restrict__ a2, const double* __restrict__ d2, int64_t dstride,
                                               double dt, const double* __restrict__ f0g, const double* __restrict__ a1g,
-                                              double* __restrict__ d1g, const double* __restrict__ xg, bool skip_top = false) {
+                                              double* __restrict__ d1g, const double* __restrict__ xg, bool skip_top = false, bool pack = false) {
   constexpr int n = 2 * NV, RW = 16, NJ = (n + RW - 1) / RW, CG = LBS / RW, NIT = (NV + CG - 1) / CG;
   const int r1 = i % NV;
+  const int cs = pack ? NV + 2 : n;
   const double eps = sqrt(sqrt(DBL_EPSILON));
   const double eps2 = eps * eps;
   const int kk = lane % RW, cg = lane / RW;
@@ -354,21 +373,24 @@
       df *= 2;
       const double dd = df / eps2;
       d1k[j] = dd;
-      if (cg == 0 && k < n && !(skip_top && k < NV && k != r1)) d1g[k] = dd;
+      if (cg == 0 && k < n && !(skip_top && k < NV && k != r1)) d1g[rec_row<NV>(pack, k, r1)] = dd;
     } else {
-      d1k[j] = d1g[kc];
+      const double v = d1g[rec_row<NV>(pack, kc, r1)];
+      d1k[j] = rec_zero<NV>(pack, kc, r1) ? 0.0 : v;
     }
   }
   double va2[2][NJ], vd2[2][NJ];
   auto fetch = [&](int it, double (&A)[NJ], double (&D)[NJ]) {
     const int c = it * CG + cg;
     const int cc = c < NV ? c : NV - 1;
+    const int rd = jb + cc < n ? (jb + cc) % NV : -1;
 #pragma unroll
     for (int j = 0; j < NJ; ++j) {
       const int k = kk + RW * j;
       const int kc = k < n ? k : n - 1;
       A[j] = a2[kc + cc * n];
-      D[j] = d2[kc + cc * dstride];
+      const double v = d2[rec_row<NV>(pack, kc, rd) + cc * dstride];
+      D[j] = rec_zero<NV>(pack, kc, rd) ? 0.0 : v;
     }
   };
   auto form = [&](int it, const double (&A)[NJ], const double (&D)[NJ]) {
@@ -397,7 +419,7 @@
       df -= eps * A[j];
       df *= 2;
       const double val = 0.5 * (df / eps2 - d1k[j] - D[j]);
-      out[k + c * n] = val;
+      out[rec_row<NV>(pack, k, r1) + c * cs] = val;
       if (mirror) mirror[k + c * mstride] = val;
     }
   };
@@ -413,7 +435,7 @@
   }
 }
 
-template <class T, bool ROWS>
+template <class T, bool ROWS, bool PACK = false>
 __global__ __launch_bounds__(LBS, ROWS ? 1 : 3) void lin_static_tau_kernel(LinParams p) {
   constexpr int nv = T::N, n = 2 * nv;
   constexpr int TRI = nv * (nv - 1) / 2, GU = (TRI + LBS - 1) / LBS, G = ROWS ? 2 * nv : GU;
@@ -471,13 +493,15 @@
 #pragma unroll
     for (int k = 0; k < nv; ++k) S.q[row * (nv + 1) + k] = s.uu[k];
     __syncthreads();
+    const bool pack = kp->pack != 0;
+    const int64_t cs = pack ? nv + 2 : n;
     rowblock_emit<nv, true>(S, lane, i, n, kp->fux + bt * n * mm * n + (int64_t)i * n * mm, nullptr, 0, kp->fu + bt * n * mm,
-                            kp->fuu + bt * n * mm * mm, (int64_t)n + (int64_t)n * mm, m.dt, kp->f_val + bt * n,
-                            kp->fx + bt * n * n + (int64_t)i * n, kp->fxx + bt * n * n * n + (int64_t)i * n + (int64_t)i * n * n, xg, kp->skip_top != 0);
+                            kp->fuu + bt * n * mm * mm, cs + (int64_t)n * mm, m.dt, kp->f_val + bt * n,
+                            kp->fx + bt * n * n + (int64_t)i * n, kp->fxx + bt * n * n * n + (int64_t)i * cs + (int64_t)i * n * n, xg, kp->skip_top != 0, pack);
   } else {
     OutStage<nv, LBS / 2>& S = s_lds.O;
     LinParams po;
-    po.f_val = kp->f_val; po.fx = kp->fx; po.fu = kp->fu; po.fxx = kp->fxx; po.fux = kp->fux; po.fuu = kp->fuu; po.skip_qv_mirror = kp->skip_qv_mirror; po.skip_top = kp->skip_top;
+    po.f_val = kp->f_val; po.fx = kp->fx; po.fu = kp->fu; po.fxx = kp->fxx; po.fux = kp->fux; po.fuu = kp->fuu; po.skip_qv_mirror = kp->skip_qv_mirror; po.skip_top = kp->skip_top; po.pack = kp->pack;
     const double dt = m.dt;
     __syncthreads();
 #pragma unroll 1
@@ -487,7 +511,7 @@
 #pragma unroll
         for (int k = 0; k < nv; ++k) S.qdd[(lane % (LBS / 2)) * (nv + 1) + k] = s.uu[k];
       }
-      offdiag_emit<nv, LBS / 2>(po, S, valid, i, j, bt, xg, dt, pass);
+      offdiag_emit_as<nv, LBS / 2, PACK, true>(po, S, valid, i, j, bt, xg, dt, pass);
     }
   }
 }
@@ -747,14 +771,16 @@
 #pragma unroll
     for (int k = 0; k < nv; ++k) S.q[row * (nv + 1) + k] = s.uu[k];
     __syncthreads();
-    rowblock_emit<nv, false>(S, lane, i, nv, fxx + (int64_t)nv * n + (int64_t)i * n * n,
+    const bool pack = kp->pack != 0;
+    const int64_t cs = pack ? nv + 2 : n;
+    rowblock_emit<nv, false>(S, lane, i, nv, fxx + (int64_t)nv * cs + (int64_t)i * n * n,
                              kp->skip_qv_mirror ? nullptr : fxx + (int64_t)i * n + (int64_t)nv * n * n, (int64_t)n * n,
-                             fxb + (int64_t)nv * n, fxx + (int64_t)nv * n + (int64_t)nv * n * n, (int64_t)n + (int64_t)n * n, dt,
-                             kp->f_val + bt * n, fxb + (int64_t)i * n, fxx + (int64_t)i * n + (int64_t)i * n * n, c.xg, kp->skip_top != 0);
+                             fxb + (int64_t)nv * n, fxx + (int64_t)nv * cs + (int64_t)nv * n * n, cs + (int64_t)n * n, dt,
+                             kp->f_val + bt * n, fxb + (int64_t)i * n, fxx + (int64_t)i * cs + (int64_t)i * n * n, c.xg, kp->skip_top != 0, pack);
   } else {
     constexpr int NP = LBS / 2;
     LinParams po;
-    po.f_val = kp->f_val; po.fx = kp->fx; po.fu = kp->fu; po.fxx = kp->fxx; po.fux = kp->fux; po.fuu = kp->fuu; po.skip_qv_mirror = kp->skip_qv_mirror; po.skip_top = kp->skip_top;
+    po.f_val = kp->f_val; po.fx = kp->fx; po.fu = kp->fu; po.fxx = kp->fxx; po.fux = kp->fux; po.fuu = kp->fuu; po.skip_qv_mirror = kp->skip_qv_mirror; po.skip_top = kp->skip_top; po.pack = kp->pack;
     __syncthreads();
     double* const own = &S.O.qdd[(lane % NP) * (nv + 1)];
     double* const row = lane < NP ? own : S.spare;
@@ -1044,7 +1070,7 @@
   typedef __attribute__((address_space(4))) const LinParams* kernarg_t;
   const kernarg_t kp = (kernarg_t)__builtin_amdgcn_kernarg_segment_ptr();
   LinParams po;
-  po.f_val = kp->f_val; po.fx = kp->fx; po.fu = kp->fu; po.fxx = kp->fxx; po.fux = kp->fux; po.fuu = kp->fuu; po.skip_qv_mirror = kp->skip_qv_mirror; po.skip_top = kp->skip_top;
+  po.f_val = kp->f_val; po.fx = kp->fx; po.fu = kp->fu; po.fxx = kp->fxx; po.fux = kp->fux; po.fuu = kp->fuu; po.skip_qv_mirror = kp->skip_qv_mirror; po.skip_top = kp->skip_top; po.pack = kp->pack;
   offdiag_emit<nv, LBS>(po, S, valid, c.i, c.j, bt, c.xg, model->dt);
 }
 
@@ -1272,14 +1298,14 @@
   typedef __attribute__((address_space(4))) const LinParams* kernarg_t;
   const kernarg_t kp = (kernarg_t)__builtin_amdgcn_kernarg_segment_ptr();
   LinParams po;
-  po.f_val = kp->f_val; po.fx = kp->fx; po.fu = kp->fu; po.fxx = kp->fxx; po.fux = kp->fux; po.fuu = kp->fuu; po.skip_qv_mirror = kp->skip_qv_mirror; po.skip_top = kp->skip_top;
+  po.f_val = kp->f_val; po.fx = kp->fx; po.fu = kp->fu; po.fxx = kp->fxx; po.fux = kp->fux; po.fuu = kp->fuu; po.skip_qv_mirror = kp->skip_qv_mirror; po.skip_top = kp->skip_top; po.pack = kp->pack;
   offdiag_emit<nv, LBS>(po, S, valid, c.i, c.j, bt, c.xg, c.m->dt);
 }
 
 template <int NV, bool DIAG>
 __device__ __forceinline__ void first_output(const double* q , int lane, int d0, double* __restrict__ out,
                                              int64_t ostride, const double* __restrict__ fcol, const double* __restrict__ f0,
-                                             const double* __restrict__ xg, double dt, double eps, bool skip_top = false) {
+                                             const double* __restrict__ xg, double dt, double eps, bool skip_top = false, bool pack = false) {
   constexpr int n = 2 * NV, TOT = NV * n;
   const double eps2 = eps * eps;
   for (int e = lane; e < TOT; e += LBS) {
@@ -1301,7 +1327,7 @@
       double df = fv - f0[k];
       df -= eps * fcol[e];
       df *= 2;
-      out[k + c * ostride] = df / eps2;
+      out[rec_row<NV>(pack, k, d < n ? d % NV : -1) + c * ostride] = df / eps2;
     } else {
       out[e] = (fv - f0[k]) / eps;
     }
@@ -1383,10 +1409,12 @@
   double* out = fcol;
   int64_t ostride = n;
   if constexpr (DIAG) {
-    if (LEVEL == 3) { out = kp->fuu + bt * n * nv * nv; ostride = n + (int64_t)n * nv; }
-    else { ostride = n + (int64_t)n * n; out = kp->fxx + bt * n * n * n + (LEVEL == 2 ? nv * ostride : 0); }
-  }
-  first_output<nv, DIAG>(s_q, lane, LEVEL == 1 ? 0 : (LEVEL == 2 ? nv : n), out, ostride, fcol, kp->f_val + bt * n, xg, model->dt, eps, kp->skip_top != 0);
+    const int64_t cs = kp->pack ? nv + 2 : n;
+    if (LEVEL == 3) { out = kp->fuu + bt * n * nv * nv; ostride = cs + (int64_t)n * nv; }
+    else { ostride = cs + (int64_t)n * n; out = kp->fxx + bt * n * n * n + (LEVEL == 2 ? nv * ostride : 0); }
+  }
+  first_output<nv, DIAG>(s_q, lane, LEVEL == 1 ? 0 : (LEVEL == 2 ? nv : n), out, ostride, fcol, kp->f_val + bt * n, xg, model->dt, eps, kp->skip_top != 0,
+                         DIAG && kp->pack != 0);
 }
 
 template <class T, int K>
@@ -1674,7 +1702,8 @@
   constexpr int nv = T::N, TRI = nv * (nv - 1) / 2, GU = (TRI + LBS - 1) / LBS;
   if (level == StaticLevel::Torque) {
     hipLaunchKernelGGL((lin_static_tau_kernel<T, true>), dim3((unsigned)(BT * 2 * nv)), dim3(LBS), 0, ctx->stream, p);
-    hipLaunchKernelGGL((lin_static_tau_kernel<T, false>), dim3((unsigned)(BT * GU)), dim3(LBS), 0, ctx->stream, p);
+    if (p.pack) hipLaunchKernelGGL((lin_static_tau_kernel<T, false, true>), dim3((unsigned)(BT * GU)), dim3(LBS), 0, ctx->stream, p);
+    else hipLaunchKernelGGL((lin_static_tau_kernel<T, false, false>), dim3((unsigned)(BT * GU)), dim3(LBS), 0, ctx->stream, p);
   } else if (level == StaticLevel::Caches) {
     hipLaunchKernelGGL((lin_static_qvcache_kernel<T>), dim3((unsigned)((BT * p.ncfg + LBS - 1) / LBS)), dim3(LBS), 0, ctx->stream, p, p.model, p.x, p.qcache, p.vcache);
     if (p.nvcfg > 1) hipLaunchKernelGGL((lin_static_vcache_kernel<T>), dim3((unsigned)BT), dim3(LBS), 0, ctx->stream, p, p.model, p.x, p.qcache, p.vcache);
```

After: 727.7, median of 6. +2.2%, better.
